# tenstack/batch-scheduler

Hardware: AMD Instinct MI355X
Metric: pod x node fit evals/sec (higher is better)
Workload: dtype int64; 1 GPU; cfg3/tail: 10000 pods / 2000 groups / 5000 nodes, 5 int64 lanes (cpu, mem, eph, pods, gpu), seed 20260921; stages=prefilter+filter+tally+ready, parallelism=single GPU

## Files before the change

### batch-scheduler_amd/build.py

```python
from __future__ import annotations

import os
import shutil
import subprocess

HERE = os.path.dirname(os.path.abspath(__file__))
CSRC = os.path.join(HERE, "csrc")
LIB_DIR = os.environ.get("BS_LIB_DIR") or HERE
PREBUILT_ONLY = bool(os.environ.get("BS_LIB_DIR"))
LIB_PATH = os.path.join(LIB_DIR, "libbsched.so")
_COMMON = ["bs_common.hpp", "bs_kernels.hpp", "bs_nodew_layout.hpp", "bs_lanes.hpp", os.path.join("..", "..", "include", "bsched.h")]
_CTX = _COMMON + ["bs_ctx.hpp", "bs_carve.hpp", "bs_hostmem.hpp", "bs_pod_ranges.hpp"]
_FAST = ["bs_launch.hpp", "bs_fast.hpp", "bs_filter_t.hpp"]
_SEQ = _CTX + ["bs_seq.hpp"]
UNITS = {
    "bsched.hip": _CTX + _FAST + ["bs_epoch.hpp", "bs_queue.hpp", "bs_fdeny.hpp", "bs_sort.hpp", "bs_fit.hpp"],
    "tu_fast.hip": _COMMON + _FAST,
    "tu_seq.hip": _SEQ,
    "tu_seq_expire.hip": _SEQ + ["bs_seq_expire.hpp", "bs_seq_expire_list.hpp"],
    "tu_preempt.hip": _CTX + ["bs_preempt.hpp", "bs_preempt_commit.hpp", "bs_preempt_commit_gang.hpp", "bs_preempt_gang_runs.hpp", "bs_preempt_geom.hpp", "bs_bound_apply.hpp",
                              "bs_bound_nodes.hpp", "bs_bound_nodes_replay.hpp", "bs_pdb.hpp"],
}
SOURCES = list(UNITS)
LATER_UNITS = {
    "tu_wait.hip": _SEQ + ["bs_wait.hpp", "bs_wait_list.hpp"],
}
ALL_UNITS = {**UNITS, **LATER_UNITS}
ALL_SOURCES = list(ALL_UNITS)
HEADERS = sorted({h for hs in ALL_UNITS.values() for h in hs})
OBJ_DIR = os.path.join(HERE, "build")
FLAGS = ["--offload-arch=gfx950", "-O3", "-std=c++17", "-fPIC", "-ffp-contract=off",
         "-fno-fast-math", "-Wall", "-Wno-unused-function"]


def hipcc() -> str:
    exe = shutil.which("hipcc") or "/opt/rocm/bin/hipcc"
    if not os.path.exists(exe):
        raise RuntimeError("hipcc not found: the gfx950 library cannot be built")
    return exe


HOST_LIB_PATH = os.path.join(LIB_DIR, "libbsched_host.so")
HOST_SRC = os.path.join(HERE, "host", "bs_host.cpp")
HOST_SRCS = [HOST_SRC, os.path.join(HERE, "host", "bs_drain.cpp"), os.path.join(HERE, "host", "bs_phase.cpp")]


def build_host(force: bool = False, verbose: bool = False) -> str:
    build()
    if PREBUILT_ONLY:
        return HOST_LIB_PATH
    deps = [*HOST_SRCS, os.path.join(HERE, "..", "include", "bsched.h"), os.path.join(HERE, "..", "include", "bsched_host.h"), LIB_PATH]
    if not force and os.path.exists(HOST_LIB_PATH) and all(os.path.getmtime(d) <= os.path.getmtime(HOST_LIB_PATH) for d in deps):
        return HOST_LIB_PATH
    cxx = shutil.which("g++") or "g++"
    tmp = f"{HOST_LIB_PATH}.{os.getpid()}.tmp"
    cmd = [cxx, "-O2", "-std=c++17", "-fPIC", "-shared", "-Wall", "-o", tmp, *HOST_SRCS, "-L" + HERE, "-lbsched",
           "-Wl,-rpath,$ORIGIN"]
    if verbose:
        print(" ".join(cmd))
    res = subprocess.run(cmd, capture_output=True, text=True)
    if res.returncode != 0:
        raise RuntimeError("g++ failed:\n" + res.stdout + res.stderr)
    os.replace(tmp, HOST_LIB_PATH)
    return HOST_LIB_PATH

# ... 77 lines not shown
```

### batch-scheduler_amd/capi.py

```python
from __future__ import annotations

import ctypes as C
import os

import numpy as np

from . import fitspec, soa

HERE = os.path.dirname(os.path.abspath(__file__))
LIB_PATH = os.path.join(os.environ.get("BS_LIB_DIR") or HERE, "libbsched.so")

KERNEL_COUNT = 8
KERNEL_PREPASS, KERNEL_LEADER, KERNEL_QUERY, KERNEL_TABLES, KERNEL_SCAN, KERNEL_RESOLVE, KERNEL_FILTER, KERNEL_TALLY = range(8)

ABI_SYMBOLS = [
    "bs_abi_version", "bs_strerror", "bs_last_error", "bs_create", "bs_destroy",
    "bs_nodes_load", "bs_fit_load", "bs_fit_build", "bs_fit_read", "bs_groups_load", "bs_groups_read", "bs_groups_apply", "bs_pods_map", "bs_pods_load",
    "bs_pods_apply", "bs_pods_count", "bs_pods_read", "bs_pods_apply_stats", "bs_filter_deny_stats", "bs_speculation_stats",
    "bs_nodes_apply", "bs_nodes_count", "bs_nodes_assume",
    "bs_cluster_fits", "bs_node_left", "bs_scan_prefix", "bs_cluster_total", "bs_filter_one", "bs_find_max_pg",
    "bs_batch_run", "bs_batch_sync", "bs_batch_read", "bs_batch_map", "bs_filter_rows_count", "bs_queue_order_load", "bs_queue_sort",
    "bs_shard_set", "bs_reduce_external", "bs_group_admit_devptr", "bs_group_admit_bind", "bs_stream", "bs_comm_unique_id", "bs_comm_init", "bs_batch_finish",
    "bs_timing_reset", "bs_timing_get", "bs_kernel_name", "bs_batch_stats_get",
    "bs_seq_run", "bs_nodes_read", "bs_first_reach_hint",
    "bs_nodes_load_flat", "bs_groups_load_flat", "bs_groups_read_flat", "bs_pods_load_flat", "bs_pods_apply_flat", "bs_pods_read_flat",
    "bs_batch_read_flat", "bs_seq_run_flat", "bs_fit_build_flat",
    "bs_bound_load", "bs_bound_count", "bs_preempt_run", "bs_bound_load_flat", "bs_preempt_run_flat",
    "bs_preempt_commit", "bs_bound_read", "bs_preempt_commit_flat",
    "bs_bound_pdb_set", "bs_preempt_pdb_read",
    "bs_bound_apply", "bs_bound_apply_flat", "bs_bound_ids", "bs_bound_dump",
    "bs_bound_nodes_apply",
    "bs_bound_apply_ex", "bs_bound_apply_ex_flat",
    "bs_pdb_load", "bs_pdb_members_append", "bs_pdb_allowed_apply", "bs_pdb_read",
    "bs_preempt_commit_gang", "bs_preempt_commit_gang_flat", "bs_preempt_gang_read",
    "bs_seq_expire", "bs_seq_expire_flat", "bs_seq_waiting_read",
    "bs_wait_load", "bs_wait_count", "bs_wait_ids", "bs_wait_read", "bs_wait_park", "bs_wait_release", "bs_wait_expire", "bs_wait_forget",
]

SEQ_EXPIRE_DENY, SEQ_EXPIRE_ALL = 1, 2
WAIT_MAX = 1 << 24

BS_BOUND_NODES = soa.BS_BOUND_NODES

PROTECTED_PHASES = (2, 5)


def group_protected(phases) -> np.ndarray:
    ph = np.asarray(phases, dtype=np.int64).reshape(-1)
    return np.isin(ph, PROTECTED_PHASES).astype(np.uint8)


def gang_order(pod_group, priority) -> np.ndarray:
    grp = np.asarray(pod_group, np.int64).reshape(-1)
    pri = np.asarray(priority, np.int64).reshape(-1)
    assert grp.shape == pri.shape
    first: dict = {}
    rank = np.zeros(grp.shape[0], np.int64)
    for i in range(grp.shape[0]):
        key = (int(pri[i]), int(grp[i])) if grp[i] >= 0 else (int(pri[i]), -1 - i)
        rank[i] = first.setdefault(key, i)
    return np.lexsort((np.arange(grp.shape[0]), rank, -pri)).astype(np.int64)


def gang_need(groups, waiting=None) -> np.ndarray:
    mm = np.asarray(groups.min_member, np.int64).reshape(-1)
    w = np.zeros_like(mm) if waiting is None else np.asarray(waiting, np.int64).reshape(-1)
    assert w.shape == mm.shape
    return np.clip(mm - np.asarray(groups.status_scheduled, np.int64).reshape(-1) - w, 0, None).astype(np.uint32)


class BsError(RuntimeError):
# ... 35 lines not shown

class SeqOut(C.Structure):
    _fields_ = [("pf_code", C.POINTER(C.c_uint8)), ("pf_first_k", C.POINTER(C.c_uint32)), ("pf_leader", C.POINTER(C.c_int32)),
                ("pod_node", C.POINTER(C.c_int32)), ("cap", C.c_uint32), ("released_group", C.POINTER(C.c_uint32)),
                ("released_pods", C.POINTER(C.c_uint32)), ("first_ns", C.POINTER(C.c_int64)), ("ready_ns", C.POINTER(C.c_int64)),
                ("n_released", C.c_uint32), ("total_ns", C.c_int64), ("node_picks", C.c_uint64), ("node_scans", C.c_uint64),
                ("scan_rounds", C.c_uint64), ("pick_rounds", C.c_uint64), ("leader_folds", C.c_uint64), ("table_builds", C.c_uint64),
                ("last_permitted", C.POINTER(C.c_uint8))]


class SeqExpireOut(C.Structure):
    _fields_ = [("n_groups", C.c_uint32), ("n_pods", C.c_uint32), ("group_cap", C.c_uint32), ("group", C.POINTER(C.c_uint32)),
                ("group_pods", C.POINTER(C.c_uint32)), ("group_earlier", C.POINTER(C.c_uint32)), ("pod_cap", C.c_uint32),
                ("pod", C.POINTER(C.c_uint32)), ("node", C.POINTER(C.c_uint32))]


_lib = None


def load_library(path: str | None = None):
    global _lib
    if _lib is not None and path is None:
        return _lib
    p = path or LIB_PATH
    if not os.path.exists(p):
        raise BsError(-2, "load_library", f"{p} not built: run `python __graft_entry__.py build` (hipcc, gfx950)")
    L = C.CDLL(p)
    vp, u32, i32, u8 = C.c_void_p, C.c_uint32, C.c_int32, C.c_uint8
    P = C.POINTER
    L.bs_abi_version.restype = u32
    L.bs_strerror.restype = C.c_char_p
    L.bs_strerror.argtypes = [C.c_int]
    L.bs_last_error.restype = C.c_char_p
    L.bs_last_error.argtypes = [vp]
    L.bs_kernel_name.restype = C.c_char_p
    L.bs_kernel_name.argtypes = [u32]
    L.bs_create.argtypes = [P(Config), P(vp)]
    L.bs_destroy.argtypes = [vp]
    L.bs_nodes_load.argtypes = [vp, P(soa.NodesStruct)]
    L.bs_fit_load.argtypes = [vp, u32, P(u32)]
    L.bs_fit_build.argtypes = [vp, P(fitspec.NodeLabelsStruct), P(fitspec.FitTemplatesStruct)]
    L.bs_fit_read.argtypes = [vp, P(u32)]
    L.bs_groups_load.argtypes = [vp, P(soa.GroupsStruct)]
    L.bs_groups_read.argtypes = [vp, P(soa.GroupsStruct)]
    L.bs_groups_apply.argtypes = [vp, P(soa.GroupDelta), u32]
    L.bs_filter_rows_count.argtypes = [vp, P(u32)]
    L.bs_pods_load.argtypes = [vp, P(soa.PodsStruct)]
    L.bs_pods_map.argtypes = [vp, u32, P(soa.PodsStruct)]
    L.bs_pods_apply.argtypes = [vp, P(soa.PodsDeltaStruct)]
    L.bs_pods_count.argtypes = [vp, P(u32)]
    L.bs_pods_apply_stats.argtypes = [vp, P(C.c_uint64), P(C.c_uint64)]
    L.bs_filter_deny_stats.argtypes = [vp, P(C.c_uint64)]
    L.bs_speculation_stats.argtypes = [vp, P(C.c_uint64), P(C.c_uint64)]
    L.bs_pods_read.argtypes = [vp, P(soa.PodsOutStruct)]
    L.bs_queue_order_load.argtypes = [vp, u32, P(u32)]
    L.bs_queue_sort.argtypes = [vp, u32, P(i32), P(i32), P(C.c_int64), P(u32)]
    L.bs_nodes_apply.argtypes = [vp, P(NodeDelta), u32]
    L.bs_nodes_count.argtypes = [vp, P(u32)]
    L.bs_nodes_assume.argtypes = [vp, P(NodeRequest), u32]
    L.bs_cluster_fits.argtypes = [vp, u32, C.c_float, P(C.c_int64), u32, P(u8), P(u32)]
    L.bs_node_left.argtypes = [vp, u32, C.c_float, P(C.c_int64), P(u32)]
    L.bs_scan_prefix.argtypes = [vp, u32, C.c_float, P(C.c_int64), P(u32), P(u32), P(u32)]
    L.bs_cluster_total.argtypes = [vp, u32, P(C.c_int64), P(u32)]
    L.bs_filter_one.argtypes = [vp, i32, P(C.c_int64), u32, i32, u32, P(u8), P(u8)]
    L.bs_find_max_pg.argtypes = [vp, P(i32), P(u32), P(u8)]
    L.bs_batch_run.argtypes = [vp, u32]
    L.bs_batch_sync.argtypes = [vp]
    L.bs_batch_read.argtypes = [vp, P(soa.BatchOutStruct)]
    L.bs_batch_map.argtypes = [vp, P(soa.BatchViewStruct)]
    L.bs_shard_set.argtypes = [vp, u32, u32]
    L.bs_group_admit_devptr.argtypes = [vp, P(vp), P(u32)]
    L.bs_reduce_external.argtypes = [vp, u32]
    L.bs_first_reach_hint.argtypes = [vp, u32]
    L.bs_group_admit_bind.argtypes = [vp, vp]
    L.bs_stream.argtypes = [vp, P(vp)]
    L.bs_comm_unique_id.argtypes = [P(u8)]
    L.bs_comm_init.argtypes = [vp, P(u8), u32, u32]
    L.bs_batch_finish.argtypes = [vp]
    L.bs_timing_reset.argtypes = [vp]
    L.bs_timing_get.argtypes = [vp, P(Timing)]
    L.bs_batch_stats_get.argtypes = [vp, P(BatchStats)]
    L.bs_seq_run.argtypes = [vp, u32, P(SeqOut)]
    L.bs_nodes_read.argtypes = [vp, P(C.c_int64), P(u32)]
    L.bs_bound_load.argtypes = [vp, P(soa.BoundStruct)]
    L.bs_bound_count.argtypes = [vp, P(u32)]
    L.bs_preempt_run.argtypes = [vp, u32, u32, P(u32), P(i32), P(u8), u32, P(soa.PreemptOutStruct)]
    L.bs_bound_load_flat.argtypes = [vp, u32, P(u32), P(i32), P(C.c_int64), P(i32), P(C.c_int64), P(u32)]
    L.bs_preempt_run_flat.argtypes = [vp, u32, u32, P(u32), P(i32), P(u8), u32, P(i32), P(u32), P(u32), P(u32), P(i32), P(C.c_int64), P(C.c_int64)]
    L.bs_preempt_commit.argtypes = [vp, u32, u32, P(u32), P(i32), P(u8), u32, u32, P(soa.PreemptOutStruct)]
    L.bs_bound_read.argtypes = [vp, P(u32), P(u32)]
    L.bs_bound_pdb_set.argtypes = [vp, u32, P(u8)]
    L.bs_bound_apply.argtypes = [vp, P(soa.BoundDeltaStruct), P(u32)]
    L.bs_bound_apply_flat.argtypes = [vp, u32, P(u32), u32, P(u32), P(i32), P(C.c_int64), P(i32), P(C.c_int64), P(u32), P(u8), P(u32)]
    L.bs_bound_apply_ex.argtypes = [vp, P(soa.BoundDeltaStruct), u32, P(u32)]
    L.bs_bound_apply_ex_flat.argtypes = [vp, u32, u32, P(u32), u32, P(u32), P(i32), P(C.c_int64), P(i32), P(C.c_int64), P(u32), P(u8), P(u32)]
    L.bs_bound_ids.argtypes = [vp, P(u32)]
    L.bs_bound_nodes_apply.argtypes = [vp, u32, P(u32), P(u32), u32, P(u32), P(u32)]
    L.bs_bound_dump.argtypes = [vp, P(i32), P(C.c_int64), P(i32), P(C.c_int64), P(u32), P(u8)]
    L.bs_preempt_pdb_read.argtypes = [vp, u32, P(u32)]
    L.bs_pdb_load.argtypes = [vp, u32, P(i32), u32, P(u32), P(u32)]
    L.bs_pdb_members_append.argtypes = [vp, u32, u32, P(u32), P(u32)]
    L.bs_pdb_allowed_apply.argtypes = [vp, u32, P(u32), P(i32)]
    L.bs_pdb_read.argtypes = [vp, P(u32), P(u32), P(i32), P(u32)]
    L.bs_preempt_commit_flat.argtypes = [vp, u32, u32, P(u32), P(i32), P(u8), u32, u32, P(i32), P(u32), P(u32), P(u32), P(i32), P(C.c_int64),
                                         P(C.c_int64)]
    L.bs_preempt_commit_gang.argtypes = [vp, u32, u32, P(u32), P(i32), P(u8), P(u32), u32, u32, P(soa.PreemptOutStruct)]
# ... 133 lines not shown
            return np.ctypeslib.as_array(C.cast(ptr, C.POINTER(ctype * n)).contents).view(dtype).reshape(shape)
        pods = soa.Pods.__new__(soa.Pods)
        pods.group = view(st.group, C.c_int32, np.int32, (p,))
        pods.req = view(st.req, C.c_int64, np.int64, (self.L, p))
        pods.req_present = view(st.req_present, C.c_uint32, np.uint32, (p,))
        pods.cls = view(st.cls, C.c_uint32, np.uint32, (p,))
        pods.owner = view(st.owner, C.c_uint64, np.uint64, (p,))
        pods.flags = view(st.flags, C.c_uint8, np.uint8, (p,))
        return pods

    def apply_group_deltas_raw(self, arr, n: int):
        self._chk(self._lib.bs_groups_apply(self._h, arr, n), "bs_groups_apply")

    def load_pods(self, pods: soa.Pods):
        assert pods.req.shape[0] == self.L
        st = pods.as_struct()
        self._chk(self._lib.bs_pods_load(self._h, C.byref(st)), "bs_pods_load")
        self.p = pods.p

    def apply_pods(self, remove=(), flag_index=(), flag_value=(), insert: soa.Pods | None = None, insert_at=None):
        rem = np.ascontiguousarray(remove, np.uint32)
        fi = np.ascontiguousarray(flag_index, np.uint32)
        fv = np.ascontiguousarray(flag_value, np.uint8)
        assert fi.shape == fv.shape
        d = soa.PodsDeltaStruct()
        d.n_remove, d.remove = len(rem), _u32p(rem if len(rem) else np.zeros(1, np.uint32))
        d.n_flags, d.flag_index = len(fi), _u32p(fi if len(fi) else np.zeros(1, np.uint32))
        d.flag_value = (fv if len(fv) else np.zeros(1, np.uint8)).ctypes.data_as(C.POINTER(C.c_uint8))
        keep = [rem, fi, fv]
        if insert is not None and insert.p:
            assert insert.req.shape[0] == self.L
            d.insert = insert.as_struct()
            if insert_at is not None:
                at = np.ascontiguousarray(insert_at, np.uint32)
                assert len(at) == insert.p
                keep.append(at)
                d.insert_at = _u32p(at)
        self._chk(self._lib.bs_pods_apply(self._h, C.byref(d)), "bs_pods_apply")
        self.p = self.pods_count()

    def apply_pods_raw(self, delta: "soa.PodsDeltaStruct"):
        self._chk(self._lib.bs_pods_apply(self._h, C.byref(delta)), "bs_pods_apply")

    def apply_stats(self) -> tuple[int, int]:
        a, r = C.c_uint64(0), C.c_uint64(0)
        self._chk(self._lib.bs_pods_apply_stats(self._h, C.byref(a), C.byref(r)), "bs_pods_apply_stats")
        return int(a.value), int(r.value)

    def speculation_stats(self) -> tuple[int, int]:
        a, m = C.c_uint64(0), C.c_uint64(0)
        self._chk(self._lib.bs_speculation_stats(self._h, C.byref(a), C.byref(m)), "bs_speculation_stats")
        return int(a.value), int(m.value)

    def filter_deny_reruns(self) -> int:
        r = C.c_uint64(0)
        self._chk(self._lib.bs_filter_deny_stats(self._h, C.byref(r)), "bs_filter_deny_stats")
        return int(r.value)

    def pods_count(self) -> int:
        n = C.c_uint32(0)
        self._chk(self._lib.bs_pods_count(self._h, C.byref(n)), "bs_pods_count")
        return int(n.value)

    def read_pods(self) -> soa.Pods:
        p = self.pods_count()
        out = soa.Pods.empty(max(p, 1), self.L)
        st = soa.PodsOutStruct(p, *[getattr(out.as_struct(), k) for k in ("group", "req", "req_present", "cls", "owner", "flags")])
        if p:
            out = soa.Pods.empty(p, self.L)
            s2 = out.as_struct()
            st = soa.PodsOutStruct(p, s2.group, s2.req, s2.req_present, s2.cls, s2.owner, s2.flags)
        self._chk(self._lib.bs_pods_read(self._h, C.byref(st)), "bs_pods_read")
        return out if p else soa.Pods.empty(0, self.L)

    def apply_node_deltas(self, deltas: list):
        arr = (NodeDelta * len(deltas))(*deltas)
        self._chk(self._lib.bs_nodes_apply(self._h, arr, len(deltas)), "bs_nodes_apply")
        n = C.c_uint32(0)
        self._chk(self._lib.bs_nodes_count(self._h, C.byref(n)), "bs_nodes_count")
        self.n = int(n.value)

    def assume_nodes(self, reqs):
        reqs = list(reqs)
        arr = (NodeRequest * max(len(reqs), 1))()
        for k, (idx, lanes, pres) in enumerate(reqs):
            arr[k].index, arr[k].requested_present = int(idx), int(pres)
            for j, v in enumerate(lanes):
                arr[k].requested[j] = int(v)
        self._chk(self._lib.bs_nodes_assume(self._h, arr, len(reqs)), "bs_nodes_assume")

    def cluster_fits(self, cls: int, pct: float, req, present: int = 0):
        r = np.zeros(soa.MAX_LANES, np.int64)
        r[: len(req)] = req
        fits, fk = C.c_uint8(0), C.c_uint32(0)
        self._chk(self._lib.bs_cluster_fits(self._h, cls, float(np.float32(pct)), _i64p(r), present, C.byref(fits), C.byref(fk)),
                  "bs_cluster_fits")
        return bool(fits.value), int(fk.value)

    def node_left(self, cls: int, pct: float):
        left = np.zeros((self.L, self.n), np.int64)
        present = np.zeros(max(self.n, 1), np.uint32)
        self._chk(self._lib.bs_node_left(self._h, cls, float(np.float32(pct)), _i64p(left), _u32p(present)), "bs_node_left")
        return left, present[: self.n]

    def scan_prefix(self, cls: int, pct: float):
        n = max(self.n, 1)
# ... 407 lines not shown
```

### batch-scheduler_amd/csrc/bs_ctx.hpp

```cpp
#pragma once
#include <rccl/rccl.h>

#include <algorithm>
#include <string>
#include <vector>

#include "bs_carve.hpp"
#include "bs_hostmem.hpp"
#include "bs_kernels.hpp"
#include "bs_lanes.hpp"
#include "bs_pod_ranges.hpp"

namespace bs {

struct EventPair { hipEvent_t a, b; uint32_t id; };

inline size_t align256(size_t x) { return (x + 255) & ~(size_t)255; }
template <class T>
T* at(T* p, size_t n) { return p ? p + n : nullptr; }

struct PodLayout {
  Piece<int32_t> group;
  Piece<int64_t> req;
  Piece<uint32_t> pres, cls, pclass, ppair;
  Piece<uint64_t> owner;
  Piece<uint8_t> flags;
  size_t in_bytes = 0, bytes = 0;
  uint32_t p = 0;
};
inline PodLayout pod_layout(uint32_t P, uint32_t L) {
  const size_t n = std::max<uint32_t>(P, 1);
  PodLayout l;
  Carve cv;
  l.group = cv.take<int32_t>(n);
  l.req = cv.take<int64_t>(n * L);
  l.pres = cv.take<uint32_t>(n);
  l.cls = cv.take<uint32_t>(n);
  l.owner = cv.take<uint64_t>(n);
  l.flags = cv.take<uint8_t>(n);
  l.in_bytes = cv.mark();
  l.pclass = cv.take<uint32_t>(n);
  l.ppair = cv.take<uint32_t>(n);
  l.bytes = cv.mark();
  l.p = P;
  return l;
}

extern const char* const kKernelNames[BS_KERNEL_COUNT];
int use_device(bs_ctx* c, bool flush = true);
int settle_pending(bs_ctx* c);
NodesDev nodes_dev(const bs_ctx* c);
GroupsDev groups_dev(const bs_ctx* c);
PodsDev pods_dev(const bs_ctx* c);
uint32_t* pclass_dev(const bs_ctx* c);
void launch_nodes_assume(bs_ctx* c, const bs_node_request* records, uint32_t n);
void mirror_node_requests(bs_ctx* c, const bs_node_request* records, uint32_t n);
void rederive_nodes(bs_ctx* c, uint32_t base0 = 0, uint32_t m_before = 0);
int analyse_groups(bs_ctx* c, bool rearm_scratch = true, const bs_group_delta* deltas = nullptr, uint32_t ndeltas = 0, bool defer = false);
int maybe_analyse_epochs(bs_ctx* c);
int check_handover(bs_ctx* c);

}

using namespace bs;

struct bs_ctx {
  bs_config cfg{};
  uint32_t L = 4, S = 0, LP = 4;
  std::string last_error;

  bool have_nodes = false, have_fit = false, have_groups = false, have_pods = false;
  uint32_t N = 0, Ncap = 0, M = 0, C = 0, fit_words = 0;
  DevBuf d_alloc, d_nreq, d_apres, d_rpres, d_nflags, d_fit, d_kmap, d_m, d_left4, d_lglob;
  DevBuf d_fitarena, d_fitcols;
  std::vector<int64_t> h_alloc, h_nreq;
  std::vector<uint32_t> h_apres, h_rpres, h_kmap;
  std::vector<uint8_t> h_nflags;
  std::vector<uint32_t> h_fit;

  uint32_t G = 0, n_uncaptured = 0;
  std::vector<uint32_t> h_gmatched, h_gcls;
  std::vector<uint8_t> h_gflags;
  int32_t steady_table = -1;
  int32_t steady_prev = -1;
  bool spec_active = false;
  int32_t spec_table = -1;
  uint32_t spec_stages = 0;
  uint32_t no_spec = 0;
  uint64_t n_spec = 0, n_spec_miss = 0;
  uint32_t host_probe = 0;
  uint64_t hp_ns[6] = {0, 0, 0, 0, 0, 0}, hp_n = 0, hp_t0 = 0, hp_t1 = 0;
  uint64_t early_filter_min = 200000000ull;
  DevBuf d_gpack, d_info, d_gdelta;
  Piece<uint32_t> off_gmm, off_gsc, off_gmatched, off_gcls, off_gmrpres;
  Piece<uint8_t> off_gflags;
  Piece<int64_t> off_gminres;
  Piece<uint64_t> off_gocc;
  size_t gpack_bytes = 0;
  int32_t info_tag = 0, kinfo_tag = 0;
  bool info_pending = false, kinfo_pending = false;
  uint32_t max_group_cls = 0, max_pod_cls = 0;
  uint32_t h_K = 0;
  uint32_t k_bound = 0;

  uint32_t P = 0;
  DevBuf d_pack[2], d_outpack;
  PodLayout lay[2], stage_lay;
  uint32_t cur_pack = 0;
  bool last_use_classes = false;
  uint32_t map_p = 0;
  DevBuf d_gstat2, d_cdir, d_pdir, d_ckeys, d_cpres, d_pkeys;
  uint32_t gstat_cur = 0;
  uint32_t pair_cap = 0, dir_slots = 0;
  uint32_t ids_used = 0;
  bool rep_valid = false;
  bool dirs_ready = false;
  uint32_t id_room = 0;
  uint32_t serial_insert_max = 2048;
  uint64_t n_applies = 0, n_rederives = 0;
  Piece<uint8_t> off_pf_code, off_fl_code, off_ready;
  Piece<uint32_t> off_pf_first_k, off_fl_feasible, off_fl_slot, off_admit;
  Piece<int32_t> off_pf_leader;
  size_t outpack_bytes = 0;

  DevBuf d_first_elig, d_first_owner, d_first_reject, d_first_pod, d_cap_epoch;
  DevBuf d_epoch, d_nepochs, d_leader_epoch, d_panic_epoch;
  DevBuf d_tcode, d_stage, d_leader_raw, d_first_row, d_first_row64, d_scan_rec, d_feas_rec, d_chunk_rec, d_qreq_s, d_qflags_s, d_qpos;
  DevBuf d_needed, d_qcount, d_ticket, d_desc;
  bool scratch_armed = false;
  bool side_ready = false;
  DevBuf d_tables, d_kp, d_stats, d_fparams, d_fflags, d_chunk_tot, d_blk_scratch, d_gmax, d_chunk_kp;
  DevBuf d_cls_slots, d_cls_rep, d_cls_id, d_qtab_s, d_fu_slot, d_uparams, d_uflags, d_uclaim, d_fu_bitmap, d_fu_feas;
  DevBuf d_nodew;
  bool batch_void = false;
  uint32_t tp_tmin = 768;
  bool no_nodew = false;
  uint32_t slot_keep = 0xFFFFFFFFu;
  uint32_t cls_cap = 0, hash_keep = 0x7FFFFFFFu, n_nominres = 0, scan_slots_cap = 0, filter_slots_cap = 0;
  DevBuf d_fl_bitmap, d_admit, d_ready, d_gcount, d_admit64, d_own_start;
  bool owner_ready = false;
  DevBuf d_order_rank, d_sort;
  uint32_t order_g = 0;
  DevBuf d_gstat, d_pair_next, d_pair_firstq, d_first_reach, d_qstamp_s, d_fast_reject, d_epoch_group;
  bool pairs_ready = false;
  bool bitmap_valid = false;
  bool last_fast = false;
  bool batch_since_pods = false;
  size_t off_hfeas = 0, off_htag = 0;
  uint32_t hstride = 0;
  int32_t host_tag = 0;
  bool last_host_out = false;
  uint32_t no_fast = 0;
  DevBuf d_run_of_epoch, d_run_leader, d_gslot, d_gfirstq;
// ... 127 lines not shown
```

### batch-scheduler_amd/csrc/bs_fast.hpp

```cpp
#pragma once

#include "bs_kernels.hpp"
#include "bs_filter_t.hpp"

#ifdef BS_NT_TABLES
#define BS_TBL_STORE(p, v) __builtin_nontemporal_store((v), (p))
#else
#define BS_TBL_STORE(p, v) (*(p) = (v))
#endif
namespace bs {

template <bool INL = false>
__device__ __forceinline__ void arm_tally(const GroupsDev& gr, const BatchDev& b, const BatchParams& prm, uint32_t i, uint32_t nthreads);

__device__ __forceinline__ const uint8_t* range_glocal(const BatchDev& b) { return reinterpret_cast<const uint8_t*>(b.pod_ranges); }
__device__ __forceinline__ const uint32_t* range_start(const BatchDev& b, uint32_t G) { return b.pod_ranges + (G + 3u) / 4u; }
__device__ __forceinline__ const uint32_t* range_lfirst(const BatchDev& b, uint32_t G, uint32_t pod_blocks) { return range_start(b, G) + pod_blocks + 1u; }
__device__ __forceinline__ bool range_local_on(const BatchDev& b, const BatchParams& prm) {
  return b.pod_ranges && prm.do_tally && prm.do_ready && !prm.filter_deny;
}

#if BS_EMIT_MAIN
__global__ void k_pods_prep(unsigned long long* tables, uint32_t ntab, uint32_t* gstat, uint32_t ngstat, uint32_t* kcount, uint32_t* gcount, uint32_t G) {
  const uint32_t t = blockIdx.x * blockDim.x + threadIdx.x, nt = gridDim.x * blockDim.x;
  for (uint32_t i = t; i < ntab; i += nt) tables[i] = 0ull;
  for (uint32_t i = t; i < G; i += nt) gcount[i] = 0;
  for (uint32_t i = t; i < ngstat; i += nt) gstat[i] = BS_INF;
  if (t == 0 && kcount) *kcount = 0;
}
#endif

#if BS_EMIT_MAIN
__global__ void k_pod_pairs(PodsDev pods, uint32_t G, const uint32_t* rep, const uint32_t* id, uint32_t* pclass, unsigned long long* slots, uint32_t mask,
                            uint32_t hash_keep, uint32_t* gstat, uint32_t* ppair, unsigned long long* pair_next, const uint32_t* kcount, int32_t tag,
                            int32_t* hinfo, uint32_t* gcount) {
  const uint32_t i = blockIdx.x * blockDim.x + threadIdx.x;
  if (i == 0 && hinfo) {
    __hip_atomic_store(reinterpret_cast<unsigned long long*>(&hinfo[4]), ((unsigned long long)(uint32_t)tag << 32) | *kcount, __ATOMIC_RELAXED, __HIP_MEMORY_SCOPE_SYSTEM);
  }
  {
    const int32_t gq = i < pods.p ? pods.group[i] : -1;
    const bool in = gq >= 0 && (uint32_t)gq < G;
    wave_aggregated_add(gcount, in ? (uint32_t)gq : 0u, in);
  }
  if (i >= pods.p) return;
  const uint32_t c = id[rep[i]];
  if (pclass) pclass[i] = c;
  const int32_t gi = pods.group[i];
  if (gi < 0 || (uint32_t)gi >= G) { ppair[i] = BS_INF; return; }
  atomicMin(&gstat[gi], i);
  if (!(pods.flags[i] & BS_POD_LAST_PERMITTED)) {
    atomicMin(&gstat[(size_t)G + gi], i);
    if (pods.owner[i] != 0) atomicMin(&gstat[(size_t)2 * G + gi], i);
// ... 162 lines not shown
      incl[j] += off;
      if (valid) BS_TBL_STORE(&T[(size_t)k * LP + j], (int64_t)incl[j]);
      if (threadIdx.x == 0) b.chunk_tot[(size_t)chunk * 16 + j] = tot;
    } else if (j < LP && valid) {
      BS_TBL_STORE(&T[(size_t)k * LP + j], (int64_t)INT64_MAX);
    }
  }
  {
    const uint32_t grp = k >> 6;
    const bool grp_valid = (chunk * kTblChunk + (threadIdx.x & ~63u)) < nd.m;
    constexpr int64_t kSafe = (int64_t)1 << 62;
#pragma unroll
    for (uint32_t j = 0; j < BS_MAX_LANES; ++j) {
      if (j < L) {
        const int64_t x = (int64_t)incl[j];
        const long long mx = wave_max_i64_lane63(valid ? x : INT64_MIN);
        const bool risky = __ballot(valid && (x >= kSafe || x <= -kSafe)) != 0ull;
        if (lane_id() == 63 && grp_valid) b.gmax[(size_t)grp * LP + j] = risky ? INT64_MAX : mx;
      }
    }
  }
#pragma unroll
  for (uint32_t s = 0; s < BS_MAX_SCALARS; ++s) {
    if (s < S) {
      const unsigned long long mk = __ballot(valid && (pres & (1u << s)));
      if (mk && lane_id() == 0) atomicMin(&s_kp[s], chunk * kTblChunk + (uint32_t)(threadIdx.x & ~63u) + (uint32_t)(__ffsll((long long)mk) - 1));
    }
  }
  __syncthreads();
  if (threadIdx.x < 16) b.chunk_kp[(size_t)chunk * 16 + threadIdx.x] = threadIdx.x < BS_MAX_SCALARS ? s_kp[threadIdx.x] : BS_INF;
}

struct LeaderPre { Res mr; bool have_mr; int64_t min_member, status_scheduled, matched; };
template <bool PUB, typename T>
__device__ __forceinline__ void st_pub(T* p, T v) {
  if constexpr (PUB) __hip_atomic_store(p, v, __ATOMIC_RELAXED, __HIP_MEMORY_SCOPE_AGENT);
  else *p = v;
}
#ifndef BS_HOME_WT
#define BS_HOME_WT 0
#endif
template <typename T>
__device__ __forceinline__ void st_home(T* p, T v) {
#if BS_HOME_WT
  __hip_atomic_store(p, v, __ATOMIC_RELAXED, __HIP_MEMORY_SCOPE_SYSTEM);
#else
  *p = v;
#endif
}
__device__ __forceinline__ uint32_t ld_agent(const uint32_t* p) { return __hip_atomic_load(p, __ATOMIC_RELAXED, __HIP_MEMORY_SCOPE_AGENT); }
__device__ __forceinline__ unsigned long long ld_agent64(const void* p) {
  return __hip_atomic_load(reinterpret_cast<const unsigned long long*>(p), __ATOMIC_RELAXED, __HIP_MEMORY_SCOPE_AGENT);
}
template <int TS>
__device__ __forceinline__ void leader_pre_load(const GroupsDev& gr, int32_t leader, Shape<TS> sh, LeaderPre& o) {
  const uint32_t l = leader >= 0 ? (uint32_t)leader : 0u;
#pragma unroll
  for (uint32_t j = 0; j < BS_MAX_LANES; ++j) o.mr.v[j] = j < sh.L() ? gr.minres[(size_t)j * gr.g + l] : 0;
  o.mr.present = gr.mrpres[l];
  o.have_mr = (gr.flags[l] & BS_GROUP_HAS_MINRES) != 0;
  o.min_member = (int64_t)gr.min_member[l];
  o.status_scheduled = (int64_t)gr.status_scheduled[l];
  o.matched = (int64_t)gr.matched[l];
}
template <int TS>
__device__ __forceinline__ void pre_allocated_from(const LeaderPre& lp, Shape<TS> sh, uint32_t gate, Res& out) {
  res_zero(out, sh);
  const int64_t mm = lp.min_member;
  const int64_t not_finished = lp.matched != 0 ? mm - lp.matched : mm - lp.status_scheduled;
  if (not_finished > 0 && lp.have_mr) {
    Res times;
#pragma unroll
    for (uint32_t j = 0; j < BS_MAX_LANES; ++j)
      if (j < sh.L()) times.v[j] = wmul(lp.mr.v[j], not_finished);
    times.present = lp.mr.present;
    res_add(out, times, sh, gate);
  }
  if (out.v[BS_LANE_PODS] == 0) out.v[BS_LANE_PODS] = mm + 1;
}
template <int TS>
__device__ __forceinline__ uint32_t filter_slot_values(const Res& cur_in, const LeaderPre& lp, Shape<TS> sh, uint32_t gate, int64_t (&R)[4], int64_t (&M)[4]) {
  Res ms, cur = cur_in;
  res_zero(ms, sh);
  res_add(ms, lp.mr, sh, gate);
  res_add(cur, ms, sh, gate);
  uint32_t ff = 0;
#pragma unroll
  for (uint32_t s = 0; s < BS_MAX_SCALARS; ++s) {
    if (s < sh.S()) {
      if ((cur.present & (1u << s)) && cur.v[4 + s] != 0) ff |= 1u;
      if ((ms.present & (1u << s)) && ms.v[4 + s] != 0) ff |= 2u;
    }
  }
#pragma unroll
  for (int j = 0; j < 4; ++j) { R[j] = cur.v[j]; M[j] = ms.v[j]; }
  return ff;
}
template <int TS, bool PUB = false>
__device__ __forceinline__ void filter_slot_from(const BatchDev& b, const BatchParams& prm, const Res& cur_in, const LeaderPre& lp, Shape<TS> sh, uint32_t gate,
                                                 uint32_t slot, bool zero_feas = true) {
  if (!lp.have_mr) return;
  int64_t R[4], M[4];
  const uint32_t ff = filter_slot_values(cur_in, lp, sh, gate, R, M);
  if (zero_feas) st_pub<PUB>(&b.fu_feas[slot], 0u);
  int64_t* dst2 = b.uparams + (size_t)slot * 8;
#pragma unroll
  for (int j = 0; j < 4; ++j) { st_pub<PUB>(&dst2[j], R[j]); st_pub<PUB>(&dst2[4 + j], M[j]); }
  st_pub<PUB>(&b.uflags[slot], ff | ((uint32_t)BS_FL_EVALUATED << 8) | (prm.stamp << 16));
}
template <int TS>
__device__ __forceinline__ uint32_t class_scan_query(const Res& cur, const LeaderPre& lp0, Shape<TS> sh, uint32_t gate, Res& q) {
  pre_allocated_from(lp0, sh, gate, q);
  res_add(q, cur, sh, gate);
  uint32_t absok = 0;
#pragma unroll
  for (uint32_t s2 = 0; s2 < BS_MAX_SCALARS; ++s2) {
    if (s2 < sh.S()) {
      const bool pres = q.present & (1u << s2);
      if (!pres || q.v[4 + s2] == 0) absok |= 1u << s2;
      if (!pres) q.v[4 + s2] = INT64_MIN;
    }
  }
  return q.present | (absok << 16);
}

template <int TS, bool PUB = false, bool SLOTS = true, bool INL = false>
__device__ __forceinline__ void fast_query_thread(const PodsDev& pods, const GroupsDev& gr, const BatchDev& b, const BatchParams& prm, uint32_t i,
                                                  uint32_t nthreads, uint32_t end = BS_INF, uint32_t t = BS_INF) {
  const Shape<TS> sh(prm.S);
  const bool valid = i < pods.p && i < end;
  const uint32_t gate = prm.eph_gate;
  const uint32_t ii = valid ? i : 0u;
  const int32_t leader0 = b.leader_epoch[0];
  const uint8_t panic0 = b.panic_epoch[0];
  const uint32_t K = prm.run_filter ? (prm.k_host ? prm.k_host : *b.kclass) : 0u;
  const int32_t gi = pods.p ? pods.group[ii] : BS_POD_NOT_GROUPED;
  const uint8_t pfl = pods.p ? pods.flags[ii] : (uint8_t)0;
  const uint64_t own = pods.p ? pods.owner[ii] : 0ull;
  const uint32_t pc = pods.p ? b.pclass[ii] : 0u;
  const uint32_t pp = pods.p ? b.ppair[ii] : BS_INF;
  Res cur;
  if (pods.p) pod_require(pods, ii, sh, gate, cur); else res_zero(cur, sh);
  arm_tally<INL>(gr, b, prm, t == BS_INF ? i : t, nthreads);
  if (i < 8 && prm.collect_stats) b.stats[i] = 0;
  const bool grouped = valid && gi >= 0 && (uint32_t)gi < gr.g;
  const uint32_t g = grouped ? (uint32_t)gi : 0u;
  const uint8_t gfl = gr.g ? gr.flags[g] : (uint8_t)0;
  const uint64_t occ0 = gr.g ? gr.occupied[g] : 0ull;
  const uint32_t fo = gr.g ? b.first_owner_s[g] : BS_INF;
  const uint32_t anchor = grouped ? b.first_pod_s[g] : i;
  LeaderPre lp0{}, lp1{};
  const bool two = prm.run_filter && prm.sop_leader0 >= 0 && prm.sop_leader0 != leader0;
  if (gr.g) {
    leader_pre_load(gr, leader0, sh, lp0);
    if (two) leader_pre_load(gr, prm.sop_leader0, sh, lp1); else lp1 = lp0;
  }
  const bool need_fo = grouped && occ0 == 0 && fo != BS_INF && i > fo;
  const uint64_t occ_fo = need_fo ? pods.owner[fo] : 0ull;
  const uint32_t owner_rank = valid ? owner_rank_of(b, prm, anchor, pods.p) : 0u;

  uint8_t code = BS_PF_PASS_NOT_GROUPED, st = 0;
  bool has_q = false;
  Res q;
  res_zero(q, sh);
  if (valid) {
    if (owner_rank == prm.rank) st |= ST_OWNED;
    if (gi == BS_POD_NOT_GROUPED) code = BS_PF_PASS_NOT_GROUPED;
    else if (pfl & BS_POD_LAST_PERMITTED) code = BS_PF_PASS_LAST_PERMITTED;
    else if (!grouped) code = BS_PF_ERR_PG_NOT_FOUND;
    else if ((gfl & BS_GROUP_DENIED) || fd_denied(b, (uint32_t)gi, i)) code = BS_PF_ERR_DENIED;
    else {
      st |= ST_ELIG;
      bool occ_err = false;
      if (occ0 != 0) occ_err = (own == 0) || (own != occ0);
      else if (need_fo) occ_err = (own == 0) || (own != occ_fo);
      if (occ_err) code = BS_PF_ERR_OCCUPIED;
      else if (panic0) code = BS_PF_PANIC_DIV0;
      else {
        st |= ST_REACH6;
        if (leader0 < 0) code = BS_PF_PASS_NO_MAX;
        else if (leader0 == gi) code = BS_PF_PASS_IS_MAX;
        else {
          pre_allocated_from(lp0, sh, gate, q);
          res_add(q, cur, sh, gate);
          code = BS_PF_PASS_RESERVE_FITS;
          has_q = (st & ST_OWNED) != 0;
        }
// ... 126 lines not shown
               : [a0] "v"(a[0]), [r0] "v"(r[0]), [a1] "v"(a[1]), [r1] "v"(r[1]), [a2] "v"(a[2]), [r2] "v"(r[2]), [a3] "v"(a[3]), [r3] "v"(r[3])
               : "vcc");
#pragma unroll
  for (int j = 4; j < NL; ++j)
    asm volatile("s_mov_b64 exec, %[m]\n\tv_cmpx_ge_i64 vcc, %[a], %[r]\n\ts_mov_b64 %[m], exec\n\ts_mov_b64 exec, -1" : [m] "+s"(m) : [a] "v"(a[j]), [r] "v"(r[j]) : "vcc");
  return m;
}
#ifndef BS_SCAN_BALLOT
#define BS_SCAN_BALLOT 1
#endif
constexpr uint32_t kSpinBound = 1u << 18;
__device__ __forceinline__ void test_chaos_delay() {
#ifdef BS_TEST_CHAOS
  uint32_t h = (blockIdx.x + 1u) * 2654435761u ^ (uint32_t)wall_clock64() * 40503u;
  h ^= h >> 15; h *= 2246822519u; h ^= h >> 13;
  for (uint32_t s = 0; s < (h & 15u); ++s) __builtin_amdgcn_s_sleep(127);
#endif
}
constexpr uint32_t kStepSlotsMax = 256;
__device__ __forceinline__ bool step_wait(const uint32_t* word, uint32_t base, uint32_t need, int32_t* h_err) {
  uint32_t spins = 0;
  while ((uint32_t)(ld_agent(word) - base) < need) {
    __builtin_amdgcn_s_sleep(1);
    if (++spins > kSpinBound) { if (h_err) __hip_atomic_store(h_err, 1, __ATOMIC_RELAXED, __HIP_MEMORY_SCOPE_SYSTEM); return false; }
  }
  return true;
}
constexpr uint32_t kScanRecChunks = 64;
constexpr uint32_t kFeasRecGroups = 32;
#ifndef BS_GATHER_DIRECT
#define BS_GATHER_DIRECT 8
#endif
constexpr uint32_t kGatherDirectBlocks = BS_GATHER_DIRECT;
constexpr uint32_t kRecStride = 32;
constexpr uint32_t kTkSlots = 32, kTkTab = 48, kTkP1 = 64, kTkDone = 64 + 16 * 16, kTkWays = 16, kTkWords = 64 + 2 * 16 * 16;
__device__ __forceinline__ void spread_add(uint32_t* words, uint32_t who) {
  (void)__hip_atomic_fetch_add(&words[16u * (who % kTkWays)], 1u, __ATOMIC_RELAXED, __HIP_MEMORY_SCOPE_AGENT);
}
__device__ __forceinline__ bool spread_wait(const uint32_t* words, uint32_t base, uint32_t need, int32_t* h_err) {
  uint32_t spins = 0;
  for (;;) {
    uint32_t v = lane_id() < (int)kTkWays ? ld_agent(&words[16u * (uint32_t)lane_id()]) : 0u;
#pragma unroll
    for (int o = 1; o < (int)kTkWays; o <<= 1) v += (uint32_t)__shfl_xor((int)v, o);
    v = (uint32_t)__builtin_amdgcn_readfirstlane((int)v);
    if ((uint32_t)(v - base) >= need) return true;
    __builtin_amdgcn_s_sleep(4);
    if (++spins > kSpinBound) { if (h_err && lane_id() == 0) __hip_atomic_store(h_err, 1, __ATOMIC_RELAXED, __HIP_MEMORY_SCOPE_SYSTEM); return false; }
  }
}
template <int TS, bool REGS = false>
__device__ __forceinline__ void table_scan_block(const NodesDev& nd, const BatchDev& b, const BatchParams& prm, const TableDesc* forced, uint32_t chunk, uint32_t nchunks,
                                                 uint32_t share, uint32_t nshares, uint32_t pod_blocks, uint32_t tk_pods0, uint32_t tk_tab0, const GroupsDev& gr,
                                                 const int64_t* ckeys, const uint32_t* cpres, uint32_t kcap, bool direct = false, uint32_t forced_cls = 0) {
  __shared__ unsigned long long s_wtot[BS_MAX_LANES][4];
  __shared__ uint32_t s_kp[BS_MAX_SCALARS];
  __shared__ unsigned long long s_off[BS_MAX_LANES];
  __shared__ uint32_t s_kpg[BS_MAX_SCALARS];
  __shared__ int64_t s_req[kStepSlotsMax][BS_MAX_LANES];
  __shared__ uint32_t s_qf[kStepSlotsMax];
  __shared__ uint32_t s_first[kStepSlotsMax];
  BS_STAMP(2, 0);
  const Shape<TS> sh(prm.S);
  const uint32_t L = sh.L(), S = sh.S(), LP = prm.LP;
  const uint32_t k = chunk * kTblChunk + threadIdx.x;
  const bool in_range = REGS ? k < nd.n : k < nd.m;
  const uint32_t n = REGS ? (in_range ? k : 0u) : (in_range ? nd.kmap[k] : 0u);
  const TableDesc d = REGS ? TableDesc{forced_cls, 0.7f} : *forced;
  const uint32_t fw = nd.fit[(size_t)d.cls * nd.fit_words + (n >> 5)];
  const uint8_t fl = nd.flags[n];
  const bool valid = in_range && (!REGS || !(fl & BS_NODE_SKIP_MASK));
  const uint32_t ap = nd.apres[n], rp = nd.rpres[n];
  int64_t al[BS_MAX_LANES], rq[BS_MAX_LANES];
#pragma unroll
  for (uint32_t j = 0; j < BS_MAX_LANES; ++j) {
    if (j < L) {
      al[j] = nd.alloc[(size_t)j * nd.stride + n];
      rq[j] = nd.req[(size_t)j * nd.stride + n];
    }
  }
  const uint32_t K = prm.k_host ? prm.k_host : *b.kclass;
  const uint32_t per = (K + nshares - 1u) / nshares, s_lo = share * per, s_hi = min(K, s_lo + per);
  Res raw;
  int32_t leader0 = -1;
  uint8_t panic0 = 0;
  LeaderPre lp0{};
  if constexpr (REGS) {
    const uint32_t cc = s_lo + threadIdx.x < s_hi ? s_lo + threadIdx.x : 0u;
#pragma unroll
    for (uint32_t j = 0; j < BS_MAX_LANES; ++j)
      if (j < L) raw.v[j] = ckeys[(size_t)j * kcap + cc];
    raw.present = cpres[cc];
    leader0 = b.leader_epoch[0];
    panic0 = b.panic_epoch[0];
    if (gr.g) leader_pre_load(gr, leader0, sh, lp0);
  }
  const bool fit = valid && ((fw >> (n & 31u)) & 1u) && !(fl & BS_NODE_TAINT_ERR);
  const uint32_t pres = fit ? (ap & rp) : 0u;
  if (threadIdx.x < BS_MAX_SCALARS) s_kp[threadIdx.x] = BS_INF;
  for (uint32_t t = threadIdx.x; t < kStepSlotsMax; t += kTblChunk) s_first[t] = BS_INF;
  unsigned long long incl[BS_MAX_LANES];
  const int w = wave_id();
#pragma unroll
  for (uint32_t j = 0; j < BS_MAX_LANES; ++j) {
    incl[j] = 0;
    if (j < L) {
      const bool live = fit && (j < 4 || (pres & (1u << (j - 4)))) && !(j == BS_LANE_EPH && !prm.eph_gate);
      const unsigned long long left = live ? (unsigned long long)wsub(scale_f32(al[j], d.pct), rq[j]) : 0ull;
      incl[j] = wave_incl_scan_add_u64(left);
      if (lane_id() == 63) s_wtot[j][w] = incl[j];
    }
  }
  __syncthreads();
#pragma unroll
  for (uint32_t s2 = 0; s2 < BS_MAX_SCALARS; ++s2) {
    if (s2 < S) {
      const unsigned long long mk = __ballot(valid && (pres & (1u << s2)));
      if (mk && lane_id() == 0) atomicMin(&s_kp[s2], chunk * kTblChunk + (uint32_t)(threadIdx.x & ~63u) + (uint32_t)(__ffsll((long long)mk) - 1));
    }
  }
#pragma unroll
  for (uint32_t j = 0; j < BS_MAX_LANES; ++j) {
    if (j < L) {
      unsigned long long off = 0, tot = 0;
#pragma unroll
      for (int i = 0; i < 4; ++i) {
        const unsigned long long x = s_wtot[j][i];
        if (i < w) off += x;
        tot += x;
      }
      incl[j] += off;
      if (threadIdx.x == 0 && share == 0) {
        if constexpr (REGS) {
          const unsigned long long tag = (unsigned long long)prm.seq_inv << 32;
          st_pub<true>(&b.chunk_rec[(size_t)chunk * kRecStride + 2u * j], tag | (uint32_t)tot);
          st_pub<true>(&b.chunk_rec[(size_t)chunk * kRecStride + 2u * j + 1u], tag | (uint32_t)(tot >> 32));
        } else {
          st_pub<true>(&b.chunk_tot[(size_t)chunk * 16 + j], tot);
        }
      }
    }
  }
  __syncthreads();
  __shared__ uint32_t s_ok;
  if constexpr (REGS) {
    if (share == 0 && threadIdx.x < S) st_pub<true>(&b.chunk_rec[(size_t)chunk * kRecStride + 16u + threadIdx.x], ((unsigned long long)prm.seq_inv << 32) | s_kp[threadIdx.x]);
    BS_STAMP(2, 1);
  } else {
    if (share == 0 && threadIdx.x < 16) st_pub<true>(&b.chunk_kp[(size_t)chunk * 16 + threadIdx.x], threadIdx.x < BS_MAX_SCALARS ? s_kp[threadIdx.x] : BS_INF);
    asm volatile("s_waitcnt vmcnt(0)" ::: "memory");
    __syncthreads();
    BS_STAMP(2, 1);
    if (threadIdx.x == 0 && share == 0) (void)__hip_atomic_fetch_add(&b.ticket[kTkTab], 1u, __ATOMIC_RELAXED, __HIP_MEMORY_SCOPE_AGENT);
  }
  if constexpr (REGS) {
    const uint32_t t = s_lo + threadIdx.x;
    if (t < s_hi) {
      uint32_t qf = 0x80000000u;
      Res q;
      res_zero(q, sh);
      if (leader0 >= 0 && !panic0) {
        Res cur;
        res_zero(cur, sh);
        res_add(cur, raw, sh, prm.eph_gate);
        qf = class_scan_query(cur, lp0, sh, prm.eph_gate, q);
      }
      s_qf[threadIdx.x] = qf;
#pragma unroll
      for (uint32_t j = 0; j < BS_MAX_LANES; ++j)
        if (j < L) s_req[threadIdx.x][j] = q.v[j];
    }
  }
  if constexpr (!REGS) {
    if (threadIdx.x == 0) s_ok = (step_wait(&b.ticket[kTkTab], tk_tab0, nchunks, b.h_err) && step_wait(&b.ticket[kTkSlots], tk_pods0, pod_blocks, b.h_err)) ? 1u : 0u;
    __syncthreads();
    BS_STAMP(2, 2);
    if (!s_ok) return;
  }
  {
    const uint32_t ch = (uint32_t)lane_id();
    unsigned long long cv[BS_MAX_LANES];
    uint32_t ckp[BS_MAX_SCALARS];
    if constexpr (REGS) {
      if (w == 0) {
        const uint32_t tagw = prm.seq_inv;
        const unsigned long long* rec = b.chunk_rec + (size_t)(ch < nchunks ? ch : 0u) * kRecStride;
        bool ok = false;
        for (uint32_t spins = 0;; ++spins) {
          unsigned long long lo[BS_MAX_LANES], hi[BS_MAX_LANES], kw[BS_MAX_SCALARS];
#pragma unroll
          for (uint32_t j = 0; j < BS_MAX_LANES; ++j)
            if (j < L) { lo[j] = ld_agent64(&rec[2u * j]); hi[j] = ld_agent64(&rec[2u * j + 1u]); }
#pragma unroll
          for (uint32_t s2 = 0; s2 < BS_MAX_SCALARS; ++s2)
            if (s2 < S) kw[s2] = ld_agent64(&rec[16u + s2]);
          bool mine_ok = true;
#pragma unroll
          for (uint32_t j = 0; j < BS_MAX_LANES; ++j) {
            cv[j] = 0ull;
            if (j < L) {
              mine_ok = mine_ok && (uint32_t)(lo[j] >> 32) == tagw && (uint32_t)(hi[j] >> 32) == tagw;
              cv[j] = (hi[j] << 32) | (uint32_t)lo[j];
            }
          }
#pragma unroll
          for (uint32_t s2 = 0; s2 < BS_MAX_SCALARS; ++s2) {
            ckp[s2] = BS_INF;
            if (s2 < S) { mine_ok = mine_ok && (uint32_t)(kw[s2] >> 32) == tagw; ckp[s2] = (uint32_t)kw[s2]; }
          }
          if (__ballot(!(mine_ok || ch >= nchunks)) == 0ull) { ok = true; break; }
          if (spins > kSpinBound) { if (b.h_err && ch == 0) __hip_atomic_store(b.h_err, 1, __ATOMIC_RELAXED, __HIP_MEMORY_SCOPE_SYSTEM); break; }
          __builtin_amdgcn_s_sleep(2);
        }
        if (ch >= nchunks) {
#pragma unroll
          for (uint32_t j = 0; j < BS_MAX_LANES; ++j) cv[j] = 0ull;
#pragma unroll
          for (uint32_t s2 = 0; s2 < BS_MAX_SCALARS; ++s2) ckp[s2] = BS_INF;
        }
        if (ch == 0) s_ok = ok ? 1u : 0u;
      }
      BS_STAMP(2, 2);
    } else if (w == 0) {
#pragma unroll
      for (uint32_t j = 0; j < BS_MAX_LANES; ++j) cv[j] = (j < L && ch < nchunks) ? ld_agent64(&b.chunk_tot[(size_t)ch * 16 + j]) : 0ull;
#pragma unroll
      for (uint32_t s2 = 0; s2 < BS_MAX_SCALARS; ++s2) ckp[s2] = (s2 < S && ch < nchunks) ? ld_agent(&b.chunk_kp[(size_t)ch * 16 + s2]) : BS_INF;
    }
    const uint32_t t = s_lo + threadIdx.x;
    uint32_t stp = 0, qf = 0x80000000u;
    int32_t tab = -1;
    unsigned long long rv[BS_MAX_LANES];
    if (!REGS && t < s_hi) {
      stp = ld_agent(&b.qstamp_s[t]);
      tab = (int32_t)ld_agent(reinterpret_cast<const uint32_t*>(&b.qtab_s[t]));
      qf = ld_agent(&b.qflags_s[t]);
#pragma unroll
      for (uint32_t j = 0; j < BS_MAX_LANES; ++j) rv[j] = j < L ? ld_agent64(&b.qreq_s[(size_t)t * LP + j]) : 0ull;
    }
    if (w == 0) {
#pragma unroll
      for (uint32_t j = 0; j < BS_MAX_LANES; ++j) {
        if (j < L) {
          const unsigned long long incl_c = wave_incl_scan_add_u64(cv[j]);
          const unsigned long long mine = bcast64(incl_c - cv[j], (int)(chunk & 63u));
          if (ch == 0) s_off[j] = mine;
        }
      }
#pragma unroll
      for (uint32_t s2 = 0; s2 < BS_MAX_SCALARS; ++s2) {
        if (s2 < S) {
          const uint32_t mn = wave_min_u32(ckp[s2]);
          if (ch == 0) s_kpg[s2] = mn;
        }
      }
    }
    if (!REGS && t < s_hi) {
      if (stp != prm.stamp || tab != 0) qf = 0x80000000u;
      s_qf[threadIdx.x] = qf;
#pragma unroll
      for (uint32_t j = 0; j < BS_MAX_LANES; ++j)
        if (j < L) s_req[threadIdx.x][j] = (int64_t)rv[j];
    }
  }
  __syncthreads();
  if constexpr (REGS) {
    if (!s_ok) return;
  }
  int64_t fin[BS_MAX_LANES];
  uint32_t keyrow = 0;
#pragma unroll
  for (uint32_t j = 0; j < BS_MAX_LANES; ++j) {
    fin[j] = 0;
    if (j < L) fin[j] = (int64_t)(incl[j] + s_off[j]);
  }
#pragma unroll
  for (uint32_t s2 = 0; s2 < BS_MAX_SCALARS; ++s2)
    if (s2 < S && k >= s_kpg[s2]) keyrow |= 1u << s2;
  BS_STAMP(2, 3);
  const uint32_t nmine = s_hi > s_lo ? s_hi - s_lo : 0u;
  const uint32_t smask = S ? ((1u << S) - 1u) : 0u;
  const uint32_t row0 = chunk * kTblChunk + ((uint32_t)w << 6);
  for (uint32_t t0 = 0; t0 < nmine; t0 += 4u) {
    uint32_t qf[4];
    int64_t r[4][BS_MAX_LANES];
#pragma unroll
    for (uint32_t u = 0; u < 4; ++u) {
      const uint32_t t = min(t0 + u, nmine - 1u);
      qf[u] = t0 + u < nmine ? s_qf[t] : 0x80000000u;
#pragma unroll
      for (uint32_t j = 0; j < BS_MAX_LANES; ++j) r[u][j] = j < L ? s_req[t][j] : 0;
    }
#pragma unroll
    for (uint32_t u = 0; u < 4; ++u) {
      const uint32_t nab = ~(qf[u] >> 16) & smask;
      unsigned long long m = (qf[u] & 0x80000000u) ? 0ull : __ballot(valid && (nab & ~keyrow) == 0u);
      static_assert(TS >= 0 && TS <= 4, "k_fast_step_a is instantiated for 0..4 scalar lanes (run_fast: step_a_possible)");
#if BS_SCAN_BALLOT
#pragma unroll
      for (uint32_t j = 0; j < 4u + (uint32_t)TS; ++j) m &= __ballot(fin[j] >= r[u][j]);
#else
      m = rows_cover<4 + TS>(m, fin, r[u]);
#endif
      if (m && lane_id() == 0) atomicMin(&s_first[t0 + u], row0 + (uint32_t)(__ffsll((long long)m) - 1));
    }
  }
  __syncthreads();
  BS_STAMP(2, 4);
  if constexpr (REGS) {
    if (direct) {
      for (uint32_t t = threadIdx.x; t < nmine; t += kTblChunk)
        st_pub<true>(&b.scan_rec[(size_t)chunk * kStepSlotsMax + s_lo + t], ((unsigned long long)prm.seq_inv << 32) | s_first[t]);
    } else {
      for (uint32_t t = threadIdx.x; t < nmine; t += kTblChunk)
        if (s_first[t] != BS_INF) atomicMin(&b.first_row64[s_lo + t], ((unsigned long long)prm.seq_inv << 32) | s_first[t]);
    }
    BS_STAMP(2, 7);
    return;
  }
  for (uint32_t t = threadIdx.x; t < nmine; t += kTblChunk) {
    if (s_first[t] == BS_INF) continue;
    atomicMin(&b.first_row[s_lo + t], s_first[t]);
  }
  BS_STAMP(2, 7);
}

__device__ __forceinline__ void step_filter_split(uint32_t K, uint32_t W, uint32_t target_waves, uint32_t& tiles, uint32_t& bpw, uint32_t& nchunk) {
  tiles = (2u * K + 63u) / 64u;
  uint32_t nsplit = max(1u, target_waves / max(tiles, 1u));
  nsplit = min(nsplit, max((W + 1u) / 2u, 1u));
  bpw = max(2u, (((W + nsplit - 1u) / nsplit + 1u) / 2u) * 2u);
  nchunk = (W + bpw - 1u) / bpw;
  if ((nchunk + 3u) / 4u > kFeasRecGroups) {
    bpw = ((W + 4u * kFeasRecGroups - 1u) / (4u * kFeasRecGroups) + 1u) / 2u * 2u;
    nchunk = (W + bpw - 1u) / bpw;
  }
}
template <int TS>
__device__ __forceinline__ void step_filter_block(const GroupsDev& gr, const NodesDev& nd, const BatchDev& b, const BatchParams& prm, const int64_t* ckeys,
                                                  const uint32_t* cpres, uint32_t kcap, uint32_t target_waves, uint32_t ustride, uint32_t bx, uint32_t nblocks,
                                                  bool direct, uint32_t tk_slots0, uint32_t slot_producers) {
  __shared__ uint32_t s_cnt[4][64];
  BS_STAMP_AT(4, 0, bx);
  const Shape<TS> sh(prm.S);
  const uint32_t gate = prm.eph_gate, K = prm.k_host ? prm.k_host : (uint32_t)__builtin_amdgcn_readfirstlane((int)*b.kclass), U = 2u * K;
  const uint32_t W = (nd.n + 63u) / 64u;
  if (!U || !W) return;
  uint32_t tiles, bpw, nchunk;
  step_filter_split(K, W, target_waves, tiles, bpw, nchunk);
  const uint32_t groups = (nchunk + 3u) / 4u;
  const int32_t leader0 = b.leader_epoch[0];
  LeaderPre lp0{}, lp1{};
  const bool two = prm.sop_leader0 >= 0 && prm.sop_leader0 != leader0;
  if (gr.g) {
    leader_pre_load(gr, leader0, sh, lp0);
    if (two) leader_pre_load(gr, prm.sop_leader0, sh, lp1); else lp1 = lp0;
  }
  bool waited = false;
  for (uint32_t bi = bx; bi < tiles * groups; bi += nblocks) {
    const uint32_t tile = bi % tiles, group = bi / tiles, chunk = group * 4u + (uint32_t)wave_id();
    const uint32_t src = tile * 64u + (uint32_t)lane_id();
    const bool second = src >= K;
    const uint32_t c = src < U ? (second ? src - K : src) : 0u;
    uint32_t cnt = 0;
    if (chunk < nchunk) {
      Res raw;
#pragma unroll
      for (uint32_t j = 0; j < BS_MAX_LANES; ++j)
        if (j < sh.L()) raw.v[j] = ckeys[(size_t)j * kcap + c];
      raw.present = cpres[c];
      Res cur;
      res_zero(cur, sh);
      res_add(cur, raw, sh, gate);
      LeaderPre lp = lp0;
      if (second) lp = lp1;
      const bool on = src < U && (second ? prm.sop_leader0 >= 0 : leader0 >= 0) && lp.have_mr;
      int64_t R[4], M[4];
      const uint32_t ff = filter_slot_values(cur, lp, sh, gate, R, M);
      filter_item<2, 4, true, true>(nd, b, U, ustride, tile, chunk * bpw, min(W, chunk * bpw + bpw), 0u,
                                    on ? (ff | ((uint32_t)BS_FL_EVALUATED << 8)) : ((uint32_t)BS_FL_NOT_RUN << 8), R, M, &cnt);
    }
    s_cnt[wave_id()][lane_id()] = cnt;
    BS_STAMP_AT(4, 1, bx);
    if (direct && b.h_rows) asm volatile("s_waitcnt vmcnt(0)" ::: "memory");
    __syncthreads();
    BS_STAMP_AT(4, 2, bx);
    if (wave_id() == 0 && src < U) {
      const uint32_t sum = s_cnt[0][lane_id()] + s_cnt[1][lane_id()] + s_cnt[2][lane_id()] + s_cnt[3][lane_id()];
      if (direct) {
        st_pub<true>(&b.feas_rec[(size_t)group * (2u * kStepSlotsMax) + src], ((unsigned long long)prm.seq_inv << 32) | sum);
      } else {
        if (!waited) { (void)step_wait(&b.ticket[kTkSlots], tk_slots0, slot_producers, b.h_err); waited = true; }
        if (sum) atomicAdd(&b.fu_feas[src], sum);
      }
    }
    __syncthreads();
  }
  BS_STAMP_AT(4, 7, bx);
}

template <int TS>
__device__ __forceinline__ void class_slots_block(const GroupsDev& gr, const BatchDev& b, const BatchParams& prm, const int64_t* ckeys, const uint32_t* cpres,
                                                  uint32_t kcap, uint32_t blk, bool zero_feas) {
  const Shape<TS> sh(prm.S);
#ifdef BS_TEST_OLD_ZERO
  zero_feas = true;
#endif
  const uint32_t gate = prm.eph_gate, K = prm.k_host ? prm.k_host : *b.kclass;
  const uint32_t c = blk * kTblChunk + threadIdx.x;
  Res raw;
  const uint32_t cc = c < K ? c : 0u;
#pragma unroll
  for (uint32_t j = 0; j < BS_MAX_LANES; ++j)
    if (j < sh.L()) raw.v[j] = ckeys[(size_t)j * kcap + cc];
  raw.present = cpres[cc];
  const int32_t leader0 = b.leader_epoch[0];
  const uint8_t panic0 = b.panic_epoch[0];
  LeaderPre lp0{}, lp1{};
  const bool two = prm.run_filter && prm.sop_leader0 >= 0 && prm.sop_leader0 != leader0;
  if (gr.g) {
    leader_pre_load(gr, leader0, sh, lp0);
    if (two) leader_pre_load(gr, prm.sop_leader0, sh, lp1); else lp1 = lp0;
  }
  if (c < K) {
    Res cur;
    res_zero(cur, sh);
    res_add(cur, raw, sh, gate);
    if (leader0 >= 0 && !panic0) {
      Res q;
      const uint32_t qfw = class_scan_query(cur, lp0, sh, gate, q);
      int64_t* dst = b.qreq_s + (size_t)c * prm.LP;
#pragma unroll
      for (uint32_t j = 0; j < BS_MAX_LANES; ++j)
        if (j < prm.LP) st_pub<true>(&dst[j], j < sh.L() ? q.v[j] : (int64_t)INT64_MIN);
      st_pub<true>(&b.qflags_s[c], qfw);
      st_pub<true>(&b.qtab_s[c], (int32_t)0);
      st_pub<true>(&b.first_row[c], BS_INF);
      st_pub<true>(&b.qstamp_s[c], prm.stamp);
    }
    if (prm.run_filter) {
      if (leader0 >= 0) filter_slot_from<TS, true>(b, prm, cur, lp0, sh, gate, c, zero_feas);
      if (prm.sop_leader0 >= 0) filter_slot_from<TS, true>(b, prm, cur, lp1, sh, gate, c + K, zero_feas);
    }
  }
  BS_STAMP(1, 4);
  asm volatile("s_waitcnt vmcnt(0)" ::: "memory");
  __syncthreads();
  BS_STAMP(1, 5);
  if (threadIdx.x == 0) (void)__hip_atomic_fetch_add(&b.ticket[kTkSlots], 1u, __ATOMIC_RELAXED, __HIP_MEMORY_SCOPE_AGENT);
}


template <bool INL>
__device__ __forceinline__ void arm_tally(const GroupsDev& gr, const BatchDev& b, const BatchParams& prm, uint32_t i, uint32_t nthreads) {
  if (i == 0) __hip_atomic_store(&b.ticket[1], 0u, __ATOMIC_RELAXED, __HIP_MEMORY_SCOPE_AGENT);
  for (uint32_t g = i; g < gr.g; g += nthreads) {
    if (INL && range_local_on(b, prm) && range_glocal(b)[g]) continue;
    st_pub<INL>(&b.admit[g], 0u);
    if (prm.do_ready) {
      st_pub<INL>(&b.admit64[g], 0ull);
      if (b.gcount[g] == 0u) {
        const uint8_t rd = gr.matched[g] >= (uint32_t)(gr.min_member[g] - gr.status_scheduled[g]) ? 1 : 0;
        b.ready[g] = rd;
        if (prm.host_tag) { st_home(&b.h_admit[g], 0u); st_home(&b.h_ready[g], rd); }
      }
    }
  }
}

template <bool WT = false>
// ... 330 lines not shown
#endif
template <int S>
__global__ __launch_bounds__(256) __attribute__((amdgpu_waves_per_eu(S <= 1 ? 4 : 1))) void k_fast_scan_filter_t(NodesDev nd, BatchDev bt, BatchParams prm, uint32_t m, uint32_t jcap, uint32_t scan_blocks,
                                                            uint32_t filter_waves, uint32_t ustride, uint32_t form) {
  __shared__ int64_t s_rows[4][64][4 + S];
  const uint32_t filter_first = form & 1u, by_tile = form & 2u;
  const uint32_t filter_blocks = gridDim.x - scan_blocks;
  const bool is_scan = filter_first ? blockIdx.x >= filter_blocks : blockIdx.x < scan_blocks;
  BS_STAMP(2, 0);
  if (is_scan)
    scan_loop<S, true, 1>(bt, prm, m, jcap, 0u, 0u, 1u, filter_first ? blockIdx.x - filter_blocks : blockIdx.x, scan_blocks, s_rows[wave_id()]);
  else
    filter_loop_t<true>(nd, bt, filter_waves, ustride, prm.collect_stats, filter_first ? blockIdx.x : blockIdx.x - scan_blocks, filter_blocks, prm.stamp, 2u * prm.k_host, by_tile);
  BS_STAMP(2, 7);
}
#if BS_EMIT_MAIN
__global__ __launch_bounds__(256) void k_fast_final(PodsDev pods, GroupsDev gr, NodesDev nd, BatchDev b, BatchParams prm, uint32_t query_blocks) {
  fast_final_block(pods, gr, nd, b, prm, query_blocks, blockIdx.x, gridDim.x, 0u);
}
#endif

template <int S>
__global__ __launch_bounds__(256) void k_fast_scan_filter_final(PodsDev pods, GroupsDev gr, NodesDev nd, BatchDev b, BatchDev bt, BatchParams prm, uint32_t m,
                                                                uint32_t jcap, uint32_t scan_blocks, uint32_t filter_blocks, uint32_t filter_waves,
                                                                uint32_t ustride, uint32_t query_blocks) {
  __shared__ int64_t s_rows[4][64][4 + S];
  const uint32_t producers = scan_blocks + filter_blocks;
  test_chaos_delay();
#ifdef BS_TEST_LATE_ROLE_B
  {
    const int role = blockIdx.x < scan_blocks ? 0 : blockIdx.x < producers ? 1 : 2;
    if (role == BS_TEST_LATE_ROLE_B) for (int spin = 0; spin < 20; ++spin) __builtin_amdgcn_s_sleep(127);
  }
#endif
  if (blockIdx.x < producers) {
    BS_STAMP(2, 0);
    if (blockIdx.x < scan_blocks)
      scan_loop<S, true, 2>(bt, prm, m, jcap, 0u, 0u, 1u, blockIdx.x, scan_blocks, s_rows[wave_id()]);
    else
      filter_loop<2>(pods, nd, bt, filter_waves, 1u, ustride, prm.collect_stats, blockIdx.x - scan_blocks, filter_blocks, prm.stamp, 2u * prm.k_host);
    asm volatile("s_waitcnt vmcnt(0)" ::: "memory");
    __syncthreads();
    if (threadIdx.x == 0) (void)__hip_atomic_fetch_add(&b.ticket[1], 1u, __ATOMIC_RELAXED, __HIP_MEMORY_SCOPE_AGENT);
    BS_STAMP(2, 7);
    return;
  }
  fast_final_block(pods, gr, nd, b, prm, query_blocks, blockIdx.x - producers, gridDim.x - producers, producers);
}

template <int TS, bool WHOLE>
__global__ __launch_bounds__(kTblChunk) void k_fast_step_a(PodsDev pods, GroupsDev gr, NodesDev nd, BatchDev b, BatchDev bt, BatchParams prm, const TableDesc* forced,
                                                           uint32_t nchunks, uint32_t query_blocks, uint32_t nshares, uint32_t filter_blocks, uint32_t filter_waves,
                                                           uint32_t ustride, uint32_t tk_pods0, uint32_t tk_tab0, uint32_t param_blocks, const int64_t* ckeys,
                                                           const uint32_t* cpres, uint32_t kcap, uint32_t tk_p1, uint32_t tk_done, uint32_t forced_cls) {
  BS_STAMP(1, 0);
  test_chaos_delay();
  const uint32_t tb = nchunks * nshares;
#ifdef BS_TEST_LATE_ROLE
  {
    const int role = blockIdx.x < query_blocks ? 0 : blockIdx.x < query_blocks + param_blocks ? 1 : blockIdx.x < query_blocks + param_blocks + tb ? 2 : 3;
    if (role == BS_TEST_LATE_ROLE) for (int spin = 0; spin < 20; ++spin) __builtin_amdgcn_s_sleep(127);
  }
#endif
  const uint32_t producers = param_blocks ? param_blocks : query_blocks;
  const bool direct = query_blocks <= kGatherDirectBlocks;
  if (blockIdx.x < query_blocks) {
    if constexpr (WHOLE) {
      const uint32_t p0 = b.pod_ranges ? range_start(b, gr.g)[blockIdx.x] : blockIdx.x * kTblChunk;
      const uint32_t p1 = b.pod_ranges ? range_start(b, gr.g)[blockIdx.x + 1u] : pods.p;
      fast_query_thread<TS, false, false, true>(pods, gr, b, prm, p0 + threadIdx.x, query_blocks * kTblChunk, p1, blockIdx.x * kTblChunk + threadIdx.x);
      asm volatile("s_waitcnt vmcnt(0)" ::: "memory");
      __syncthreads();
      if (threadIdx.x == 0) spread_add(&b.ticket[kTkP1], blockIdx.x);
      fast_final_block<true>(pods, gr, nd, b, prm, query_blocks, blockIdx.x, query_blocks, nchunks, tk_p1, filter_waves, tk_done, tb + filter_blocks, p0, p1);
    } else if (param_blocks) {
      fast_query_thread<TS, false, false>(pods, gr, b, prm, blockIdx.x * kTblChunk + threadIdx.x, query_blocks * kTblChunk);
    } else {
      fast_query_thread<TS, true>(pods, gr, b, prm, blockIdx.x * kTblChunk + threadIdx.x, query_blocks * kTblChunk);
      BS_STAMP(1, 4);
      asm volatile("s_waitcnt vmcnt(0)" ::: "memory");
      __syncthreads();
      BS_STAMP(1, 5);
      if (threadIdx.x == 0) (void)__hip_atomic_fetch_add(&b.ticket[kTkSlots], 1u, __ATOMIC_RELAXED, __HIP_MEMORY_SCOPE_AGENT);
    }
  } else if (blockIdx.x < query_blocks + param_blocks) {
    class_slots_block<TS>(gr, b, prm, ckeys, cpres, kcap, blockIdx.x - query_blocks, !(WHOLE && direct));
  } else if (blockIdx.x < query_blocks + param_blocks + tb) {
    const uint32_t x = blockIdx.x - query_blocks - param_blocks;
    table_scan_block<TS, WHOLE>(nd, bt, prm, forced, x / nshares, nchunks, x % nshares, nshares, producers, tk_pods0, tk_tab0, gr, ckeys, cpres, kcap, direct, forced_cls);
    if constexpr (WHOLE) {
      if (!direct) {
        asm volatile("s_waitcnt vmcnt(0)" ::: "memory");
        __syncthreads();
        if (threadIdx.x == 0) spread_add(&b.ticket[kTkDone], blockIdx.x);
      }
    }
  } else if constexpr (WHOLE) {
    step_filter_block<TS>(gr, nd, bt, prm, ckeys, cpres, kcap, filter_waves, ustride, blockIdx.x - query_blocks - param_blocks - tb, filter_blocks, direct, tk_pods0, producers);
    if (!direct) {
      asm volatile("s_waitcnt vmcnt(0)" ::: "memory");
      __syncthreads();
      if (threadIdx.x == 0) spread_add(&b.ticket[kTkDone], blockIdx.x);
    }
  } else {
    __shared__ uint32_t s_go;
    if (threadIdx.x == 0) {
      s_go = step_wait(&b.ticket[kTkSlots], tk_pods0, producers, b.h_err) ? 1u : 0u;
      __builtin_amdgcn_fence(__ATOMIC_ACQUIRE, "agent");
    }
    __syncthreads();
    if (!s_go) return;
    filter_loop<2>(pods, nd, bt, filter_waves, 1u, ustride, prm.collect_stats, blockIdx.x - query_blocks - param_blocks - tb, filter_blocks, prm.stamp, 2u * prm.k_host);
  }
  BS_STAMP(1, 7);
}


template <int TS>
__global__ __launch_bounds__(kTblChunk) void k_tables_local_nofix(NodesDev nd, BatchDev b, BatchParams prm, uint32_t nchunks, uint32_t cstride,
                                                                  uint32_t gstride) {
  const uint32_t slot = blockIdx.x;
  if (!b.needed[slot]) return;
  BatchDev bt = b;
  bt.tables = b.tables + (size_t)slot * prm.mcap * prm.LP;
  bt.kp = b.kp + (size_t)slot * 16;
  bt.chunk_tot = b.chunk_tot + (size_t)slot * cstride * 16;
  bt.chunk_kp = b.chunk_kp + (size_t)slot * cstride * 16;
  bt.gmax = b.gmax + (size_t)slot * gstride * prm.LP;
  const TableDesc d = table_desc(slot, prm.C, nullptr);
  tables_local_fast<TS>(nd, bt, prm, &d, blockIdx.y);
}

#if BS_EMIT_MAIN
__global__ __launch_bounds__(kLeaderBlock) void k_leader_scan(GroupsDev gr, BatchDev b) {
  __shared__ unsigned long long s_w[kLeaderBlock / 64];
  __shared__ uint32_t s_p[kLeaderBlock / 64];
  __shared__ unsigned long long s_carry;
  __shared__ uint32_t s_pcarry, s_nexact, s_exact[64];
  const uint32_t E1 = *b.nepochs;
  auto key_of = [&](uint32_t g, bool& panic) -> unsigned long long {
    if (gr.flags[g] & BS_GROUP_SCHEDULED_LATCH) return 0ull;
    const uint32_t f = leader_finished(gr, g, panic);
    return (((unsigned long long)f + 1ull) << 31) | (unsigned long long)(0x7FFFFFFFu - g);
  };
  unsigned long long k0 = 0;
  bool p0 = false;
  for (uint32_t g = threadIdx.x; g < gr.g; g += kLeaderBlock)
    if (b.cap_epoch[g] == 0u) { const unsigned long long k = key_of(g, p0); k0 = k > k0 ? k : k0; }
  {
    const unsigned long long m = block_max_u64(k0, s_w);
    const unsigned long long anyp = __ballot(p0);
// ... 76 lines not shown
```

### batch-scheduler_amd/csrc/bs_launch.hpp

```cpp
#pragma once
#include <hip/hip_runtime.h>
#include <stdint.h>

#include "bs_kernels.hpp"
#include "bs_lanes.hpp"

namespace bs {

struct FastLaunch {
  hipStream_t stream;
  uint32_t S, M, P, filter_waves, filter_slots_cap, tp_filter;
  int device;
  uint32_t filter_split = 0;
};
void launch_fast_bc(const FastLaunch& c, dim3 grid, const PodsDev& pd, const GroupsDev& gr, const NodesDev& nd, const BatchDev& b, const BatchDev& bt,
                    const BatchParams& prm, uint32_t nseg, uint32_t scan_blocks, uint32_t filter_blocks);
void launch_fast_b(const FastLaunch& c, dim3 grid, const PodsDev& pd, const NodesDev& nd, const BatchDev& bt, const BatchParams& prm, uint32_t nseg,
                   uint32_t scan_blocks);
void launch_fast_scan(const FastLaunch& c, dim3 grid, const BatchDev& bt, const BatchParams& prm, uint32_t nseg);
void launch_fast_bt(const FastLaunch& c, dim3 grid, const NodesDev& nd, const BatchDev& bt, const BatchParams& prm, uint32_t nseg, uint32_t scan_blocks);
void launch_fast_filter(const FastLaunch& c, dim3 grid, const PodsDev& pd, const NodesDev& nd, const BatchDev& bt, const BatchParams& prm);
int fused_residency_query(const FastLaunch& c);
void launch_fast_step_a(const FastLaunch& c, dim3 grid, const PodsDev& pd, const GroupsDev& gr, const NodesDev& nd, const BatchDev& b, const BatchDev& bt,
                        const BatchParams& prm, const TableDesc* forced, uint32_t nchunks, uint32_t query_blocks, uint32_t nshares, uint32_t filter_blocks,
                        uint32_t tk_pods0, uint32_t tk_tab0, uint32_t param_blocks, const int64_t* ckeys, const uint32_t* cpres, uint32_t kcap,
                        uint32_t whole, uint32_t tk_p1, uint32_t tk_done, uint32_t forced_cls);
int step_a_residency_query(const FastLaunch& c, bool whole);

}
```

### batch-scheduler_amd/csrc/bsched.hip

```cpp
#include <dlfcn.h>
#include <hip/hip_runtime.h>

#include <algorithm>
#include <cstdio>
#include <cstdlib>
#include <cstring>
#include <new>
#include <string>
#include <vector>

#ifndef BS_UNITY
#define BS_TU_MAIN
#endif
#include "bs_ctx.hpp"
#include "bs_fast.hpp"
#include "bs_epoch.hpp"
#include "bs_sort.hpp"
#include "bs_fit.hpp"
#include "bs_queue.hpp"
#include "bs_fdeny.hpp"
#include "bs_launch.hpp"
#ifdef BS_UNITY
#include "tu_fast.hip"
#include "tu_seq.hip"
// ... 155 lines not shown
  b.ready = c->off_ready.in(ok);
  return b;
}
BatchParams batch_params(const bs_ctx* c) {
  BatchParams p{};
  p.L = c->L; p.S = c->S; p.LP = c->LP; p.C = c->C;
  p.eph_gate = c->cfg.eph_gate;
  p.rank = c->reduce_external ? 0u : c->rank;
  p.nranks = c->reduce_external ? 1u : c->nranks;
  p.sop_leader0 = c->sop_leader0;
  p.run_filter = 0;
  p.hash_keep = c->hash_keep;
  p.use_classes = 0;
  p.scan_slots_cap = 0;
  p.filter_slots_cap = 0;
  p.collect_stats = c->collect_stats;
  p.mcap = c->table_mcap;
  p.filter_deny = c->fd_on ? 1u : 0u;
  p.fd_iter = c->fd_iter;
  p.first_reach_hint = c->reduce_external ? c->first_reach_hint : BS_INF;
  return p;
}

int reserve_filled(bs_ctx* c, DevBuf& d, size_t bytes, int byte_value) {
  const void* before = d.p;
  HIPCHK(c, d.reserve(bytes));
  if (d.p != before) HIPCHK(c, hipMemsetAsync(d.p, byte_value, d.cap, c->stream));
  return BS_OK;
}

int ensure_tables(bs_ctx* c) {
  if (!c->have_nodes || !c->have_fit) return BS_OK;
  const uint32_t slots = 2 * c->C + 1;
  const size_t bytes = (size_t)slots * c->Ncap * c->LP * sizeof(int64_t);
  if (bytes > ((size_t)64 << 30)) { c->last_error = "table storage exceeds 64 GiB"; return BS_ERR_CAPACITY; }
  HIPCHK(c, c->d_tables.reserve(bytes));
  HIPCHK(c, c->d_kp.reserve((size_t)slots * 16 * sizeof(uint32_t)));
  HIPCHK(c, c->d_chunk_tot.reserve((size_t)slots * cdiv(c->Ncap, 256) * 16 * 8));
  HIPCHK(c, c->d_gmax.reserve((size_t)slots * cdiv(c->Ncap, 64) * c->LP * 8));
  HIPCHK(c, c->d_chunk_kp.reserve((size_t)slots * cdiv(c->Ncap, 256) * 16 * 4));
  HIPCHK(c, c->d_desc.reserve((size_t)slots * sizeof(TableDesc)));
  HIPCHK(c, c->d_needed.reserve((size_t)(2 * c->C + 1) * 4));
  HIPCHK(c, c->d_qcount.reserve(16));
  HIPCHK(c, c->d_stats.reserve(8 * sizeof(uint64_t)));
  HIPCHK(c, c->d_sq.reserve(4096));
  c->table_slots = slots;
  c->table_mcap = c->Ncap;
  c->epochs_ready = false;
  return BS_OK;
}

int upload_nodes(bs_ctx* c, uint32_t lo = 0) {
  const uint32_t N = c->N, L = c->L;
  if (N > c->Ncap || c->Ncap == 0) {
    c->Ncap = std::max<uint32_t>(64, N + N / 4 + 64);
    c->d_tables.release();
    lo = 0;
  }
  const size_t cap = c->Ncap;
  const size_t old_cap_bytes = c->d_alloc.cap;
  HIPCHK(c, c->d_alloc.reserve(cap * L * 8));
  if (c->d_alloc.cap != old_cap_bytes) lo = 0;
  HIPCHK(c, c->d_nreq.reserve(cap * L * 8));
  HIPCHK(c, c->d_left4.reserve(cap * 4 * 8 + 128 * 8));
  HIPCHK(c, c->d_lglob.reserve(64));
  HIPCHK(c, c->d_apres.reserve(cap * 4));
  HIPCHK(c, c->d_rpres.reserve(cap * 4));
  HIPCHK(c, c->d_nflags.reserve(cap));
  HIPCHK(c, c->d_kmap.reserve(cap * 4));
  HIPCHK(c, c->d_m.reserve(16));
  lo = std::min(lo, N);
  const uint32_t base0 = (lo / kScanBlock) * kScanBlock;
  const uint32_t cnt = N - base0;
  if (cnt) {
    for (uint32_t j = 0; j < L; ++j) {
      HIPCHK(c, hipMemcpyAsync(c->d_alloc.as<int64_t>() + j * cap + base0, c->h_alloc.data() + (size_t)j * N + base0, (size_t)cnt * 8, hipMemcpyHostToDevice, c->stream));
      HIPCHK(c, hipMemcpyAsync(c->d_nreq.as<int64_t>() + j * cap + base0, c->h_nreq.data() + (size_t)j * N + base0, (size_t)cnt * 8, hipMemcpyHostToDevice, c->stream));
    }
    HIPCHK(c, hipMemcpyAsync(c->d_apres.as<uint32_t>() + base0, c->h_apres.data() + base0, (size_t)cnt * 4, hipMemcpyHostToDevice, c->stream));
    HIPCHK(c, hipMemcpyAsync(c->d_rpres.as<uint32_t>() + base0, c->h_rpres.data() + base0, (size_t)cnt * 4, hipMemcpyHostToDevice, c->stream));
    HIPCHK(c, hipMemcpyAsync(c->d_nflags.as<uint8_t>() + base0, c->h_nflags.data() + base0, (size_t)cnt, hipMemcpyHostToDevice, c->stream));
  }
  uint32_t m_before = 0;
  if (base0) m_before = (uint32_t)(std::lower_bound(c->h_kmap.begin(), c->h_kmap.end(), base0) - c->h_kmap.begin());
  rederive_nodes(c, base0, m_before);
  HIPCHK(c, hipGetLastError());
  uint32_t m = 0;
  HIPCHK(c, hipMemcpyAsync(&m, c->d_m.p, 4, hipMemcpyDeviceToHost, c->stream));
  HIPCHK(c, hipStreamSynchronize(c->stream));
  c->M = m;
  c->h_kmap.resize(m);
  if (m > m_before) HIPCHK(c, hipMemcpy(c->h_kmap.data() + m_before, c->d_kmap.as<uint32_t>() + m_before, (size_t)(m - m_before) * 4, hipMemcpyDeviceToHost));
  c->have_nodes = true;
  return ensure_tables(c);
}

int upload_fit(bs_ctx* c) {
  HIPCHK(c, c->d_fit.reserve(std::max<size_t>(4, c->h_fit.size() * 4)));
  if (!c->h_fit.empty())
    HIPCHK(c, hipMemcpyAsync(c->d_fit.p, c->h_fit.data(), c->h_fit.size() * 4, hipMemcpyHostToDevice, c->stream));
  HIPCHK(c, hipStreamSynchronize(c->stream));
  c->have_fit = true;
  return ensure_tables(c);
}

template <int S>
void launch_scan_s(bs_ctx* c, dim3 grid, const BatchDev& b, const BatchParams& p, uint32_t m, uint32_t nseg, uint32_t nslots, uint32_t ng, uint32_t ts,
                   bool local) {
  if (local) hipLaunchKernelGGL(HIP_KERNEL_NAME(k_scan<S, true>), grid, dim3(256), 0, c->stream, b, p, m, nseg, nslots, ng, ts);
  else hipLaunchKernelGGL(HIP_KERNEL_NAME(k_scan<S, false>), grid, dim3(256), 0, c->stream, b, p, m, nseg, nslots, ng, ts);
}
void launch_scan(bs_ctx* c, dim3 grid, const BatchDev& b, const BatchParams& p, uint32_t m, uint32_t nseg, uint32_t nslots, uint32_t ng, uint32_t ts,
                 bool local = false) {
  lanes_wide(c->S, [&](auto s) { launch_scan_s<decltype(s)::value>(c, grid, b, p, m, nseg, nslots, ng, ts, local); });
}

void launch_tables_local(bs_ctx* c, hipStream_t st, dim3 grid, const NodesDev& nd, const BatchDev& b, const BatchParams& p, const TableDesc* forced) {
  lanes_narrow(c->S, [&](auto s) { hipLaunchKernelGGL(HIP_KERNEL_NAME(k_tables_local<decltype(s)::value>), grid, dim3(kTblChunk), 0, st, nd, b, p, forced); });
}

template <int S>
void launch_scan_filter_s(bs_ctx* c, uint32_t scan_blocks, uint32_t filter_blocks, const PodsDev& pd, const NodesDev& nd, const BatchDev& b,
                          const BatchParams& p, uint32_t m, uint32_t jcap, uint32_t nslots, uint32_t ng, uint32_t ts, bool local) {
  if (local)
    hipLaunchKernelGGL(HIP_KERNEL_NAME(k_scan_filter<S, true>), dim3(scan_blocks + filter_blocks), dim3(256), 0, c->stream, pd, nd, b, p, m, jcap, nslots,
                       ng, ts, scan_blocks, c->filter_waves, c->filter_slots_cap);
  else
    hipLaunchKernelGGL(HIP_KERNEL_NAME(k_scan_filter<S, false>), dim3(scan_blocks + filter_blocks), dim3(256), 0, c->stream, pd, nd, b, p, m, jcap, nslots,
                       ng, ts, scan_blocks, c->filter_waves, c->filter_slots_cap);
}
void launch_scan_filter(bs_ctx* c, uint32_t scan_blocks, uint32_t filter_blocks, const PodsDev& pd, const NodesDev& nd, const BatchDev& b,
                        const BatchParams& p, uint32_t m, uint32_t jcap, uint32_t nslots, uint32_t ng, uint32_t ts, bool local) {
  lanes_wide(c->S, [&](auto s) { launch_scan_filter_s<decltype(s)::value>(c, scan_blocks, filter_blocks, pd, nd, b, p, m, jcap, nslots, ng, ts, local); });
}

void launch_tables_nofix(bs_ctx* c, dim3 grid, const NodesDev& nd, const BatchDev& b, const BatchParams& p, uint32_t nchunks) {
  lanes_narrow(c->S, [&](auto s) {
    hipLaunchKernelGGL(HIP_KERNEL_NAME(k_tables_local_nofix<decltype(s)::value>), grid, dim3(kTblChunk), 0, c->stream, nd, b, p, nchunks, cdiv(c->Ncap, 256),
                       cdiv(c->Ncap, 64));
  });
}

static FastLaunch fast_launch(const bs_ctx* c) {
  FastLaunch f{c->stream, c->S, c->M, c->P, c->filter_waves, c->filter_slots_cap, c->tp_filter, c->cfg.device};
  const uint32_t mul = c->tp_split ? c->tp_split : ((!c->reduce_external && c->nranks > 1u) ? 2u : 1u);
  if (mul > 1u) f.filter_split = (uint32_t)std::min<uint64_t>((uint64_t)c->filter_waves * mul, 1u << 22);
  return f;
}
static int fused_residency(bs_ctx* c) {
  if (c->fused_blocks_resident < 0) c->fused_blocks_resident = fused_residency_query(fast_launch(c));
// ... 9 lines not shown

uint32_t pick_scan_share(const bs_ctx* c) { return c->scan_share_override ? c->scan_share_override : 8u; }

int build_scratch_table(bs_ctx* c, uint32_t cls, float pct, uint32_t* slot_out) {
  if (!c->have_nodes || !c->have_fit) { c->last_error = "nodes / fit not loaded"; return BS_ERR_STATE; }
  if (cls >= c->C) { c->last_error = "class out of range"; return BS_ERR_INVALID; }
  const uint32_t slot = c->table_slots - 1;
  BatchDev b = batch_dev(c);
  BatchParams p = batch_params(c);
  TableDesc d{cls, pct};
  HIPCHK(c, hipMemcpyAsync(b.desc + slot, &d, sizeof(d), hipMemcpyHostToDevice, c->stream));
  const uint32_t nchunks = std::max<uint32_t>(1, cdiv(c->M, 256));
  BatchDev b2 = b;
  b2.tables = b.tables + (size_t)slot * p.mcap * p.LP;
  b2.kp = b.kp + (size_t)slot * 16;
  b2.desc = b.desc + slot;
  b2.chunk_tot = b.chunk_tot + (size_t)slot * cdiv(c->Ncap, 256) * 16;
  b2.gmax = b.gmax + (size_t)slot * cdiv(c->Ncap, 64) * p.LP;
  b2.chunk_kp = b.chunk_kp + (size_t)slot * cdiv(c->Ncap, 256) * 16;
  const TableDesc* forced = b.desc + slot;
  launch_tables_local(c, c->stream, dim3(1, nchunks), nodes_dev(c), b2, p, forced);
  if (nchunks > 1) hipLaunchKernelGGL(k_tables_fix, dim3(1, nchunks - 1), dim3(kTblChunk), 0, c->stream, nodes_dev(c), b2, p, forced);
  HIPCHK(c, hipGetLastError());
  *slot_out = slot;
  return BS_OK;
}

int flush_groups(bs_ctx* c) {
  if (!c->groups_launch_pending) return BS_OK;
  c->groups_launch_pending = false;
  GroupsDev gr = groups_dev(c);
  BatchDev b = batch_dev(c);
  hipLaunchKernelGGL(k_leader_info, dim3(1), dim3(kLeaderBlock), 0, c->stream, gr, b, (c->have_fit && c->have_nodes) ? c->C : 0u, c->info_tag, c->h_info.p,
                     c->pending_dp, const_cast<uint32_t*>(gr.matched), const_cast<uint32_t*>(gr.status_scheduled), const_cast<uint8_t*>(gr.flags));
  LAUNCHCHK(c, BS_KERNEL_LEADER);
  return BS_OK;
}

int wait_host_tag(bs_ctx* c, int tag_at, int32_t tag, const int32_t* base = nullptr) {
  volatile const int32_t* info = base ? base : c->h_info.p;
  for (uint32_t spin = 0; info[tag_at] != tag; ++spin) {
    if (spin == 2000) (void)hipStreamQuery(c->stream);
    if (spin > 20000000u) { HIPCHK(c, hipStreamSynchronize(c->stream)); if (info[tag_at] != tag) { c->last_error = "host info tag never arrived"; return BS_ERR_HIP; } }
  }
  __atomic_thread_fence(__ATOMIC_ACQUIRE);
  return BS_OK;
}

int resolve_groups(bs_ctx* c) {
  if (!c->info_pending) return BS_OK;
  int rc = wait_host_tag(c, 3, c->info_tag);
  if (rc) return rc;
  c->info_pending = false;
  c->steady_table = (c->n_uncaptured == 0 && c->h_info.p[2] >= 0) ? c->h_info.p[2] : -1;
  c->steady_prev = c->steady_table;
  return BS_OK;
}

int resolve_pods(bs_ctx* c) {
  if (!c->kinfo_pending) return BS_OK;
  int rc = wait_host_tag(c, 5, c->kinfo_tag);
  if (rc) return rc;
  c->kinfo_pending = false;
  c->h_K = (uint32_t)c->h_info.p[4];
  c->k_bound = c->h_K;
  return BS_OK;
}

int derive_pods(bs_ctx* c, bool pairs_only) {
  const uint32_t G = c->G, P = c->P, L = c->L;
  HIPCHK(c, c->d_gstat.reserve((size_t)5 * std::max<uint32_t>(G, 1) * 4 + 16));
  HIPCHK(c, c->d_fast_reject.reserve((size_t)std::max<uint32_t>(G, 1) * 4));
  HIPCHK(c, c->d_gcount.reserve((size_t)std::max<uint32_t>(G, 1) * 4));
  HIPCHK(c, c->d_admit64.reserve((size_t)std::max<uint32_t>(G, 1) * 8));
  uint32_t* gcount = c->d_gcount.as<uint32_t>();
  const uint32_t gcn = c->have_groups ? G : 0u;
  c->gstat_cur = 0;
  unsigned long long* ctab = c->d_cls_slots.as<unsigned long long>();
  unsigned long long* ptab = ctab + c->cls_cap;
  uint32_t* kcount = c->d_nepochs.as<uint32_t>() + 2;
  const uint32_t ngstat = c->have_groups ? 5 * G + 1 : 0u;
  if (P) {
    if (pairs_only) {
      hipLaunchKernelGGL(k_pods_prep, dim3(64), dim3(256), 0, c->stream, ptab, c->cls_cap, c->d_gstat.as<uint32_t>(), ngstat, (uint32_t*)nullptr, gcount, gcn);
    } else {
      hipLaunchKernelGGL(k_pods_prep, dim3(64), dim3(256), 0, c->stream, ctab, 2 * c->cls_cap, c->d_gstat.as<uint32_t>(), ngstat, kcount, gcount, gcn);
      hipLaunchKernelGGL(k_pod_class_a, dim3(cdiv(P, 256)), dim3(256), 0, c->stream, pods_dev(c), ctab, c->cls_cap - 1, c->hash_keep, L,
                         c->d_cls_rep.as<uint32_t>(), c->d_blk_scratch.as<uint32_t>());
      hipLaunchKernelGGL(k_pod_class_ids, dim3(cdiv(P, 256)), dim3(256), 0, c->stream, P, c->d_cls_rep.as<uint32_t>(), c->d_blk_scratch.as<uint32_t>(),
                         c->d_cls_id.as<uint32_t>(), kcount);
    }
    LAUNCHCHK(c, BS_KERNEL_PREPASS);
  } else {
    if (!pairs_only) HIPCHK(c, hipMemsetAsync(kcount, 0, 4, c->stream));
    if (gcn) HIPCHK(c, hipMemsetAsync(gcount, 0, (size_t)gcn * 4, c->stream));
  }
  c->kinfo_tag++;
  hipLaunchKernelGGL(k_pod_pairs, dim3(std::max<uint32_t>(1, cdiv(P, 256))), dim3(256), 0, c->stream, pods_dev(c), G, c->d_cls_rep.as<uint32_t>(),
                     c->d_cls_id.as<uint32_t>(), pclass_dev(c), ptab, c->cls_cap - 1, c->hash_keep, c->d_gstat.as<uint32_t>(),
                     ppair_dev(c), c->d_pair_next.as<unsigned long long>(), kcount, c->kinfo_tag, c->h_info.p, gcount);
  LAUNCHCHK(c, BS_KERNEL_PREPASS);
  c->kinfo_pending = true;
  c->k_bound = P;
  c->pairs_ready = c->have_groups;
  c->owner_ready = false;
  c->epochs_ready = false;
// ... 101 lines not shown

}

extern "C" { static int fd_settle(bs_ctx* c); }
namespace bs {
const char* const kKernelNames[BS_KERNEL_COUNT] = {"prepass", "leader", "query", "tables", "scan", "resolve", "filter", "tally"};

int use_device(bs_ctx* c, bool flush) {
  HIPCHK(c, hipSetDevice(c->cfg.device));
  if (flush && c->groups_launch_pending) return flush_groups(c);
  return BS_OK;
}

NodesDev nodes_dev(const bs_ctx* c) {
  NodesDev nd{};
  nd.n = c->N;
  nd.stride = c->Ncap;
  nd.alloc = c->d_alloc.as<int64_t>();
  nd.req = c->d_nreq.as<int64_t>();
  nd.apres = c->d_apres.as<uint32_t>();
  nd.rpres = c->d_rpres.as<uint32_t>();
  nd.flags = c->d_nflags.as<uint8_t>();
  nd.fit = c->d_fit.as<uint32_t>();
  nd.fit_words = c->fit_words;
  nd.n_classes = c->C;
  nd.kmap = c->d_kmap.as<uint32_t>();
  nd.m = c->M;
  nd.left4 = c->d_left4.as<int64_t>();
  nd.lglob = c->d_lglob.as<int64_t>();
  return nd;
}
GroupsDev groups_dev(const bs_ctx* c) {
  GroupsDev g{};
  g.g = c->G;
  void* pk = c->d_gpack.p;
  g.min_member = c->off_gmm.in(pk);
  g.status_scheduled = c->off_gsc.in(pk);
  g.matched = c->off_gmatched.in(pk);
  g.flags = c->off_gflags.in(pk);
  g.cls = c->off_gcls.in(pk);
  g.minres = c->off_gminres.in(pk);
  g.mrpres = c->off_gmrpres.in(pk);
  g.occupied = c->off_gocc.in(pk);
  return g;
}
PodsDev pods_dev(const bs_ctx* c) {
  PodsDev p{};
  p.p = c->P;
  pod_cols(p, c->lay[c->cur_pack], c->d_pack[c->cur_pack].p);
  return p;
}
uint32_t* pclass_dev(const bs_ctx* c) { return c->lay[c->cur_pack].pclass.in(c->d_pack[c->cur_pack].p); }

void rederive_nodes(bs_ctx* c, uint32_t base0, uint32_t m_before) {
  hipLaunchKernelGGL(k_nodes_derive, dim3(1), dim3(kScanBlock), 0, c->stream, nodes_dev(c), c->d_kmap.as<uint32_t>(), c->d_m.as<uint32_t>(), c->d_left4.as<int64_t>(),
                     c->d_lglob.as<int64_t>(), base0, m_before);
}

int analyse_groups(bs_ctx* c, bool rearm_scratch, const bs_group_delta* deltas, uint32_t ndeltas, bool defer) {
  if (c->groups_launch_pending) { int rc = flush_groups(c); if (rc) return rc; }
  c->steady_table = -1;
  c->side_ready = false;
  c->info_pending = false;
  if (!c->G) { c->scratch_armed = false; return BS_OK; }
  GroupsDev gr = groups_dev(c);
  BatchDev b = batch_dev(c);
  if (rearm_scratch) {
    hipLaunchKernelGGL(k_init, dim3(cdiv(std::max<uint32_t>(c->G, 8), 256)), dim3(256), 0, c->stream, gr, b);
    c->scratch_armed = true;
  }
  DeltaPack dp;
  dp.n = ndeltas;
  static_assert(sizeof(bs_group_delta) == sizeof(GroupDelta), "delta layout");
  if (ndeltas) std::memcpy(dp.d, deltas, (size_t)ndeltas * sizeof(GroupDelta));
  c->info_tag++;
  c->info_pending = true;
  c->epochs_ready = false;
  if (defer) {
    c->pending_dp = dp;
    c->groups_launch_pending = true;
    return BS_OK;
  }
  hipLaunchKernelGGL(k_leader_info, dim3(1), dim3(kLeaderBlock), 0, c->stream, gr, b, (c->have_fit && c->have_nodes) ? c->C : 0u, c->info_tag, c->h_info.p,
                     dp, const_cast<uint32_t*>(gr.matched), const_cast<uint32_t*>(gr.status_scheduled), const_cast<uint8_t*>(gr.flags));
  LAUNCHCHK(c, BS_KERNEL_LEADER);
  return BS_OK;
}

int maybe_analyse_epochs(bs_ctx* c) {
  if (c->epochs_ready || c->no_fast || c->no_epoch) return BS_OK;
  if (!c->have_groups || !c->have_pods || !c->have_fit || !c->have_nodes || !c->pairs_ready || !c->P || !c->G) return BS_OK;
  if (c->n_uncaptured == 0 && c->n_nominres == 0) return BS_OK;
  if (c->groups_launch_pending) { int rc = flush_groups(c); if (rc) return rc; }
  return analyse_epochs(c);
}

void launch_nodes_assume(bs_ctx* c, const bs_node_request* records, uint32_t n) {
  static_assert(sizeof(bs_node_request) == sizeof(NodeRequest), "node request layout");
  hipLaunchKernelGGL(k_nodes_assume, dim3(cdiv(n, 256)), dim3(256), 0, c->stream, reinterpret_cast<const NodeRequest*>(records), n, c->L, c->Ncap,
                     c->d_alloc.as<int64_t>(), c->d_nreq.as<int64_t>(), c->d_rpres.as<uint32_t>(), c->d_nflags.as<uint8_t>(), c->d_left4.as<int64_t>(),
                     c->d_lglob.as<int64_t>());
}
void mirror_node_requests(bs_ctx* c, const bs_node_request* records, uint32_t n) {
  for (uint32_t i = 0; i < n; ++i) {
    const bs_node_request& r = records[i];
    for (uint32_t j = 0; j < c->L; ++j) c->h_nreq[(size_t)j * c->N + r.index] = r.requested[j];
    c->h_rpres[r.index] = r.requested_present;
  }
}

int settle_pending(bs_ctx* c) { return (c->fd_active || c->spec_active) ? fd_settle(c) : BS_OK; }

int check_handover(bs_ctx* c) {
  if (c->h_info.p && ((volatile int32_t*)c->h_info.p)[13]) {
    ((volatile int32_t*)c->h_info.p)[13] = 0;
    c->pairs_ready = false;
    c->dirs_ready = false;
    c->rep_valid = false;
    c->ids_used = c->pair_cap;
    const int rc2 = derive_pods(c, false);
    c->n_rederives++;
    c->batch_void = true;
    c->last_error = "bs_pods_apply: class / pair id space overflowed on the device; the queue was re-derived, run the batch again";
    return rc2 ? rc2 : BS_ERR_RETRY;
  }
  if (c->h_info.p && ((volatile int32_t*)c->h_info.p)[12]) {
    ((volatile int32_t*)c->h_info.p)[12] = 0;
    c->no_fuse_final = 1;
    c->batch_void = true;
    c->last_error = "in-launch hand-over timed out (producer blocks not resident): batch void, run it again (the context now uses separate launches)";
    return BS_ERR_RETRY;
  }
  if (c->batch_void) {
    c->last_error = "the last batch's results are void (hand-over time-out or queue re-derivation, reported earlier): run the batch again";
    return BS_ERR_RETRY;
  }
  return BS_OK;
}

}

extern "C" {

uint32_t bs_abi_version(void) { return BS_ABI_VERSION; }

const char* bs_strerror(int status) {
  switch (status) {
    case BS_OK: return "ok";
    case BS_ERR_INVALID: return "invalid argument";
    case BS_ERR_NO_DEVICE: return "no usable gfx950 device";
    case BS_ERR_HIP: return "HIP runtime error";
    case BS_ERR_STATE: return "call order: snapshot / groups / pods not loaded";
    case BS_ERR_CAPACITY: return "capacity exceeded";
    case BS_ERR_NOMEM: return "out of memory";
    case BS_ERR_COMM: return "RCCL error";
    case BS_ERR_RETRY: return "the last batch's results are void and the cause is repaired: run the batch again";
    default: return "unknown status";
  }
}

const char* bs_last_error(const bs_ctx* ctx) { return ctx ? ctx->last_error.c_str() : ""; }
const char* bs_kernel_name(uint32_t id) { return id < BS_KERNEL_COUNT ? kKernelNames[id] : "?"; }

static void read_env_switches(bs_ctx* c) {
  if (const char* e = std::getenv("BS_STAMP_START")) c->stamp_ctr = (uint32_t)(std::strtoul(e, nullptr, 0) % 65535u);
  if (const char* e = std::getenv("BS_KEYSEQ_START")) { c->key_seq = (uint32_t)std::strtoul(e, nullptr, 0); if (c->key_seq == 0u || c->key_seq == 0xFFFFFFFFu) c->key_seq = 1; }
  if (const char* e = std::getenv("BS_NO_FAST")) c->no_fast = std::atoi(e) ? 1u : 0u;
  if (const char* e = std::getenv("BS_NO_EPOCH")) c->no_epoch = std::atoi(e) ? 1u : 0u;
  if (const char* e = std::getenv("BS_NO_FUSE_FILTER")) c->no_fuse_filter = std::atoi(e) ? 1u : 0u;
  if (const char* e = std::getenv("BS_NO_FUSE_FINAL")) c->no_fuse_final = std::atoi(e) ? 1u : 0u;
  if (const char* e = std::getenv("BS_TP_FILTER")) c->tp_filter = (uint32_t)std::min(8, std::max(0, std::atoi(e)));
  if (const char* e = std::getenv("BS_TEST_HANDOVER_TIMEOUT")) c->test_timeout_after = (uint32_t)std::atoi(e);
  if (const char* e = std::getenv("BS_TEST_PC_CHUNK_NODES")) c->test_pc_chunk_nodes = (uint32_t)std::max(0, std::atoi(e));
  if (const char* e = std::getenv("BS_STEP_A")) { c->step_a_on = std::atoi(e) != 0; c->step_a_form = (uint32_t)std::atoi(e); }
  if (const char* e = std::getenv("BS_POD_RANGES")) c->pod_ranges_on = std::atoi(e) != 0;
  if (const char* e = std::getenv("BS_STEP_SHARES")) c->step_shares = (uint32_t)std::min(32, std::max(1, std::atoi(e)));
  if (const char* e = std::getenv("BS_TP_SHARE")) c->tp_share = (uint32_t)std::min(64, std::max(1, std::atoi(e)));
  if (const char* e = std::getenv("BS_TP_FWAVES")) c->tp_fwaves = (uint32_t)std::max(1, std::atoi(e));
  if (const char* e = std::getenv("BS_TP_SPLIT")) c->tp_split = (uint32_t)std::max(1, std::atoi(e));
  if (const char* e = std::getenv("BS_NO_NODEW")) c->no_nodew = std::atoi(e) != 0;
  if (const char* e = std::getenv("BS_TP_TMIN")) c->tp_tmin = (uint32_t)std::max(1, std::atoi(e));
  if (const char* e = std::getenv("BS_NO_SPECULATE")) c->no_spec = std::atoi(e) ? 1u : 0u;
  if (const char* e = std::getenv("BS_HOST_PROBE")) c->host_probe = std::atoi(e) ? 1u : 0u;
  if (const char* e = std::getenv("BS_HASH_SLOT_BITS")) { const int hb = std::atoi(e); c->slot_keep = hb >= 32 ? 0xFFFFFFFFu : ((1u << std::max(0, hb)) - 1u); }
  if (const char* e = std::getenv("BS_HASH_BITS")) { const int hb = std::atoi(e); c->hash_keep = hb >= 31 ? 0x7FFFFFFFu : ((1u << std::max(0, hb)) - 1u); }
  if (const char* e = std::getenv("BS_EARLY_FILTER_MIN")) { c->early_filter_min = std::strtoull(e, nullptr, 10); c->early_forced = 1; }
  if (const char* e = std::getenv("BS_SCAN_SHARE")) c->scan_share_override = (uint32_t)std::max(0, std::atoi(e));
  if (const char* e = std::getenv("BS_TARGET_WAVES")) { c->target_waves = std::max(1, std::atoi(e)); c->general_waves = c->target_waves; }
  if (const char* e = std::getenv("BS_FILTER_WAVES")) { c->filter_waves = std::max(1, std::atoi(e)); c->filter_waves_env = true; }
  if (const char* e = std::getenv("BS_SERIAL_INSERT_MAX")) c->serial_insert_max = (uint32_t)std::max(0, std::atoi(e));
  if (const char* e = std::getenv("BS_ID_ROOM")) c->id_room = (uint32_t)std::max(1, std::atoi(e));
}

int bs_create(const bs_config* cfg, bs_ctx** out) {
  if (!cfg || !out) return BS_ERR_INVALID;
  *out = nullptr;
  if (cfg->abi_version != BS_ABI_VERSION || cfg->scalar_lanes > BS_MAX_SCALARS) return BS_ERR_INVALID;
  int ndev = 0;
  if (hipGetDeviceCount(&ndev) != hipSuccess || ndev <= 0 || cfg->device < 0 || cfg->device >= ndev) return BS_ERR_NO_DEVICE;
  hipDeviceProp_t prop;
  if (hipGetDeviceProperties(&prop, cfg->device) != hipSuccess) return BS_ERR_NO_DEVICE;
  if (std::strncmp(prop.gcnArchName, "gfx950", 6) != 0) return BS_ERR_NO_DEVICE;
  bs_ctx* c = new (std::nothrow) bs_ctx();
  if (!c) return BS_ERR_NOMEM;
  c->cfg = *cfg;
  c->S = cfg->scalar_lanes;
  c->L = BS_FIXED_LANES + c->S;
  c->LP = c->S == 0 ? 4 : (c->S <= 4 ? 8 : 16);
  if (hipSetDevice(cfg->device) != hipSuccess || hipStreamCreateWithFlags(&c->stream.h, hipStreamNonBlocking) != hipSuccess ||
      hipStreamCreateWithFlags(&c->stream3.h, hipStreamNonBlocking) != hipSuccess ||
      hipEventCreateWithFlags(&c->ev_query.h, hipEventDisableTiming) != hipSuccess ||
      hipEventCreateWithFlags(&c->ev_filter.h, hipEventDisableTiming) != hipSuccess) {
    delete c;
    return BS_ERR_NO_DEVICE;
  }
  if (c->d_nepochs.reserve(64) != hipSuccess || hipMemset(c->d_nepochs.p, 0, 64) != hipSuccess || c->d_ticket.reserve(kTkWords * 4) != hipSuccess ||
      hipMemset(c->d_ticket.p, 0, kTkWords * 4) != hipSuccess) {
    delete c;
    return BS_ERR_NOMEM;
  }
  if (c->d_info.reserve(64) != hipSuccess || c->d_first_reach.reserve(64) != hipSuccess || hipMemset(c->d_first_reach.p, 0xFF, 64) != hipSuccess ||
      c->h_info.reserve(64) != hipSuccess) {
    delete c;
    return BS_ERR_NOMEM;
  }
  std::memset(c->h_info.p, 0, 64);
  c->batch_seq = 1;
  read_env_switches(c);
  *out = c;
  return BS_OK;
}

int bs_destroy(bs_ctx* c) {
  if (!c) return BS_OK;
  if (c->host_probe && c->hp_n)
// ... 99 lines not shown
    o[1] = A.put(r.op, r.count);
    o[2] = A.put(r.count ? r.val_off : zero_off, (size_t)(r.count + 1) * 4);
    o[3] = A.put(r.val, (size_t)nv * 4);
    o[4] = A.put(r.val_int, (size_t)nv * 8);
    o[5] = A.put(r.val_int_ok, nv);
  };
  size_t o_ex[6], o_fl[6];
  put_req(tp->exprs, ex_col.data(), o_ex);
  put_req(tp->fields, tp->fields.key, o_fl);
  const size_t o_ooff = A.put(tp->tol_off, (size_t)(C + 1) * 4);
  const size_t o_okey = A.put(tp->tol_key, (size_t)ntol * 4), o_oval = A.put(tp->tol_val, (size_t)ntol * 4);
  const size_t o_oop = A.put(tp->tol_op, ntol), o_oeff = A.put(tp->tol_effect, ntol);

  HIPCHK(c, c->d_fitarena.reserve(A.bytes.size() + 16));
  HIPCHK(c, hipMemcpyAsync(c->d_fitarena.p, A.bytes.data(), A.bytes.size(), hipMemcpyHostToDevice, c->stream));
  const size_t colcells = (size_t)std::max<uint32_t>(K, 1) * Npad;
  const size_t o_cval = 0, o_cival = (colcells * 4 + 15) & ~(size_t)15, o_cflag = o_cival + colcells * 8;
  HIPCHK(c, c->d_fitcols.reserve(o_cflag + colcells));
  HIPCHK(c, hipMemsetAsync(c->d_fitcols.p, 0, o_cflag + colcells, c->stream));

  const void* B = c->d_fitarena.p;
  FitNodesDev nd{};
  nd.n = N;
  nd.name = at_dev<uint32_t>(B, o_name);
  nd.label_off = at_dev<uint32_t>(B, o_loff); nd.label_key = at_dev<uint32_t>(B, o_lkey); nd.label_val = at_dev<uint32_t>(B, o_lval);
  nd.label_int = at_dev<int64_t>(B, o_lint); nd.label_int_ok = at_dev<uint8_t>(B, o_lok);
  nd.taint_off = at_dev<uint32_t>(B, o_toff); nd.taint_key = at_dev<uint32_t>(B, o_tkey); nd.taint_val = at_dev<uint32_t>(B, o_tval);
  nd.taint_effect = at_dev<uint8_t>(B, o_teff);
  nd.nflags = c->d_nflags.as<uint8_t>();
  FitCols cols{};
  cols.K = K; cols.Npad = Npad;
  cols.keys = at_dev<uint32_t>(B, o_keys);
  cols.val = (uint32_t*)((uint8_t*)c->d_fitcols.p + o_cval);
  cols.ival = (int64_t*)((uint8_t*)c->d_fitcols.p + o_cival);
  cols.flag = (uint8_t*)c->d_fitcols.p + o_cflag;
  FitTplDev td{};
  td.c = C; td.field_name_key = tp->field_name_key;
  td.flags = at_dev<uint8_t>(B, o_flags);
  td.sel_off = at_dev<uint32_t>(B, o_soff); td.sel_col = at_dev<uint32_t>(B, o_scol); td.sel_val = at_dev<uint32_t>(B, o_sval);
  td.term_off = at_dev<uint32_t>(B, o_moff); td.term_expr_off = at_dev<uint32_t>(B, o_meo); td.term_field_off = at_dev<uint32_t>(B, o_mfo);
  auto req_dev = [&](const size_t (&o)[6]) {
    FitReqDev r{};
    r.key = at_dev<uint32_t>(B, o[0]); r.op = at_dev<uint8_t>(B, o[1]); r.val_off = at_dev<uint32_t>(B, o[2]);
    r.val = at_dev<uint32_t>(B, o[3]); r.val_int = at_dev<int64_t>(B, o[4]); r.val_int_ok = at_dev<uint8_t>(B, o[5]);
    return r;
  };
  td.ex = req_dev(o_ex); td.fl = req_dev(o_fl);
  td.tol_off = at_dev<uint32_t>(B, o_ooff); td.tol_key = at_dev<uint32_t>(B, o_okey); td.tol_val = at_dev<uint32_t>(B, o_oval);
  td.tol_op = at_dev<uint8_t>(B, o_oop); td.tol_effect = at_dev<uint8_t>(B, o_oeff);

  c->C = C;
  c->fit_words = cdiv(N, 32);
  c->h_fit.assign((size_t)C * c->fit_words, 0);
  HIPCHK(c, c->d_fit.reserve(std::max<size_t>(4, c->h_fit.size() * 4)));
  if (N) {
    const uint32_t nb = cdiv(N, 256);
    hipLaunchKernelGGL(k_fit_cols, dim3(nb), dim3(256), 0, c->stream, nd, cols);
    hipLaunchKernelGGL(k_fit_match, dim3(nb, std::min<uint32_t>(C, 1024)), dim3(256), 0, c->stream, nd, td, cols, c->d_fit.as<uint32_t>(), c->fit_words);
    HIPCHK(c, hipGetLastError());
    HIPCHK(c, hipMemcpyAsync(c->h_fit.data(), c->d_fit.p, c->h_fit.size() * 4, hipMemcpyDeviceToHost, c->stream));
  }
  HIPCHK(c, hipStreamSynchronize(c->stream));
  c->have_fit = true;
  rc = ensure_tables(c);
  if (rc == BS_OK && c->have_groups) rc = analyse_groups(c);
  return rc;
}

int bs_fit_read(bs_ctx* c, uint32_t* out) {
  if (!c || !out) return BS_ERR_INVALID;
  if (!c->have_fit) { c->last_error = "bs_fit_read before a fit load / build"; return BS_ERR_STATE; }
  int rc = use_device(c);
  if (rc) return rc;
  const size_t bytes = (size_t)c->C * c->fit_words * 4;
  if (bytes) HIPCHK(c, hipMemcpyAsync(out, c->d_fit.p, bytes, hipMemcpyDeviceToHost, c->stream));
  HIPCHK(c, hipStreamSynchronize(c->stream));
  return BS_OK;
}

int bs_groups_load(bs_ctx* c, const bs_groups_soa* g) {
  if (!c || !g) return BS_ERR_INVALID;
  c->seq_wait_valid = false;
  int rc = use_device(c);
  if (rc) return rc;
  if ((rc = settle_pending(c))) return rc;
  c->steady_prev = -1;
  c->first_reach_hint = 0xFFFFFFFFu;
  const uint32_t G = g->g, L = c->L;
  if (G && (!g->min_member || !g->status_scheduled || !g->matched || !g->flags || !g->cls || !g->min_resources || !g->min_resources_present ||
            !g->occupied_by))
    return BS_ERR_INVALID;
  const size_t n = std::max<uint32_t>(G, 1);
  Carve cv;
  c->off_gmm = cv.take<uint32_t>(n);
  c->off_gsc = cv.take<uint32_t>(n);
  c->off_gmatched = cv.take<uint32_t>(n);
  c->off_gflags = cv.take<uint8_t>(n);
  c->off_gcls = cv.take<uint32_t>(n);
  c->off_gminres = cv.take<int64_t>(n * L);
  c->off_gmrpres = cv.take<uint32_t>(n);
  c->off_gocc = cv.take<uint64_t>(n);
  c->gpack_bytes = cv.mark();
  HIPCHK(c, c->d_gpack.reserve(c->gpack_bytes));
  HIPCHK(c, c->d_first_elig.reserve(n * 4));
  HIPCHK(c, c->d_first_owner.reserve(n * 4));
  HIPCHK(c, c->d_first_reject.reserve(n * 4));
// ... 631 lines not shown
  const uint32_t P = c->P, G = c->G, N = c->N;
  const uint32_t W = cdiv(N, 64);
  const bool run_filter = stages & BS_STAGE_FILTER;
  const bool commit = stages & BS_BATCH_COMMIT;
  NodesDev nd = nodes_dev(c);
  GroupsDev gr = groups_dev(c);
  PodsDev pd = pods_dev(c);
  BatchDev b = batch_dev(c);
  BatchParams prm = batch_params(c);
  prm.run_filter = run_filter;
  prm.use_classes = 1;
  prm.fuse_filter = run_filter ? 1u : 0u;
  prm.scan_slots_cap = c->scan_slots_cap;
  prm.filter_slots_cap = c->filter_slots_cap;
  prm.stamp = 1u + c->stamp_ctr;
  prm.seq_inv = ~c->key_seq;
  prm.commit = commit ? 1u : 0u;
  prm.do_tally = (stages & BS_STAGE_TALLY) ? 1u : 0u;
  prm.do_ready = (prm.do_tally && c->nranks == 1 && !c->reduce_external) ? 1u : 0u;
  if ((rc = setup_host_out(c, stages, run_filter, b, prm))) return rc;
  const uint32_t side_slot = (uint32_t)c->steady_table;
  const uint32_t nchunks = std::max<uint32_t>(1, cdiv(c->M, 256));
  BatchDev bt = b;
  bt.tables = b.tables + (size_t)side_slot * prm.mcap * prm.LP;
  bt.kp = b.kp + (size_t)side_slot * 16;
  bt.chunk_tot = b.chunk_tot + (size_t)side_slot * cdiv(c->Ncap, 256) * 16;
  bt.chunk_kp = b.chunk_kp + (size_t)side_slot * cdiv(c->Ncap, 256) * 16;
  bt.gmax = b.gmax + (size_t)side_slot * cdiv(c->Ncap, 64) * prm.LP;
  const TableDesc* forced = b.desc + side_slot;
  if (commit && G) HIPCHK(c, hipMemsetAsync(c->d_fast_reject.p, 0xFF, (size_t)G * 4, c->stream));

  if (c->kinfo_pending && ((volatile int32_t*)c->h_info.p)[5] == c->kinfo_tag && (rc = resolve_pods(c))) return rc;
  prm.k_host = c->kinfo_pending ? 0u : c->h_K;
  const uint64_t hp1 = c->host_probe ? host_ns() : 0;
  const bool k_known = !c->kinfo_pending;
  const uint32_t k_step = k_known ? prm.k_host : ((c->step_a_form >= 3u && c->dirs_ready) ? c->k_bound : 0u);
  if (step_a_possible(c, stages, k_step, nchunks) && (c->step_a_form == 1u || c->dirs_ready || (c->batch_since_pods && c->pairs_ready && c->rep_valid && c->have_groups))) {
    const uint32_t K = k_step;
    const uint32_t nshares = std::max<uint32_t>(1, std::min<uint32_t>(c->step_shares, cdiv(K, 8)));
    const uint32_t fblocks = run_filter ? cdiv(std::min<uint32_t>(c->filter_waves, cdiv(2 * K, 64) * std::max<uint32_t>(1, cdiv(W, 2))), 4) : 0u;
    uint32_t pb = 0;
    if (c->step_a_form >= 2u) {
      if (!c->dirs_ready && c->batch_since_pods && c->pairs_ready && c->rep_valid && c->have_groups && (rc = build_dirs(c))) return rc;
      if (c->dirs_ready) pb = cdiv(K, kTblChunk);
    }
    const uint32_t nch_nodes = std::max<uint32_t>(1, cdiv(N, 256));
    const uint32_t whole = (c->step_a_form >= 3u && pb && nch_nodes <= 64 && c->d_first_row64.p && c->d_scan_rec.p && c->d_feas_rec.p && c->d_chunk_rec.p) ? 1u : 0u;
    const uint32_t nchunks_s = whole ? nch_nodes : nchunks;
    const bool ranges = whole && c->ranges_valid && c->nranges && c->d_pod_ranges.p;
    const uint32_t qb = ranges ? c->nranges : cdiv(P, kTblChunk);
    if (ranges) b.pod_ranges = c->d_pod_ranges.as<uint32_t>();
    const uint32_t grid = qb + pb + nchunks_s * nshares + fblocks;
    if ((k_known || whole) && (int)grid <= step_a_residency(c, whole != 0)) {
      TIMED(c, BS_KERNEL_QUERY, {
        launch_fast_step_a(fast_launch(c), dim3(grid), pd, gr, nd, b, bt, prm, forced, nchunks_s, qb, nshares, fblocks, c->tk_pods, c->tk_tab, pb,
                           c->d_ckeys.as<int64_t>(), c->d_cpres.as<uint32_t>(), c->pair_cap, whole, c->tk_p1, c->tk_done, side_slot - c->C);
      });
      c->tk_pods += pb ? pb : qb;
      if (!whole) c->tk_tab += nchunks_s;
      if (whole) {
        c->tk_p1 += qb;
        if (qb > kGatherDirectBlocks) c->tk_done += nchunks_s * nshares + fblocks;
      } else {
        TIMED(c, BS_KERNEL_RESOLVE, hipLaunchKernelGGL(k_fast_final, dim3(cdiv(P, 256)), dim3(256), 0, c->stream, pd, gr, nd, b, prm, cdiv(P, kTblChunk)));
      }
      c->launches = whole ? 1 : 2;
      c->last_step_a = true;
      if (c->test_timeout_after && --c->test_timeout_after == 0 && c->h_info.p) {
        HIPCHK(c, hipStreamSynchronize(c->stream));
        ((volatile int32_t*)c->h_info.p)[12] = 1;
      }
      if (prm.filter_deny && (rc = launch_filter_deny(c, pd, gr, nd, b, prm, true))) return rc;
      if (commit) {
        if (prm.filter_deny && (rc = launch_filter_deny_marks(c, b, prm, b.fast_reject))) return rc;
        if (G) hipLaunchKernelGGL(k_fast_commit, dim3(cdiv(G, 256)), dim3(256), 0, c->stream, pd, b, const_cast<uint8_t*>(gr.flags),
                                  const_cast<uint64_t*>(gr.occupied), G, prm.filter_deny ? b.fd_flag : nullptr);
        LAUNCHCHK(c, BS_KERNEL_RESOLVE);
        int32_t last = -1;
        HIPCHK(c, hipMemcpyAsync(&last, b.pf_leader + (P - 1), 4, hipMemcpyDeviceToHost, c->stream));
        if (G) HIPCHK(c, hipMemcpyAsync(c->h_gflags.data(), gr.flags, G, hipMemcpyDeviceToHost, c->stream));
        HIPCHK(c, hipStreamSynchronize(c->stream));
        if (!fd_commit_gated(c) && !handover_commit_gated(c)) c->sop_leader0 = last;
        c->launches++;
      }
      return batch_collective(c, stages, gr, b);
    }
  }
  c->last_step_a = false;
  const uint32_t k_est = std::min<uint32_t>(P, c->kinfo_pending ? std::max<uint32_t>(2 * c->h_K, 1024) : std::max<uint32_t>(c->h_K, 1));
  const bool node_words = run_filter && cdiv(k_est, 64) > 16 && c->tp_filter >= 5u && !c->no_nodew && c->d_nodew.p;
  if (node_words) {
    b.nodew = bt.nodew = c->d_nodew.as<uint64_t>();
    b.nodew_stride = bt.nodew_stride = nodew_stride(N);
    b.tiles2_min = bt.tiles2_min = c->tp_tmin * std::max<uint32_t>(1u, c->nranks);
  }
  TIMED(c, BS_KERNEL_QUERY, {
    const uint32_t qb = cdiv(P, kTblChunk);
    const dim3 qg(qb + nchunks + (node_words ? nodew_blocks(N) : 0u)), blk(kTblChunk);
    lanes_narrow(c->S, [&](auto s) {
      hipLaunchKernelGGL(HIP_KERNEL_NAME(k_fast_query_tables<decltype(s)::value>), qg, blk, 0, c->stream, pd, gr, nd, b, bt, prm, forced, nchunks, qb);
    });
  });
  const uint64_t hp2 = c->host_probe ? host_ns() : 0;
  bool fused = false, tp_split = false;
  uint64_t hp3 = 0;
  TIMED(c, BS_KERNEL_SCAN, {
    const uint32_t nseg = pick_scan_share(c);
    const uint32_t tiles = cdiv(k_est, 64);
    const bool throughput = tiles > 16;
    const uint32_t share_b = c->tp_share ? c->tp_share : (throughput ? 2u : 64u);
    struct FwGuard { bs_ctx* c; uint32_t saved; ~FwGuard() { c->filter_waves = saved; } } fw_guard{c, c->filter_waves};
    if (throughput && c->tp_filter >= 5u && !c->filter_waves_env)
      c->filter_waves = c->tp_fwaves ? c->tp_fwaves
                                     : ((uint64_t)cdiv(2 * k_est, 64) * std::max<uint32_t>(1, cdiv(W, 2)) >= 65536u ? std::max<uint32_t>(c->filter_waves, 16384u) : c->filter_waves);
    const uint32_t fblocks = run_filter ? cdiv(std::min<uint32_t>(c->filter_waves, cdiv(2 * k_est, 64) * std::max<uint32_t>(1, cdiv(W, 2))), 4) : 0u;
    auto scan_grid = [&](uint32_t nsub) {
      const uint32_t items = tiles * std::min<uint32_t>(nsub == 4u ? nseg : share_b, cdiv(c->M, 64));
      return std::max<uint32_t>(1, std::min<uint32_t>(cdiv(c->target_waves, 4), nsub == 4u ? items : cdiv(items, 4)));
    };
    fused = tiles <= 16 && !c->no_fuse_final && (int)(scan_grid(4u) + fblocks + cdiv(P, 256)) <= fused_residency(c);
    prm.scan_nsub = fused ? 4u : 1u;
    const uint32_t scan_blocks = scan_grid(prm.scan_nsub);
    hp3 = c->host_probe ? host_ns() : 0;
    if (fused) {
      const dim3 grid(scan_blocks + fblocks + cdiv(P, 256));
      launch_fast_bc(fast_launch(c), grid, pd, gr, nd, b, bt, prm, nseg, scan_blocks, fblocks);
    } else if (c->tp_filter == 8u && fblocks && throughput) {
      FastLaunch side = fast_launch(c);
      side.stream = c->stream3;
      HIPCHK(c, hipEventRecord(c->ev_query, c->stream));
      HIPCHK(c, hipStreamWaitEvent(c->stream3, c->ev_query, 0));
      launch_fast_scan(side, dim3(scan_blocks), bt, prm, share_b);
      HIPCHK(c, hipEventRecord(c->ev_filter, c->stream3));
      launch_fast_filter(fast_launch(c), dim3(fblocks), pd, nd, bt, prm);
      HIPCHK(c, hipStreamWaitEvent(c->stream, c->ev_filter, 0));
      tp_split = true;
    } else if (c->tp_filter >= 6u && fblocks && throughput && c->S <= 4u) {
      launch_fast_bt(fast_launch(c), dim3(scan_blocks + fblocks), nd, bt, prm, share_b, scan_blocks);
    } else if (c->tp_filter && fblocks && throughput) {
      launch_fast_scan(fast_launch(c), dim3(scan_blocks), bt, prm, share_b);
      launch_fast_filter(fast_launch(c), dim3(fblocks), pd, nd, bt, prm);
// ... 133 lines not shown
static int batch_run_inner(bs_ctx* c, uint32_t stages) {
  int rc = BS_OK;
  if (c->host_probe) c->hp_t0 = host_ns();
  c->fd_on = (stages & BS_BATCH_FILTER_DENY) != 0;
  if (c->fd_on) {
    const size_t g1 = std::max<uint32_t>(c->G, 1);
    if ((rc = reserve_filled(c, c->d_fd_event, g1 * 8, 0xFF)) || (rc = reserve_filled(c, c->d_fd_in, g1 * 4, 0xFF)) || (rc = reserve_filled(c, c->d_fd_flag, 16, 0))) return rc;
    HIPCHK(c, hipMemsetAsync(c->d_fd_flag.p, 0, 4, c->stream));
    ((volatile int32_t*)c->h_info.p)[14] = 0;
    ((volatile int32_t*)c->h_info.p)[15] = 0;
  }
  const uint32_t P = c->P, G = c->G, N = c->N, C = c->C;
  if ((G > c->n_uncaptured && c->max_group_cls >= C) || (P && c->max_pod_cls >= C)) {
    c->last_error = "fit class index out of range (groups.cls / pods.cls vs the loaded fit classes)";
    return BS_ERR_INVALID;
  }
  c->spec_active = false;
  if (c->info_pending && ((volatile int32_t*)c->h_info.p)[3] != c->info_tag && !c->no_spec && c->steady_prev >= 0 && (uint32_t)c->steady_prev < 2 * c->C && c->n_uncaptured == 0 &&
      c->n_nominres == 0 && !(stages & BS_BATCH_COMMIT) && c->cfg.enable_timing < 2 && !c->collect_stats && c->nranks == 1 && !c->reduce_external &&
      c->fd_iter == 0 && !c->groups_launch_pending && !c->ext_admit) {
    c->steady_table = c->steady_prev;
    c->spec_active = true;
    c->spec_table = c->steady_prev;
    c->spec_stages = stages;
    c->n_spec++;
  } else if ((rc = resolve_groups(c))) {
    return rc;
  }
  if (!c->pairs_ready && (rc = build_pairs(c))) return rc;
  if (c->nranks > 1 && !c->owner_ready && P) {
    HIPCHK(c, c->d_own_start.reserve((size_t)P * 4));
    hipLaunchKernelGGL(k_owner_starts, dim3(1), dim3(kScanBlock), 0, c->stream, pods_dev(c), G, gstat_dev(c), c->d_gcount.as<uint32_t>(),
                       c->d_own_start.as<uint32_t>());
    LAUNCHCHK(c, BS_KERNEL_PREPASS);
    c->owner_ready = true;
  }
  const uint32_t W = cdiv(N, 64);
  const bool run_filter = stages & BS_STAGE_FILTER;
  if ((rc = reserve_slots(c, run_filter))) return rc;
  const uint32_t scan_cap = c->scan_slots_cap, filter_cap = c->filter_slots_cap;
  (void)W;
  if (c->stamp_ctr == 0) {
    if (c->d_qstamp_s.p) HIPCHK(c, hipMemsetAsync(c->d_qstamp_s.p, 0, c->d_qstamp_s.cap, c->stream));
    if (c->d_uflags.p) HIPCHK(c, hipMemsetAsync(c->d_uflags.p, 0, c->d_uflags.cap, c->stream));
    if (c->d_uclaim.p) HIPCHK(c, hipMemsetAsync(c->d_uclaim.p, 0, c->d_uclaim.cap, c->stream));
  }
  if (c->rekey_pending) {
    if (c->d_pair_firstq.p) HIPCHK(c, hipMemsetAsync(c->d_pair_firstq.p, 0xFF, c->d_pair_firstq.cap, c->stream));
    if (c->d_first_reach.p) HIPCHK(c, hipMemsetAsync(c->d_first_reach.p, 0xFF, c->d_first_reach.cap, c->stream));
    if (c->d_first_row64.p) HIPCHK(c, hipMemsetAsync(c->d_first_row64.p, 0xFF, c->d_first_row64.cap, c->stream));
    if (c->d_scan_rec.p) HIPCHK(c, hipMemsetAsync(c->d_scan_rec.p, 0, c->d_scan_rec.cap, c->stream));
    if (c->d_feas_rec.p) HIPCHK(c, hipMemsetAsync(c->d_feas_rec.p, 0, c->d_feas_rec.cap, c->stream));
    if (c->d_chunk_rec.p) HIPCHK(c, hipMemsetAsync(c->d_chunk_rec.p, 0, c->d_chunk_rec.cap, c->stream));
    if (c->d_gfirstq.p) HIPCHK(c, hipMemsetAsync(c->d_gfirstq.p, 0xFF, c->d_gfirstq.cap, c->stream));
    if (c->d_fd_event.p) HIPCHK(c, hipMemsetAsync(c->d_fd_event.p, 0xFF, c->d_fd_event.cap, c->stream));
    c->rekey_pending = false;
  }

  const bool captures_possible = c->n_uncaptured > 0 && P > 0;
  const bool use_classes = !captures_possible && c->n_nominres == 0;
  c->last_use_classes = use_classes;
  c->last_stages = stages;
  c->bitmap_valid = false;
  c->batch_since_pods = true;
  const bool inline_tables = !captures_possible && c->steady_table >= 0 && c->M && P && c->cfg.enable_timing < 2;
  const bool early_filter = run_filter && !captures_possible && P && N && !(stages & BS_BATCH_COMMIT) && c->cfg.enable_timing < 2 &&
                            (uint64_t)P * N >= c->early_filter_min && (!use_classes || c->early_forced);
  c->last_fast = use_classes && inline_tables && !early_filter && N && !c->no_fast && !c->no_fuse_filter;
  c->last_chain = c->last_fast ? 1u : 0u;
  if (c->last_fast) {
    if (c->host_probe) c->hp_t1 = host_ns();
    rc = run_fast(c, stages);
    advance_batch_seq(c);
    return rc;
  }
  if (!c->no_fast && !c->no_epoch && !c->no_fuse_filter && P && G && N && c->M && !early_filter && c->cfg.enable_timing < 2) {
    bool taken = false;
    rc = run_epoch(c, stages, &taken);
    if (rc) return rc;
    if (taken) {
      c->last_chain = 2;
      advance_batch_seq(c);
      return BS_OK;
    }
  }
  c->epochs_ready = false;

  c->last_host_out = false;
  NodesDev nd = nodes_dev(c);
  GroupsDev gr = groups_dev(c);
  PodsDev pd = pods_dev(c);
  BatchDev b = batch_dev(c);
  BatchParams prm = batch_params(c);
  prm.run_filter = run_filter;
  const uint32_t tiles_est = cdiv(std::max<uint32_t>(P, 1), 64);
  const uint32_t nseg = c->scan_share_override ? c->scan_share_override : 2u;
  const dim3 blk(256);
  prm.use_classes = use_classes ? 1u : 0u;
  prm.scan_slots_cap = scan_cap;
  prm.filter_slots_cap = filter_cap;
  bool commit_dirty = false;
  const uint32_t side_slot = inline_tables ? (uint32_t)c->steady_table : 0u;
  prm.early_filter = early_filter ? 1u : 0u;
  const bool local_ready = c->nranks == 1 && !c->reduce_external;
  const bool rearm = !(stages & BS_BATCH_COMMIT);
  const bool fuse_filter = run_filter && use_classes && !early_filter && P && N && !c->no_fuse_filter;
  prm.fuse_filter = fuse_filter ? 1u : 0u;
  const uint32_t nchunks = std::max<uint32_t>(1, cdiv(c->M, 256));
  uint32_t launches = 0;
  BatchDev bt = b;
  const TableDesc* forced = nullptr;
  if (inline_tables) {
    bt.tables = b.tables + (size_t)side_slot * prm.mcap * prm.LP;
    bt.kp = b.kp + (size_t)side_slot * 16;
    bt.chunk_tot = b.chunk_tot + (size_t)side_slot * cdiv(c->Ncap, 256) * 16;
    bt.gmax = b.gmax + (size_t)side_slot * cdiv(c->Ncap, 64) * prm.LP;
    bt.chunk_kp = b.chunk_kp + (size_t)side_slot * cdiv(c->Ncap, 256) * 16;
    forced = b.desc + side_slot;
  }

  TIMED(c, BS_KERNEL_PREPASS, {
    if (!c->scratch_armed) { hipLaunchKernelGGL(k_init, dim3(cdiv(std::max<uint32_t>(G, 4), 256)), blk, 0, c->stream, gr, b); launches++; }
    const uint32_t span = std::max(std::max(P, G), (2 * C + 1) * 16);
    const uint32_t fused = captures_possible ? 0u : 1u;
    launches++;
    if (inline_tables) {
      const uint32_t pre = cdiv(span, kPrepassBlock);
      const dim3 pg(pre + 1 + nchunks), pb(kPrepassBlock);
// ... 73 lines not shown
      launches++;
    }
  } else if (early_filter) {
    HIPCHK(c, hipStreamWaitEvent(c->stream, c->ev_filter, 0));
    hipLaunchKernelGGL(k_void_rows, dim3(cdiv(P, 256)), blk, 0, c->stream, pd, b);
    LAUNCHCHK(c, BS_KERNEL_FILTER);
    launches++;
  } else if (P) {
    HIPCHK(c, hipMemsetAsync(b.fl_code, BS_FL_NOT_RUN, P, c->stream));
  }
  if (prm.filter_deny && P) {
    c->launches = launches;
    if ((rc = launch_filter_deny(c, pd, gr, nd, b, prm, false))) return rc;
    launches = c->launches;
  }
  const bool do_tally = stages & BS_STAGE_TALLY;
  if (P ? (run_filter || do_tally) : do_tally) {
    TIMED(c, BS_KERNEL_TALLY, {
      hipLaunchKernelGGL(k_tally, dim3(std::max<uint32_t>(1, cdiv(P, kTallyBlock))), dim3(kTallyBlock), 0, c->stream, pd, gr, nd, b,
                         run_filter ? 1u : 0u, do_tally ? 1u : 0u, (do_tally && local_ready) ? 1u : 0u, (do_tally && rearm) ? 1u : 0u);
    });
    launches++;
  }
  if (stages & BS_BATCH_COMMIT) {
    if (prm.filter_deny && P) {
      c->launches = launches;
      if ((rc = launch_filter_deny_marks(c, b, prm, b.first_reject))) return rc;
      launches = c->launches;
    }
    if (G) hipLaunchKernelGGL(k_commit, dim3(cdiv(G, 256)), blk, 0, c->stream, pd, b, prm, const_cast<uint8_t*>(gr.flags), const_cast<uint32_t*>(gr.cls),
                              const_cast<int64_t*>(gr.minres), const_cast<uint32_t*>(gr.mrpres), const_cast<uint64_t*>(gr.occupied), G,
                              (prm.filter_deny && P) ? b.fd_flag : nullptr);
    LAUNCHCHK(c, BS_KERNEL_RESOLVE);
    launches++;
    if ((rc = commit_readback(c, gr, b))) return rc;
    commit_dirty = true;
  }
  c->launches = launches;
  advance_batch_seq(c);
  if (do_tally) {
    c->scratch_armed = rearm;
    c->side_ready = rearm && inline_tables;
  }
  rc = batch_collective(c, stages, gr, b);
  if (rc) return rc;
  if (commit_dirty) return analyse_groups(c);
  return BS_OK;
}

static void discard_handover(bs_ctx* c) {
  if (c->h_info.p && ((volatile int32_t*)c->h_info.p)[12]) {
    ((volatile int32_t*)c->h_info.p)[12] = 0;
    c->no_fuse_final = 1;
  }
}

static int fd_resolve(bs_ctx* c) {
  if (!c->fd_active) return BS_OK;
  c->fd_active = false;
  c->fd_unsynced = false;
  volatile int32_t* hf = c->h_info.p + 14;
  if (!hf[0]) return BS_OK;
  int rc = BS_OK;
  bool settled = false;
  const uint32_t stages = c->fd_stages;
  for (uint32_t iter = 1; iter <= c->P + 2 && !settled; ++iter) {
    BatchDev b = batch_dev(c);
    b.fd_in = c->d_fd_in.as<uint32_t>();
    BatchParams prm = batch_params(c);
    prm.seq_inv = c->fd_seq_inv;
    hipLaunchKernelGGL(k_fd_next, dim3(cdiv(std::max<uint32_t>(c->G, 1), 256)), dim3(256), 0, c->stream, b, prm, c->G);
    LAUNCHCHK(c, BS_KERNEL_RESOLVE);
    c->fd_in_live = true;
    c->fd_iter = iter;
    c->epochs_ready = false;
    discard_handover(c);
    rc = batch_run_inner(c, stages);
    if (rc == BS_OK) rc = hipStreamSynchronize(c->stream) == hipSuccess ? BS_OK : BS_ERR_HIP;
    c->n_fd_reruns++;
    if (rc) break;
    settled = !hf[1];
  }
  c->fd_in_live = false;
  c->fd_iter = 0;
  c->fd_on = false;
  c->epochs_ready = false;
  if (rc) return rc;
  if (!settled) { c->last_error = "BS_BATCH_FILTER_DENY: the fixed-point iteration did not settle"; return BS_ERR_STATE; }
  return BS_OK;
}

static int fd_settle(bs_ctx* c) {
  if (!c->fd_active && !c->spec_active) return BS_OK;
  if (!c->batch_since_pods) { c->fd_active = false; c->spec_active = false; return BS_OK; }
  int rc;
  if (c->last_host_out) {
    if ((rc = wait_host_tag(c, 0, c->host_tag, reinterpret_cast<const int32_t*>(c->h_hout.p + c->off_htag)))) return rc;
  } else {
    HIPCHK(c, hipStreamSynchronize(c->stream));
  }
  if (c->spec_active) {
    c->spec_active = false;
    if ((rc = resolve_groups(c))) return rc;
    if (c->steady_table != c->spec_table) {
      c->n_spec_miss++;
      const bool fd = c->fd_active;
// ... 637 lines not shown
  std::memcpy(u.internal, id, 128);
  auto init = (decltype(&ncclCommInitRank))dlsym(h, "ncclCommInitRank");
  c->rccl_allreduce = (decltype(&ncclAllReduce))dlsym(h, "ncclAllReduce");
  c->rccl_destroy = (decltype(&ncclCommDestroy))dlsym(h, "ncclCommDestroy");
  ncclComm_t comm = nullptr;
  if (!init || !c->rccl_allreduce || !c->rccl_destroy) { c->last_error = "librccl lacks ncclCommInitRank / ncclAllReduce / ncclCommDestroy"; return BS_ERR_COMM; }
  const ncclResult_t r = init(&comm, (int)nranks, u, (int)rank);
  if (r != ncclSuccess) { c->last_error = std::string("ncclCommInitRank failed: code ") + std::to_string((int)r); return BS_ERR_COMM; }
  c->rccl_handle = h;
  c->comm = comm;
  c->rank = rank;
  c->nranks = nranks;
  return BS_OK;
}

#ifdef BS_PROBE
int bs_probe_read(bs_ctx* c, unsigned long long* out) {
  if (!c || !out) return BS_ERR_INVALID;
  int rc = use_device(c);
  if (rc) return rc;
  HIPCHK(c, hipStreamSynchronize(c->stream));
  HIPCHK(c, hipMemcpyFromSymbol(out, HIP_SYMBOL(g_probe), sizeof(g_probe)));
  static std::vector<unsigned long long> zero(sizeof(g_probe) / 8, 0ull);
  HIPCHK(c, hipMemcpyToSymbol(HIP_SYMBOL(g_probe), zero.data(), sizeof(g_probe)));
  return BS_OK;
}
#endif

int bs_timing_reset(bs_ctx* c) {
  if (!c) return BS_ERR_INVALID;
  int rc = use_device(c);
  if (rc) return rc;
  rc = timer_collect(c);
  std::memset(&c->timing, 0, sizeof(c->timing));
  return rc;
}

int bs_timing_get(bs_ctx* c, bs_timing* out) {
  if (!c || !out) return BS_ERR_INVALID;
  int rc = use_device(c);
  if (rc) return rc;
  rc = timer_collect(c);
  *out = c->timing;
  return rc;
}

int bs_speculation_stats(const bs_ctx* c, uint64_t* launched, uint64_t* missed) {
  if (!c || !launched || !missed) return BS_ERR_INVALID;
  *launched = c->n_spec;
  *missed = c->n_spec_miss;
  return BS_OK;
}

int bs_filter_deny_stats(const bs_ctx* c, uint64_t* reruns) {
  if (!c || !reruns) return BS_ERR_INVALID;
  *reruns = c->n_fd_reruns;
  return BS_OK;
}

int bs_batch_stats_get(bs_ctx* c, bs_batch_stats* out) {
  if (!c || !out) return BS_ERR_INVALID;
  int rc = use_device(c);
  if (rc) return rc;
  std::memset(out, 0, sizeof(*out));
  if (!c->collect_stats) {
    c->collect_stats = 1;
    return BS_OK;
  }
  HIPCHK(c, hipStreamSynchronize(c->stream));
  uint64_t raw[8] = {0};
  uint32_t nt = 0, nq = 0;
  if (c->d_stats.p) HIPCHK(c, hipMemcpy(raw, c->d_stats.p, sizeof(raw), hipMemcpyDeviceToHost));
  if (c->d_qcount.p) HIPCHK(c, hipMemcpy(&nq, c->d_qcount.p, 4, hipMemcpyDeviceToHost));
  if (c->d_needed.p && c->C) {
    std::vector<uint32_t> need(2 * c->C);
    HIPCHK(c, hipMemcpy(need.data(), c->d_needed.p, need.size() * 4, hipMemcpyDeviceToHost));
    for (uint32_t x : need) nt += x ? 1u : 0u;
  }
  out->scan_rows_executed = raw[0];
  out->scan_evals_executed = raw[1];
  out->scan_queries = raw[4];
  out->scan_queries_logical = raw[2];
  out->filter_lane_blocks = raw[5];
  out->filter_tile_blocks = raw[6];
  out->class_mode = c->last_use_classes ? 1 : 0;
  out->fast_path = c->last_fast ? 1 : 0;
  out->chain = c->last_chain;
  out->launches = c->launches;
  out->tables_built = c->last_fast ? 1 : nt;
  out->logical_evals = (uint64_t)c->P * c->N;
  out->filter_evals = (c->last_stages & BS_STAGE_FILTER) ? (uint64_t)c->P * c->N : 0;
  if (c->last_stages & BS_STAGE_FILTER) {
    out->filter_distinct = raw[3];
    out->filter_evals_executed = raw[3] * c->N;
  }
  c->collect_stats = 0;
  return BS_OK;
}

}
```

### batch-scheduler_amd/csrc/tu_fast.hip

```cpp
#ifndef BS_UNITY
#define BS_TU_FAST
#endif
#include "bs_fast.hpp"
#include "bs_launch.hpp"

#include <algorithm>

namespace bs {

void launch_fast_b(const FastLaunch& c, dim3 grid, const PodsDev& pd, const NodesDev& nd, const BatchDev& bt, const BatchParams& prm, uint32_t nseg,
                          uint32_t scan_blocks) {
  lanes_wide(c.S, [&](auto s) {
    hipLaunchKernelGGL(HIP_KERNEL_NAME(k_fast_scan_filter<decltype(s)::value>), grid, dim3(256), 0, c.stream, pd, nd, bt, prm, c.M, nseg, scan_blocks,
                       c.filter_waves, c.filter_slots_cap);
  });
}
void launch_fast_scan(const FastLaunch& c, dim3 grid, const BatchDev& bt, const BatchParams& prm, uint32_t nseg) {
  lanes_wide(c.S, [&](auto s) { hipLaunchKernelGGL(HIP_KERNEL_NAME(k_fast_scan<decltype(s)::value>), grid, dim3(256), 0, c.stream, bt, prm, c.M, nseg); });
}
void launch_fast_bt(const FastLaunch& c, dim3 grid, const NodesDev& nd, const BatchDev& bt, const BatchParams& prm, uint32_t nseg, uint32_t scan_blocks) {
  lanes_clamped(c.S, [&](auto s) {
    hipLaunchKernelGGL(HIP_KERNEL_NAME(k_fast_scan_filter_t<decltype(s)::value>), grid, dim3(256), 0, c.stream, nd, bt, prm, c.M, nseg, scan_blocks,
                       c.filter_split ? c.filter_split : c.filter_waves, c.filter_slots_cap, (c.tp_filter == 7u ? 1u : 0u) | (c.filter_split ? 2u : 0u));
  });
}
void launch_fast_filter(const FastLaunch& c, dim3 grid, const PodsDev& pd, const NodesDev& nd, const BatchDev& bt, const BatchParams& prm) {
  switch (c.tp_filter) {
    case 1: hipLaunchKernelGGL(HIP_KERNEL_NAME(k_fast_filter<4, true>), grid, dim3(256), 0, c.stream, pd, nd, bt, prm, c.filter_waves, c.filter_slots_cap); break;
    case 2: hipLaunchKernelGGL(HIP_KERNEL_NAME(k_fast_filter<2, true>), grid, dim3(256), 0, c.stream, pd, nd, bt, prm, c.filter_waves, c.filter_slots_cap); break;
    case 3: hipLaunchKernelGGL(HIP_KERNEL_NAME(k_fast_filter<2, false>), grid, dim3(256), 0, c.stream, pd, nd, bt, prm, c.filter_waves, c.filter_slots_cap); break;
    case 4: hipLaunchKernelGGL(k_fast_filter_w7, grid, dim3(256), 0, c.stream, pd, nd, bt, prm, c.filter_waves, c.filter_slots_cap); break;
    default: hipLaunchKernelGGL(k_fast_filter_t, grid, dim3(256), 0, c.stream, nd, bt, prm, c.filter_split ? c.filter_split : c.filter_waves, c.filter_slots_cap, c.filter_split ? 1u : 0u); break;
  }
}
template <class K>
static int blocks_resident(const FastLaunch& c, K kernel, int block) {
  int per_cu = 0;
  if (hipOccupancyMaxActiveBlocksPerMultiprocessor(&per_cu, kernel, block, 0) != hipSuccess || per_cu <= 0) return 0;
  hipDeviceProp_t prop;
  if (hipGetDeviceProperties(&prop, c.device) != hipSuccess) return 0;
  return std::max(0, per_cu - 1) * prop.multiProcessorCount;
}
int fused_residency_query(const FastLaunch& c) {
  return lanes_wide(c.S, [&](auto s) { return blocks_resident(c, k_fast_scan_filter_final<decltype(s)::value>, 256); });
}
void launch_fast_bc(const FastLaunch& c, dim3 grid, const PodsDev& pd, const GroupsDev& gr, const NodesDev& nd, const BatchDev& b, const BatchDev& bt,
                           const BatchParams& prm, uint32_t nseg, uint32_t scan_blocks, uint32_t filter_blocks) {
  lanes_wide(c.S, [&](auto s) {
    hipLaunchKernelGGL(HIP_KERNEL_NAME(k_fast_scan_filter_final<decltype(s)::value>), grid, dim3(256), 0, c.stream, pd, gr, nd, b, bt, prm, c.M, nseg,
                       scan_blocks, filter_blocks, c.filter_waves, c.filter_slots_cap, cdiv(c.P, kTblChunk));
  });
}

void launch_fast_step_a(const FastLaunch& c, dim3 grid, const PodsDev& pd, const GroupsDev& gr, const NodesDev& nd, const BatchDev& b, const BatchDev& bt,
                        const BatchParams& prm, const TableDesc* forced, uint32_t nchunks, uint32_t query_blocks, uint32_t nshares, uint32_t filter_blocks,
                        uint32_t tk_pods0, uint32_t tk_tab0, uint32_t param_blocks, const int64_t* ckeys, const uint32_t* cpres, uint32_t kcap,
                        uint32_t whole, uint32_t tk_p1, uint32_t tk_done, uint32_t forced_cls) {
  lanes_clamped(c.S, [&](auto s) {
    auto launch = [&](auto whole_step) {
      hipLaunchKernelGGL(HIP_KERNEL_NAME(k_fast_step_a<decltype(s)::value, decltype(whole_step)::value>), grid, dim3(kTblChunk), 0, c.stream, pd, gr, nd, b, bt,
                         prm, forced, nchunks, query_blocks, nshares, filter_blocks, c.filter_waves, c.filter_slots_cap, tk_pods0, tk_tab0, param_blocks,
                         ckeys, cpres, kcap, tk_p1, tk_done, forced_cls);
    };
    if (whole) launch(std::true_type{});
    else launch(std::false_type{});
  });
}
int step_a_residency_query(const FastLaunch& c, bool whole) {
  return lanes_clamped(c.S, [&](auto s) {
    constexpr int TS = decltype(s)::value;
    return whole ? blocks_resident(c, k_fast_step_a<TS, true>, (int)kTblChunk) : blocks_resident(c, k_fast_step_a<TS, false>, (int)kTblChunk);
  });
}

}
```

### include/bsched.h

```cpp
#ifndef BSCHED_H
#define BSCHED_H

#include <stddef.h>
#include <stdint.h>

#ifdef __cplusplus
extern "C" {
#endif

#define BS_ABI_VERSION 7u

enum {
  BS_LANE_CPU = 0,
  BS_LANE_MEM = 1,
  BS_LANE_EPH = 2,
  BS_LANE_PODS = 3,
  BS_FIXED_LANES = 4,
  BS_MAX_SCALARS = 12,
  BS_MAX_LANES = 16
};

typedef enum bs_status {
  BS_OK = 0,
  BS_ERR_INVALID = -1,
// ... 435 lines not shown
                       const int64_t* req, const uint32_t* req_present);
int bs_preempt_run_flat(bs_ctx* ctx, uint32_t stages, uint32_t count, const uint32_t* pod_index, const int32_t* priority, const uint8_t* group_protected,
                        uint32_t victim_cap, int32_t* node, uint32_t* n_candidates, uint32_t* n_victims, uint32_t* victims, int32_t* top_priority,
                        int64_t* priority_sum, int64_t* earliest_start);
int bs_bound_apply_flat(bs_ctx* ctx, uint32_t n_remove, const uint32_t* remove, uint32_t n_insert, const uint32_t* node, const int32_t* priority,
                        const int64_t* start_ns, const int32_t* group, const int64_t* req, const uint32_t* req_present,
                        const uint8_t* pdb_violating, uint32_t* first_id_out);
int bs_bound_apply_ex_flat(bs_ctx* ctx, uint32_t flags, uint32_t n_remove, const uint32_t* remove, uint32_t n_insert, const uint32_t* node,
                           const int32_t* priority, const int64_t* start_ns, const int32_t* group, const int64_t* req,
                           const uint32_t* req_present, const uint8_t* pdb_violating, uint32_t* first_id_out);
int bs_preempt_commit_flat(bs_ctx* ctx, uint32_t stages, uint32_t count, const uint32_t* pod_index, const int32_t* priority,
                           const uint8_t* group_protected, uint32_t flags, uint32_t victim_cap, int32_t* node, uint32_t* n_candidates,
                           uint32_t* n_victims, uint32_t* victims, int32_t* top_priority, int64_t* priority_sum, int64_t* earliest_start);
int bs_seq_expire_flat(bs_ctx* ctx, uint32_t count, const uint32_t* group, uint32_t flags, uint32_t group_cap, uint32_t* group_out,
                       uint32_t* group_pods, uint32_t* group_earlier, uint32_t pod_cap, uint32_t* pod, uint32_t* node, uint32_t* counts_out );
int bs_preempt_commit_gang_flat(bs_ctx* ctx, uint32_t stages, uint32_t count, const uint32_t* pod_index, const int32_t* priority,
                                const uint8_t* group_protected, const uint32_t* gang_need, uint32_t flags, uint32_t victim_cap,
                                int32_t* node, uint32_t* n_candidates, uint32_t* n_victims, uint32_t* victims, int32_t* top_priority,
                                int64_t* priority_sum, int64_t* earliest_start);

#define BS_KERNEL_PREPASS   0u
#define BS_KERNEL_LEADER    1u
#define BS_KERNEL_QUERY     2u
#define BS_KERNEL_TABLES    3u
#define BS_KERNEL_SCAN      4u
#define BS_KERNEL_RESOLVE   5u
#define BS_KERNEL_FILTER    6u
#define BS_KERNEL_TALLY     7u
#define BS_KERNEL_COUNT     8u
typedef struct bs_timing {
  double   total_ms[BS_KERNEL_COUNT];
  uint64_t launches[BS_KERNEL_COUNT];
} bs_timing;
int bs_timing_reset(bs_ctx* ctx);
int bs_timing_get(bs_ctx* ctx, bs_timing* out);
const char* bs_kernel_name(uint32_t kernel_id);
typedef struct bs_batch_stats {
  uint64_t scan_queries, scan_rows_executed, scan_evals_executed, tables_built, logical_evals;
  uint64_t filter_evals;
  uint64_t filter_distinct;
  uint64_t filter_evals_executed;
  uint64_t scan_queries_logical;
  uint64_t class_mode;
  uint64_t fast_path;
  uint64_t launches;
  uint64_t chain;
  uint64_t filter_lane_blocks;
  uint64_t filter_tile_blocks;
} bs_batch_stats;
int bs_batch_stats_get(bs_ctx* ctx, bs_batch_stats* out);
int bs_pods_apply_stats(const bs_ctx* ctx, uint64_t* applies, uint64_t* rederives);
int bs_filter_deny_stats(const bs_ctx* ctx, uint64_t* reruns);
int bs_speculation_stats(const bs_ctx* ctx, uint64_t* launched, uint64_t* missed);

#ifdef __cplusplus
}
#endif
#endif
```

Measured before the change: 3742 billion evals/s.

## Reuse per-chunk node totals across whole-step launches and pass leader as argument

```diff
diff --git a/batch-scheduler_amd/build.py b/batch-scheduler_amd/build.py
--- a/batch-scheduler_amd/build.py
+++ b/batch-scheduler_amd/build.py
@@ -10,7 +10,7 @@
 PREBUILT_ONLY = bool(os.environ.get("BS_LIB_DIR"))
 LIB_PATH = os.path.join(LIB_DIR, "libbsched.so")
 _COMMON = ["bs_common.hpp", "bs_kernels.hpp", "bs_nodew_layout.hpp", "bs_lanes.hpp", os.path.join("..", "..", "include", "bsched.h")]
-_CTX = _COMMON + ["bs_ctx.hpp", "bs_carve.hpp", "bs_hostmem.hpp", "bs_pod_ranges.hpp"]
+_CTX = _COMMON + ["bs_ctx.hpp", "bs_carve.hpp", "bs_hostmem.hpp", "bs_pod_ranges.hpp", "bs_totals_key.hpp"]
 _FAST = ["bs_launch.hpp", "bs_fast.hpp", "bs_filter_t.hpp"]
 _SEQ = _CTX + ["bs_seq.hpp"]
 UNITS = {
diff --git a/batch-scheduler_amd/capi.py b/batch-scheduler_amd/capi.py
--- a/batch-scheduler_amd/capi.py
+++ b/batch-scheduler_amd/capi.py
@@ -17,6 +17,7 @@
     "bs_abi_version", "bs_strerror", "bs_last_error", "bs_create", "bs_destroy",
     "bs_nodes_load", "bs_fit_load", "bs_fit_build", "bs_fit_read", "bs_groups_load", "bs_groups_read", "bs_groups_apply", "bs_pods_map", "bs_pods_load",
     "bs_pods_apply", "bs_pods_count", "bs_pods_read", "bs_pods_apply_stats", "bs_filter_deny_stats", "bs_speculation_stats",
+    "bs_step_leader_stats", "bs_step_totals_stats",
     "bs_nodes_apply", "bs_nodes_count", "bs_nodes_assume",
     "bs_cluster_fits", "bs_node_left", "bs_scan_prefix", "bs_cluster_total", "bs_filter_one", "bs_find_max_pg",
     "bs_batch_run", "bs_batch_sync", "bs_batch_read", "bs_batch_map", "bs_filter_rows_count", "bs_queue_order_load", "bs_queue_sort",
@@ -158,6 +159,8 @@
     L.bs_pods_apply_stats.argtypes = [vp, P(C.c_uint64), P(C.c_uint64)]
     L.bs_filter_deny_stats.argtypes = [vp, P(C.c_uint64)]
     L.bs_speculation_stats.argtypes = [vp, P(C.c_uint64), P(C.c_uint64)]
+    L.bs_step_leader_stats.argtypes = [vp, P(C.c_uint64), P(C.c_uint64)]
+    L.bs_step_totals_stats.argtypes = [vp, P(C.c_uint64), P(C.c_uint64)]
     L.bs_pods_read.argtypes = [vp, P(soa.PodsOutStruct)]
     L.bs_queue_order_load.argtypes = [vp, u32, P(u32)]
     L.bs_queue_sort.argtypes = [vp, u32, P(i32), P(i32), P(C.c_int64), P(u32)]
@@ -397,6 +400,16 @@
         self._chk(self._lib.bs_speculation_stats(self._h, C.byref(a), C.byref(m)), "bs_speculation_stats")
         return int(a.value), int(m.value)
 
+    def step_leader_stats(self) -> tuple[int, int]:
+        a, d = C.c_uint64(0), C.c_uint64(0)
+        self._chk(self._lib.bs_step_leader_stats(self._h, C.byref(a), C.byref(d)), "bs_step_leader_stats")
+        return int(a.value), int(d.value)
+
+    def step_totals_stats(self) -> tuple[int, int]:
+        a, d = C.c_uint64(0), C.c_uint64(0)
+        self._chk(self._lib.bs_step_totals_stats(self._h, C.byref(a), C.byref(d)), "bs_step_totals_stats")
+        return int(a.value), int(d.value)
+
     def filter_deny_reruns(self) -> int:
         r = C.c_uint64(0)
         self._chk(self._lib.bs_filter_deny_stats(self._h, C.byref(r)), "bs_filter_deny_stats")
diff --git a/batch-scheduler_amd/csrc/bs_ctx.hpp b/batch-scheduler_amd/csrc/bs_ctx.hpp
--- a/batch-scheduler_amd/csrc/bs_ctx.hpp
+++ b/batch-scheduler_amd/csrc/bs_ctx.hpp
@@ -10,6 +10,7 @@
 #include "bs_kernels.hpp"
 #include "bs_lanes.hpp"
 #include "bs_pod_ranges.hpp"
+#include "bs_totals_key.hpp"
 
 namespace bs {
 
@@ -59,6 +60,7 @@
 int analyse_groups(bs_ctx* c, bool rearm_scratch = true, const bs_group_delta* deltas = nullptr, uint32_t ndeltas = 0, bool defer = false);
 int maybe_analyse_epochs(bs_ctx* c);
 int check_handover(bs_ctx* c);
+void nodes_touched(bs_ctx* c);
 
 }
 
@@ -99,6 +101,13 @@
   size_t gpack_bytes = 0;
   int32_t info_tag = 0, kinfo_tag = 0;
   bool info_pending = false, kinfo_pending = false;
+  bool leader_known = false;
+  int32_t h_leader = -1, h_panic = 0;
+  TotalsCache totals;
+  uint32_t totals_on = 1;
+  uint64_t n_totals_rebuilt = 0, n_totals_reused = 0;
+  uint32_t no_leader_arg = 0;
+  uint64_t n_leader_arg = 0, n_leader_dev = 0;
   uint32_t max_group_cls = 0, max_pod_cls = 0;
   uint32_t h_K = 0;
   uint32_t k_bound = 0;
diff --git a/batch-scheduler_amd/csrc/bs_fast.hpp b/batch-scheduler_amd/csrc/bs_fast.hpp
--- a/batch-scheduler_amd/csrc/bs_fast.hpp
+++ b/batch-scheduler_amd/csrc/bs_fast.hpp
@@ -1,4 +1,6 @@
 #pragma once
+
+#include <type_traits>
 
 #include "bs_kernels.hpp"
 #include "bs_filter_t.hpp"
@@ -267,6 +269,11 @@
 __device__ __forceinline__ unsigned long long ld_agent64(const void* p) {
   return __hip_atomic_load(reinterpret_cast<const unsigned long long*>(p), __ATOMIC_RELAXED, __HIP_MEMORY_SCOPE_AGENT);
 }
+constexpr int32_t kLeaderOnDevice = INT32_MIN;
+__device__ __forceinline__ int32_t leader_arg_or_load(const BatchDev& b, int32_t leader_host) { return leader_host != kLeaderOnDevice ? leader_host : b.leader_epoch[0]; }
+__device__ __forceinline__ uint8_t panic_arg_or_load(const BatchDev& b, int32_t leader_host, uint32_t panic_host) {
+  return leader_host != kLeaderOnDevice ? (uint8_t)(panic_host ? 1 : 0) : b.panic_epoch[0];
+}
 template <int TS>
 __device__ __forceinline__ void leader_pre_load(const GroupsDev& gr, int32_t leader, Shape<TS> sh, LeaderPre& o) {
   const uint32_t l = leader >= 0 ? (uint32_t)leader : 0u;
@@ -341,13 +348,14 @@
 
 template <int TS, bool PUB = false, bool SLOTS = true, bool INL = false>
 __device__ __forceinline__ void fast_query_thread(const PodsDev& pods, const GroupsDev& gr, const BatchDev& b, const BatchParams& prm, uint32_t i,
-                                                  uint32_t nthreads, uint32_t end = BS_INF, uint32_t t = BS_INF) {
+                                                  uint32_t nthreads, uint32_t end = BS_INF, uint32_t t = BS_INF, int32_t leader_host = kLeaderOnDevice,
+                                                  uint32_t panic_host = 0) {
   const Shape<TS> sh(prm.S);
   const bool valid = i < pods.p && i < end;
   const uint32_t gate = prm.eph_gate;
   const uint32_t ii = valid ? i : 0u;
-  const int32_t leader0 = b.leader_epoch[0];
-  const uint8_t panic0 = b.panic_epoch[0];
+  const int32_t leader0 = leader_arg_or_load(b, leader_host);
+  const uint8_t panic0 = panic_arg_or_load(b, leader_host, panic_host);
   const uint32_t K = prm.run_filter ? (prm.k_host ? prm.k_host : *b.kclass) : 0u;
   const int32_t gi = pods.p ? pods.group[ii] : BS_POD_NOT_GROUPED;
   const uint8_t pfl = pods.p ? pods.flags[ii] : (uint8_t)0;
@@ -580,8 +588,10 @@
 template <int TS, bool REGS = false>
 __device__ __forceinline__ void table_scan_block(const NodesDev& nd, const BatchDev& b, const BatchParams& prm, const TableDesc* forced, uint32_t chunk, uint32_t nchunks,
                                                  uint32_t share, uint32_t nshares, uint32_t pod_blocks, uint32_t tk_pods0, uint32_t tk_tab0, const GroupsDev& gr,
-                                                 const int64_t* ckeys, const uint32_t* cpres, uint32_t kcap, bool direct = false, uint32_t forced_cls = 0) {
+                                                 const int64_t* ckeys, const uint32_t* cpres, uint32_t kcap, bool direct = false, uint32_t forced_cls = 0,
+                                                 int32_t leader_host = kLeaderOnDevice, uint32_t panic_host = 0, uint32_t totals_tag = 0, bool totals_reuse = false) {
   __shared__ unsigned long long s_wtot[BS_MAX_LANES][4];
+  __shared__ uint32_t s_ok;
   __shared__ uint32_t s_kp[BS_MAX_SCALARS];
   __shared__ unsigned long long s_off[BS_MAX_LANES];
   __shared__ uint32_t s_kpg[BS_MAX_SCALARS];
@@ -619,9 +629,92 @@
     for (uint32_t j = 0; j < BS_MAX_LANES; ++j)
       if (j < L) raw.v[j] = ckeys[(size_t)j * kcap + cc];
     raw.present = cpres[cc];
-    leader0 = b.leader_epoch[0];
-    panic0 = b.panic_epoch[0];
+    leader0 = leader_arg_or_load(b, leader_host);
+    panic0 = panic_arg_or_load(b, leader_host, panic_host);
     if (gr.g) leader_pre_load(gr, leader0, sh, lp0);
+  }
+  constexpr bool kTotalsFirst = TS > 2;
+  unsigned long long e_lo[BS_MAX_LANES], e_hi[BS_MAX_LANES], e_kw[BS_MAX_SCALARS];
+#pragma unroll
+  for (uint32_t j = 0; j < BS_MAX_LANES; ++j) e_lo[j] = e_hi[j] = 0ull;
+#pragma unroll
+  for (uint32_t s2 = 0; s2 < BS_MAX_SCALARS; ++s2) e_kw[s2] = 0ull;
+  const unsigned long long* const my_rec = b.chunk_rec + (size_t)((uint32_t)lane_id() < nchunks ? (uint32_t)lane_id() : 0u) * kRecStride;
+  if constexpr (REGS && !kTotalsFirst) {
+    if (totals_reuse && wave_id() == 0) {
+#pragma unroll
+      for (uint32_t j = 0; j < BS_MAX_LANES; ++j)
+        if (j < L) { e_lo[j] = ld_agent64(&my_rec[2u * j]); e_hi[j] = ld_agent64(&my_rec[2u * j + 1u]); }
+#pragma unroll
+      for (uint32_t s2 = 0; s2 < BS_MAX_SCALARS; ++s2)
+        if (s2 < S) e_kw[s2] = ld_agent64(&my_rec[16u + s2]);
+    }
+  }
+  auto totals_in = [&](auto early) {
+    const uint32_t ch = (uint32_t)lane_id();
+    unsigned long long cv[BS_MAX_LANES];
+    uint32_t ckp[BS_MAX_SCALARS];
+    const uint32_t tagw = totals_tag;
+    const unsigned long long* rec = my_rec;
+    bool ok = false;
+    for (uint32_t spins = 0;; ++spins) {
+      unsigned long long lo[BS_MAX_LANES], hi[BS_MAX_LANES], kw[BS_MAX_SCALARS];
+      if (decltype(early)::value && spins == 0u) {
+#pragma unroll
+        for (uint32_t j = 0; j < BS_MAX_LANES; ++j) { lo[j] = e_lo[j]; hi[j] = e_hi[j]; }
+#pragma unroll
+        for (uint32_t s2 = 0; s2 < BS_MAX_SCALARS; ++s2) kw[s2] = e_kw[s2];
+      } else {
+#pragma unroll
+        for (uint32_t j = 0; j < BS_MAX_LANES; ++j)
+          if (j < L) { lo[j] = ld_agent64(&rec[2u * j]); hi[j] = ld_agent64(&rec[2u * j + 1u]); }
+#pragma unroll
+        for (uint32_t s2 = 0; s2 < BS_MAX_SCALARS; ++s2)
+          if (s2 < S) kw[s2] = ld_agent64(&rec[16u + s2]);
+      }
+      bool mine_ok = true;
+#pragma unroll
+      for (uint32_t j = 0; j < BS_MAX_LANES; ++j) {
+        cv[j] = 0ull;
+        if (j < L) {
+          mine_ok = mine_ok && (uint32_t)(lo[j] >> 32) == tagw && (uint32_t)(hi[j] >> 32) == tagw;
+          cv[j] = (hi[j] << 32) | (uint32_t)lo[j];
+        }
+      }
+#pragma unroll
+      for (uint32_t s2 = 0; s2 < BS_MAX_SCALARS; ++s2) {
+        ckp[s2] = BS_INF;
+        if (s2 < S) { mine_ok = mine_ok && (uint32_t)(kw[s2] >> 32) == tagw; ckp[s2] = (uint32_t)kw[s2]; }
+      }
+      if (__ballot(!(mine_ok || ch >= nchunks)) == 0ull) { ok = true; break; }
+      if (spins > kSpinBound) { if (b.h_err && ch == 0) __hip_atomic_store(b.h_err, 1, __ATOMIC_RELAXED, __HIP_MEMORY_SCOPE_SYSTEM); break; }
+      __builtin_amdgcn_s_sleep(2);
+    }
+    if (ch >= nchunks) {
+#pragma unroll
+      for (uint32_t j = 0; j < BS_MAX_LANES; ++j) cv[j] = 0ull;
+#pragma unroll
+      for (uint32_t s2 = 0; s2 < BS_MAX_SCALARS; ++s2) ckp[s2] = BS_INF;
+    }
+    if (ch == 0) s_ok = ok ? 1u : 0u;
+#pragma unroll
+    for (uint32_t j = 0; j < BS_MAX_LANES; ++j) {
+      if (j < L) {
+        const unsigned long long incl_c = wave_incl_scan_add_u64(cv[j]);
+        const unsigned long long mine = bcast64(incl_c - cv[j], (int)(chunk & 63u));
+        if (ch == 0) s_off[j] = mine;
+      }
+    }
+#pragma unroll
+    for (uint32_t s2 = 0; s2 < BS_MAX_SCALARS; ++s2) {
+      if (s2 < S) {
+        const uint32_t mn = wave_min_u32(ckp[s2]);
+        if (ch == 0) s_kpg[s2] = mn;
+      }
+    }
+  };
+  if constexpr (REGS && kTotalsFirst) {
+    if (totals_reuse && wave_id() == 0) totals_in(std::false_type{});
   }
   const bool fit = valid && ((fw >> (n & 31u)) & 1u) && !(fl & BS_NODE_TAINT_ERR);
   const uint32_t pres = fit ? (ap & rp) : 0u;
@@ -658,7 +751,7 @@
         tot += x;
       }
       incl[j] += off;
-      if (threadIdx.x == 0 && share == 0) {
+      if (threadIdx.x == 0 && share == 0 && !(REGS && totals_reuse)) {
         if constexpr (REGS) {
           const unsigned long long tag = (unsigned long long)prm.seq_inv << 32;
           st_pub<true>(&b.chunk_rec[(size_t)chunk * kRecStride + 2u * j], tag | (uint32_t)tot);
@@ -670,9 +763,8 @@
     }
   }
   __syncthreads();
-  __shared__ uint32_t s_ok;
   if constexpr (REGS) {
-    if (share == 0 && threadIdx.x < S) st_pub<true>(&b.chunk_rec[(size_t)chunk * kRecStride + 16u + threadIdx.x], ((unsigned long long)prm.seq_inv << 32) | s_kp[threadIdx.x]);
+    if (share == 0 && !totals_reuse && threadIdx.x < S) st_pub<true>(&b.chunk_rec[(size_t)chunk * kRecStride + 16u + threadIdx.x], ((unsigned long long)prm.seq_inv << 32) | s_kp[threadIdx.x]);
     BS_STAMP(2, 1);
   } else {
     if (share == 0 && threadIdx.x < 16) st_pub<true>(&b.chunk_kp[(size_t)chunk * 16 + threadIdx.x], threadIdx.x < BS_MAX_SCALARS ? s_kp[threadIdx.x] : BS_INF);
@@ -711,42 +803,8 @@
     uint32_t ckp[BS_MAX_SCALARS];
     if constexpr (REGS) {
       if (w == 0) {
-        const uint32_t tagw = prm.seq_inv;
-        const unsigned long long* rec = b.chunk_rec + (size_t)(ch < nchunks ? ch : 0u) * kRecStride;
-        bool ok = false;
-        for (uint32_t spins = 0;; ++spins) {
-          unsigned long long lo[BS_MAX_LANES], hi[BS_MAX_LANES], kw[BS_MAX_SCALARS];
-#pragma unroll
-          for (uint32_t j = 0; j < BS_MAX_LANES; ++j)
-            if (j < L) { lo[j] = ld_agent64(&rec[2u * j]); hi[j] = ld_agent64(&rec[2u * j + 1u]); }
-#pragma unroll
-          for (uint32_t s2 = 0; s2 < BS_MAX_SCALARS; ++s2)
-            if (s2 < S) kw[s2] = ld_agent64(&rec[16u + s2]);
-          bool mine_ok = true;
-#pragma unroll
-          for (uint32_t j = 0; j < BS_MAX_LANES; ++j) {
-            cv[j] = 0ull;
-            if (j < L) {
-              mine_ok = mine_ok && (uint32_t)(lo[j] >> 32) == tagw && (uint32_t)(hi[j] >> 32) == tagw;
-              cv[j] = (hi[j] << 32) | (uint32_t)lo[j];
-            }
-          }
-#pragma unroll
-          for (uint32_t s2 = 0; s2 < BS_MAX_SCALARS; ++s2) {
-            ckp[s2] = BS_INF;
-            if (s2 < S) { mine_ok = mine_ok && (uint32_t)(kw[s2] >> 32) == tagw; ckp[s2] = (uint32_t)kw[s2]; }
-          }
-          if (__ballot(!(mine_ok || ch >= nchunks)) == 0ull) { ok = true; break; }
-          if (spins > kSpinBound) { if (b.h_err && ch == 0) __hip_atomic_store(b.h_err, 1, __ATOMIC_RELAXED, __HIP_MEMORY_SCOPE_SYSTEM); break; }
-          __builtin_amdgcn_s_sleep(2);
-        }
-        if (ch >= nchunks) {
-#pragma unroll
-          for (uint32_t j = 0; j < BS_MAX_LANES; ++j) cv[j] = 0ull;
-#pragma unroll
-          for (uint32_t s2 = 0; s2 < BS_MAX_SCALARS; ++s2) ckp[s2] = BS_INF;
-        }
-        if (ch == 0) s_ok = ok ? 1u : 0u;
+        if (!totals_reuse) totals_in(std::false_type{});
+        else if constexpr (!kTotalsFirst) totals_in(std::true_type{});
       }
       BS_STAMP(2, 2);
     } else if (w == 0) {
@@ -766,7 +824,7 @@
 #pragma unroll
       for (uint32_t j = 0; j < BS_MAX_LANES; ++j) rv[j] = j < L ? ld_agent64(&b.qreq_s[(size_t)t * LP + j]) : 0ull;
     }
-    if (w == 0) {
+    if (!REGS && w == 0) {
 #pragma unroll
       for (uint32_t j = 0; j < BS_MAX_LANES; ++j) {
         if (j < L) {
@@ -867,7 +925,7 @@
 template <int TS>
 __device__ __forceinline__ void step_filter_block(const GroupsDev& gr, const NodesDev& nd, const BatchDev& b, const BatchParams& prm, const int64_t* ckeys,
                                                   const uint32_t* cpres, uint32_t kcap, uint32_t target_waves, uint32_t ustride, uint32_t bx, uint32_t nblocks,
-                                                  bool direct, uint32_t tk_slots0, uint32_t slot_producers) {
+                                                  bool direct, uint32_t tk_slots0, uint32_t slot_producers, int32_t leader_host) {
   __shared__ uint32_t s_cnt[4][64];
   BS_STAMP_AT(4, 0, bx);
   const Shape<TS> sh(prm.S);
@@ -877,7 +935,7 @@
   uint32_t tiles, bpw, nchunk;
   step_filter_split(K, W, target_waves, tiles, bpw, nchunk);
   const uint32_t groups = (nchunk + 3u) / 4u;
-  const int32_t leader0 = b.leader_epoch[0];
+  const int32_t leader0 = leader_arg_or_load(b, leader_host);
   LeaderPre lp0{}, lp1{};
   const bool two = prm.sop_leader0 >= 0 && prm.sop_leader0 != leader0;
   if (gr.g) {
@@ -908,6 +966,9 @@
       filter_item<2, 4, true, true>(nd, b, U, ustride, tile, chunk * bpw, min(W, chunk * bpw + bpw), 0u,
                                     on ? (ff | ((uint32_t)BS_FL_EVALUATED << 8)) : ((uint32_t)BS_FL_NOT_RUN << 8), R, M, &cnt);
     }
+    uint32_t tk_seen = tk_slots0;
+    const bool look = !direct && !waited && wave_id() == 0;
+    if (look) tk_seen = ld_agent(&b.ticket[kTkSlots]);
     s_cnt[wave_id()][lane_id()] = cnt;
     BS_STAMP_AT(4, 1, bx);
     if (direct && b.h_rows) asm volatile("s_waitcnt vmcnt(0)" ::: "memory");
@@ -918,7 +979,10 @@
       if (direct) {
         st_pub<true>(&b.feas_rec[(size_t)group * (2u * kStepSlotsMax) + src], ((unsigned long long)prm.seq_inv << 32) | sum);
       } else {
-        if (!waited) { (void)step_wait(&b.ticket[kTkSlots], tk_slots0, slot_producers, b.h_err); waited = true; }
+        if (!waited) {
+          if ((uint32_t)(tk_seen - tk_slots0) < slot_producers) (void)step_wait(&b.ticket[kTkSlots], tk_slots0, slot_producers, b.h_err);
+          waited = true;
+        }
         if (sum) atomicAdd(&b.fu_feas[src], sum);
       }
     }
@@ -929,7 +993,7 @@
 
 template <int TS>
 __device__ __forceinline__ void class_slots_block(const GroupsDev& gr, const BatchDev& b, const BatchParams& prm, const int64_t* ckeys, const uint32_t* cpres,
-                                                  uint32_t kcap, uint32_t blk, bool zero_feas) {
+                                                  uint32_t kcap, uint32_t blk, bool zero_feas, int32_t leader_host = kLeaderOnDevice, uint32_t panic_host = 0) {
   const Shape<TS> sh(prm.S);
 #ifdef BS_TEST_OLD_ZERO
   zero_feas = true;
@@ -942,8 +1006,8 @@
   for (uint32_t j = 0; j < BS_MAX_LANES; ++j)
     if (j < sh.L()) raw.v[j] = ckeys[(size_t)j * kcap + cc];
   raw.present = cpres[cc];
-  const int32_t leader0 = b.leader_epoch[0];
-  const uint8_t panic0 = b.panic_epoch[0];
+  const int32_t leader0 = leader_arg_or_load(b, leader_host);
+  const uint8_t panic0 = panic_arg_or_load(b, leader_host, panic_host);
   LeaderPre lp0{}, lp1{};
   const bool two = prm.run_filter && prm.sop_leader0 >= 0 && prm.sop_leader0 != leader0;
   if (gr.g) {
@@ -1380,7 +1444,8 @@
 __global__ __launch_bounds__(kTblChunk) void k_fast_step_a(PodsDev pods, GroupsDev gr, NodesDev nd, BatchDev b, BatchDev bt, BatchParams prm, const TableDesc* forced,
                                                            uint32_t nchunks, uint32_t query_blocks, uint32_t nshares, uint32_t filter_blocks, uint32_t filter_waves,
                                                            uint32_t ustride, uint32_t tk_pods0, uint32_t tk_tab0, uint32_t param_blocks, const int64_t* ckeys,
-                                                           const uint32_t* cpres, uint32_t kcap, uint32_t tk_p1, uint32_t tk_done, uint32_t forced_cls) {
+                                                           const uint32_t* cpres, uint32_t kcap, uint32_t tk_p1, uint32_t tk_done, uint32_t forced_cls, int32_t leader_host,
+                                                           uint32_t panic_host, uint32_t totals_tag, uint32_t totals_reuse) {
   BS_STAMP(1, 0);
   test_chaos_delay();
   const uint32_t tb = nchunks * nshares;
@@ -1396,7 +1461,8 @@
     if constexpr (WHOLE) {
       const uint32_t p0 = b.pod_ranges ? range_start(b, gr.g)[blockIdx.x] : blockIdx.x * kTblChunk;
       const uint32_t p1 = b.pod_ranges ? range_start(b, gr.g)[blockIdx.x + 1u] : pods.p;
-      fast_query_thread<TS, false, false, true>(pods, gr, b, prm, p0 + threadIdx.x, query_blocks * kTblChunk, p1, blockIdx.x * kTblChunk + threadIdx.x);
+      fast_query_thread<TS, false, false, true>(pods, gr, b, prm, p0 + threadIdx.x, query_blocks * kTblChunk, p1, blockIdx.x * kTblChunk + threadIdx.x,
+                                                leader_host, panic_host);
       asm volatile("s_waitcnt vmcnt(0)" ::: "memory");
       __syncthreads();
       if (threadIdx.x == 0) spread_add(&b.ticket[kTkP1], blockIdx.x);
@@ -1412,10 +1478,11 @@
       if (threadIdx.x == 0) (void)__hip_atomic_fetch_add(&b.ticket[kTkSlots], 1u, __ATOMIC_RELAXED, __HIP_MEMORY_SCOPE_AGENT);
     }
   } else if (blockIdx.x < query_blocks + param_blocks) {
-    class_slots_block<TS>(gr, b, prm, ckeys, cpres, kcap, blockIdx.x - query_blocks, !(WHOLE && direct));
+    class_slots_block<TS>(gr, b, prm, ckeys, cpres, kcap, blockIdx.x - query_blocks, !(WHOLE && direct), leader_host, panic_host);
   } else if (blockIdx.x < query_blocks + param_blocks + tb) {
     const uint32_t x = blockIdx.x - query_blocks - param_blocks;
-    table_scan_block<TS, WHOLE>(nd, bt, prm, forced, x / nshares, nchunks, x % nshares, nshares, producers, tk_pods0, tk_tab0, gr, ckeys, cpres, kcap, direct, forced_cls);
+    table_scan_block<TS, WHOLE>(nd, bt, prm, forced, x / nshares, nchunks, x % nshares, nshares, producers, tk_pods0, tk_tab0, gr, ckeys, cpres, kcap, direct, forced_cls,
+                                leader_host, panic_host, totals_tag, totals_reuse != 0u);
     if constexpr (WHOLE) {
       if (!direct) {
         asm volatile("s_waitcnt vmcnt(0)" ::: "memory");
@@ -1424,7 +1491,8 @@
       }
     }
   } else if constexpr (WHOLE) {
-    step_filter_block<TS>(gr, nd, bt, prm, ckeys, cpres, kcap, filter_waves, ustride, blockIdx.x - query_blocks - param_blocks - tb, filter_blocks, direct, tk_pods0, producers);
+    step_filter_block<TS>(gr, nd, bt, prm, ckeys, cpres, kcap, filter_waves, ustride, blockIdx.x - query_blocks - param_blocks - tb, filter_blocks, direct, tk_pods0, producers,
+                          leader_host);
     if (!direct) {
       asm volatile("s_waitcnt vmcnt(0)" ::: "memory");
       __syncthreads();
diff --git a/batch-scheduler_amd/csrc/bs_launch.hpp b/batch-scheduler_amd/csrc/bs_launch.hpp
--- a/batch-scheduler_amd/csrc/bs_launch.hpp
+++ b/batch-scheduler_amd/csrc/bs_launch.hpp
@@ -24,7 +24,8 @@
 void launch_fast_step_a(const FastLaunch& c, dim3 grid, const PodsDev& pd, const GroupsDev& gr, const NodesDev& nd, const BatchDev& b, const BatchDev& bt,
                         const BatchParams& prm, const TableDesc* forced, uint32_t nchunks, uint32_t query_blocks, uint32_t nshares, uint32_t filter_blocks,
                         uint32_t tk_pods0, uint32_t tk_tab0, uint32_t param_blocks, const int64_t* ckeys, const uint32_t* cpres, uint32_t kcap,
-                        uint32_t whole, uint32_t tk_p1, uint32_t tk_done, uint32_t forced_cls);
+                        uint32_t whole, uint32_t tk_p1, uint32_t tk_done, uint32_t forced_cls, int32_t leader_host, uint32_t panic_host,
+                        uint32_t totals_tag, uint32_t totals_reuse);
 int step_a_residency_query(const FastLaunch& c, bool whole);
 
 }
diff --git a/batch-scheduler_amd/csrc/bs_totals_key.hpp b/batch-scheduler_amd/csrc/bs_totals_key.hpp
--- /dev/null
+++ b/batch-scheduler_amd/csrc/bs_totals_key.hpp
@@ -0,0 +1,31 @@
+#pragma once
+#include <stdint.h>
+
+namespace bs {
+
+struct TotalsKey {
+  uint64_t node_epoch = 0;
+  uint32_t forced_cls = 0;
+  uint32_t eph_gate = 0;
+  uint32_t S = 0, N = 0, nchunks = 0;
+  const void* rec = nullptr;
+  bool operator==(const TotalsKey& o) const {
+    return node_epoch == o.node_epoch && forced_cls == o.forced_cls && eph_gate == o.eph_gate && S == o.S && N == o.N && nchunks == o.nchunks && rec == o.rec;
+  }
+};
+
+class TotalsCache {
+  TotalsKey key_{};
+  uint32_t tag_ = 0;
+  bool valid_ = false;
+  uint64_t epoch_ = 1;
+
+ public:
+  uint64_t epoch() const { return epoch_; }
+  void touch_nodes() { ++epoch_; }
+  void invalidate() { valid_ = false; }
+  uint32_t reusable(const TotalsKey& k) const { return (valid_ && k == key_) ? tag_ : 0u; }
+  void rebuilt(const TotalsKey& k, uint32_t tag) { key_ = k; tag_ = tag; valid_ = tag != 0u; }
+};
+
+}
diff --git a/batch-scheduler_amd/csrc/bsched.hip b/batch-scheduler_amd/csrc/bsched.hip
--- a/batch-scheduler_amd/csrc/bsched.hip
+++ b/batch-scheduler_amd/csrc/bsched.hip
@@ -231,6 +231,7 @@
 
 int upload_nodes(bs_ctx* c, uint32_t lo = 0) {
   const uint32_t N = c->N, L = c->L;
+  nodes_touched(c);
   if (N > c->Ncap || c->Ncap == 0) {
     c->Ncap = std::max<uint32_t>(64, N + N / 4 + 64);
     c->d_tables.release();
@@ -275,6 +276,7 @@
 }
 
 int upload_fit(bs_ctx* c) {
+  nodes_touched(c);
   HIPCHK(c, c->d_fit.reserve(std::max<size_t>(4, c->h_fit.size() * 4)));
   if (!c->h_fit.empty())
     HIPCHK(c, hipMemcpyAsync(c->d_fit.p, c->h_fit.data(), c->h_fit.size() * 4, hipMemcpyHostToDevice, c->stream));
@@ -390,6 +392,9 @@
   int rc = wait_host_tag(c, 3, c->info_tag);
   if (rc) return rc;
   c->info_pending = false;
+  c->h_leader = c->h_info.p[0];
+  c->h_panic = c->h_info.p[1];
+  c->leader_known = true;
   c->steady_table = (c->n_uncaptured == 0 && c->h_info.p[2] >= 0) ? c->h_info.p[2] : -1;
   c->steady_prev = c->steady_table;
   return BS_OK;
@@ -597,7 +602,9 @@
 }
 uint32_t* pclass_dev(const bs_ctx* c) { return c->lay[c->cur_pack].pclass.in(c->d_pack[c->cur_pack].p); }
 
+void nodes_touched(bs_ctx* c) { c->totals.touch_nodes(); }
 void rederive_nodes(bs_ctx* c, uint32_t base0, uint32_t m_before) {
+  nodes_touched(c);
   hipLaunchKernelGGL(k_nodes_derive, dim3(1), dim3(kScanBlock), 0, c->stream, nodes_dev(c), c->d_kmap.as<uint32_t>(), c->d_m.as<uint32_t>(), c->d_left4.as<int64_t>(),
                      c->d_lglob.as<int64_t>(), base0, m_before);
 }
@@ -607,6 +614,7 @@
   c->steady_table = -1;
   c->side_ready = false;
   c->info_pending = false;
+  c->leader_known = false;
   if (!c->G) { c->scratch_armed = false; return BS_OK; }
   GroupsDev gr = groups_dev(c);
   BatchDev b = batch_dev(c);
@@ -642,6 +650,7 @@
 
 void launch_nodes_assume(bs_ctx* c, const bs_node_request* records, uint32_t n) {
   static_assert(sizeof(bs_node_request) == sizeof(NodeRequest), "node request layout");
+  nodes_touched(c);
   hipLaunchKernelGGL(k_nodes_assume, dim3(cdiv(n, 256)), dim3(256), 0, c->stream, reinterpret_cast<const NodeRequest*>(records), n, c->L, c->Ncap,
                      c->d_alloc.as<int64_t>(), c->d_nreq.as<int64_t>(), c->d_rpres.as<uint32_t>(), c->d_nflags.as<uint8_t>(), c->d_left4.as<int64_t>(),
                      c->d_lglob.as<int64_t>());
@@ -672,6 +681,7 @@
   if (c->h_info.p && ((volatile int32_t*)c->h_info.p)[12]) {
     ((volatile int32_t*)c->h_info.p)[12] = 0;
     c->no_fuse_final = 1;
+    c->totals.invalidate();
     c->batch_void = true;
     c->last_error = "in-launch hand-over timed out (producer blocks not resident): batch void, run it again (the context now uses separate launches)";
     return BS_ERR_RETRY;
@@ -726,6 +736,8 @@
   if (const char* e = std::getenv("BS_NO_NODEW")) c->no_nodew = std::atoi(e) != 0;
   if (const char* e = std::getenv("BS_TP_TMIN")) c->tp_tmin = (uint32_t)std::max(1, std::atoi(e));
   if (const char* e = std::getenv("BS_NO_SPECULATE")) c->no_spec = std::atoi(e) ? 1u : 0u;
+  if (const char* e = std::getenv("BS_STEP_TOTALS")) c->totals_on = std::atoi(e) ? 1u : 0u;
+  if (const char* e = std::getenv("BS_STEP_LEADER_ARG")) c->no_leader_arg = std::atoi(e) ? 0u : 1u;
   if (const char* e = std::getenv("BS_HOST_PROBE")) c->host_probe = std::atoi(e) ? 1u : 0u;
   if (const char* e = std::getenv("BS_HASH_SLOT_BITS")) { const int hb = std::atoi(e); c->slot_keep = hb >= 32 ? 0xFFFFFFFFu : ((1u << std::max(0, hb)) - 1u); }
   if (const char* e = std::getenv("BS_HASH_BITS")) { const int hb = std::atoi(e); c->hash_keep = hb >= 31 ? 0x7FFFFFFFu : ((1u << std::max(0, hb)) - 1u); }
@@ -931,6 +943,7 @@
   c->C = C;
   c->fit_words = cdiv(N, 32);
   c->h_fit.assign((size_t)C * c->fit_words, 0);
+  nodes_touched(c);
   HIPCHK(c, c->d_fit.reserve(std::max<size_t>(4, c->h_fit.size() * 4)));
   if (N) {
     const uint32_t nb = cdiv(N, 256);
@@ -1668,9 +1681,22 @@
     if (ranges) b.pod_ranges = c->d_pod_ranges.as<uint32_t>();
     const uint32_t grid = qb + pb + nchunks_s * nshares + fblocks;
     if ((k_known || whole) && (int)grid <= step_a_residency(c, whole != 0)) {
+      const bool leader_on_host = whole && c->leader_known && !c->spec_active && !c->info_pending && !c->no_leader_arg;
+      const int32_t leader_host = leader_on_host ? c->h_leader : kLeaderOnDevice;
+      if (whole) (leader_on_host ? c->n_leader_arg : c->n_leader_dev)++;
+      uint32_t totals_tag = prm.seq_inv, totals_reuse = 0;
+      if (whole) {
+        const TotalsKey key{c->totals.epoch(), side_slot - c->C, prm.eph_gate, c->S, N, nchunks_s, c->d_chunk_rec.p};
+        const uint32_t have = c->totals_on ? c->totals.reusable(key) : 0u;
+        if (have) { totals_tag = have; totals_reuse = 1; c->n_totals_reused++; }
+        else { c->totals.rebuilt(key, c->totals_on ? prm.seq_inv : 0u); c->n_totals_rebuilt++; }
+      } else {
+        c->totals.invalidate();
+      }
       TIMED(c, BS_KERNEL_QUERY, {
         launch_fast_step_a(fast_launch(c), dim3(grid), pd, gr, nd, b, bt, prm, forced, nchunks_s, qb, nshares, fblocks, c->tk_pods, c->tk_tab, pb,
-                           c->d_ckeys.as<int64_t>(), c->d_cpres.as<uint32_t>(), c->pair_cap, whole, c->tk_p1, c->tk_done, side_slot - c->C);
+                           c->d_ckeys.as<int64_t>(), c->d_cpres.as<uint32_t>(), c->pair_cap, whole, c->tk_p1, c->tk_done, side_slot - c->C, leader_host,
+                           leader_on_host ? (uint32_t)(c->h_panic != 0) : 0u, totals_tag, totals_reuse);
       });
       c->tk_pods += pb ? pb : qb;
       if (!whole) c->tk_tab += nchunks_s;
@@ -1703,6 +1729,7 @@
     }
   }
   c->last_step_a = false;
+  c->totals.invalidate();
   const uint32_t k_est = std::min<uint32_t>(P, c->kinfo_pending ? std::max<uint32_t>(2 * c->h_K, 1024) : std::max<uint32_t>(c->h_K, 1));
   const bool node_words = run_filter && cdiv(k_est, 64) > 16 && c->tp_filter >= 5u && !c->no_nodew && c->d_nodew.p;
   if (node_words) {
@@ -1942,6 +1969,7 @@
     if (c->d_scan_rec.p) HIPCHK(c, hipMemsetAsync(c->d_scan_rec.p, 0, c->d_scan_rec.cap, c->stream));
     if (c->d_feas_rec.p) HIPCHK(c, hipMemsetAsync(c->d_feas_rec.p, 0, c->d_feas_rec.cap, c->stream));
     if (c->d_chunk_rec.p) HIPCHK(c, hipMemsetAsync(c->d_chunk_rec.p, 0, c->d_chunk_rec.cap, c->stream));
+    c->totals.invalidate();
     if (c->d_gfirstq.p) HIPCHK(c, hipMemsetAsync(c->d_gfirstq.p, 0xFF, c->d_gfirstq.cap, c->stream));
     if (c->d_fd_event.p) HIPCHK(c, hipMemsetAsync(c->d_fd_event.p, 0xFF, c->d_fd_event.cap, c->stream));
     c->rekey_pending = false;
@@ -1964,6 +1992,7 @@
     advance_batch_seq(c);
     return rc;
   }
+  c->totals.invalidate();
   if (!c->no_fast && !c->no_epoch && !c->no_fuse_filter && P && G && N && c->M && !early_filter && c->cfg.enable_timing < 2) {
     bool taken = false;
     rc = run_epoch(c, stages, &taken);
@@ -2143,6 +2172,7 @@
   if (c->h_info.p && ((volatile int32_t*)c->h_info.p)[12]) {
     ((volatile int32_t*)c->h_info.p)[12] = 0;
     c->no_fuse_final = 1;
+    c->totals.invalidate();
   }
 }
 
@@ -2886,6 +2916,20 @@
   return BS_OK;
 }
 
+int bs_step_totals_stats(const bs_ctx* c, uint64_t* rebuilt, uint64_t* reused) {
+  if (!c || !rebuilt || !reused) return BS_ERR_INVALID;
+  *rebuilt = c->n_totals_rebuilt;
+  *reused = c->n_totals_reused;
+  return BS_OK;
+}
+
+int bs_step_leader_stats(const bs_ctx* c, uint64_t* on_host, uint64_t* on_device) {
+  if (!c || !on_host || !on_device) return BS_ERR_INVALID;
+  *on_host = c->n_leader_arg;
+  *on_device = c->n_leader_dev;
+  return BS_OK;
+}
+
 int bs_filter_deny_stats(const bs_ctx* c, uint64_t* reruns) {
   if (!c || !reruns) return BS_ERR_INVALID;
   *reruns = c->n_fd_reruns;
diff --git a/batch-scheduler_amd/csrc/tu_fast.hip b/batch-scheduler_amd/csrc/tu_fast.hip
--- a/batch-scheduler_amd/csrc/tu_fast.hip
+++ b/batch-scheduler_amd/csrc/tu_fast.hip
@@ -55,12 +55,13 @@
 void launch_fast_step_a(const FastLaunch& c, dim3 grid, const PodsDev& pd, const GroupsDev& gr, const NodesDev& nd, const BatchDev& b, const BatchDev& bt,
                         const BatchParams& prm, const TableDesc* forced, uint32_t nchunks, uint32_t query_blocks, uint32_t nshares, uint32_t filter_blocks,
                         uint32_t tk_pods0, uint32_t tk_tab0, uint32_t param_blocks, const int64_t* ckeys, const uint32_t* cpres, uint32_t kcap,
-                        uint32_t whole, uint32_t tk_p1, uint32_t tk_done, uint32_t forced_cls) {
+                        uint32_t whole, uint32_t tk_p1, uint32_t tk_done, uint32_t forced_cls, int32_t leader_host, uint32_t panic_host,
+                        uint32_t totals_tag, uint32_t totals_reuse) {
   lanes_clamped(c.S, [&](auto s) {
     auto launch = [&](auto whole_step) {
       hipLaunchKernelGGL(HIP_KERNEL_NAME(k_fast_step_a<decltype(s)::value, decltype(whole_step)::value>), grid, dim3(kTblChunk), 0, c.stream, pd, gr, nd, b, bt,
                          prm, forced, nchunks, query_blocks, nshares, filter_blocks, c.filter_waves, c.filter_slots_cap, tk_pods0, tk_tab0, param_blocks,
-                         ckeys, cpres, kcap, tk_p1, tk_done, forced_cls);
+                         ckeys, cpres, kcap, tk_p1, tk_done, forced_cls, leader_host, panic_host, totals_tag, totals_reuse);
     };
     if (whole) launch(std::true_type{});
     else launch(std::false_type{});
diff --git a/include/bsched.h b/include/bsched.h
--- a/include/bsched.h
+++ b/include/bsched.h
@@ -511,6 +511,8 @@
 int bs_pods_apply_stats(const bs_ctx* ctx, uint64_t* applies, uint64_t* rederives);
 int bs_filter_deny_stats(const bs_ctx* ctx, uint64_t* reruns);
 int bs_speculation_stats(const bs_ctx* ctx, uint64_t* launched, uint64_t* missed);
+int bs_step_leader_stats(const bs_ctx* ctx, uint64_t* on_host, uint64_t* on_device);
+int bs_step_totals_stats(const bs_ctx* ctx, uint64_t* rebuilt, uint64_t* reused);
 
 #ifdef __cplusplus
 }
```

Measured after the change: 3765 billion evals/s, median of 3. Within noise of the previous version (+0.6%).
